# Bazs/structure_from_motion

Measured on NVIDIA B200. Metric: hyp x point evals/sec (fp64), higher is better.
Workload: dtype f64

## Files before the change

### structure_from_motion_b200/csrc/sfm_api.cu

```cuda
#include "../../include/sfm_b200.h"

#include <dlfcn.h>

#include <cmath>
#include <cstdarg>
#include <cstdio>
#include <cstdlib>
#include <cstring>
#include <string>
#include <vector>

#include "sfm_device.cuh"
#include "sfm_fit.cuh"
#include "sfm_linalg.cuh"
#include "sfm_score.cuh"
#include "sfm_homography.cuh"
#include "sfm_pose.cuh"
#include "sfm_tail.cuh"
#include "sfm_misc.cuh"
#include "sfm_match.cuh"
#include "sfm_harris.cuh"
#include "sfm_select.cuh"

using namespace sfm;

static_assert(sizeof(Corr) == 32, "Corr must be 32 bytes");
static_assert(sizeof(PoseSet) == sizeof(sfm_poses), "PoseSet/sfm_poses layout mismatch");
static_assert(sizeof(SelectRecord) == SFM_RECORD_BYTES, "SelectRecord / SFM_RECORD_BYTES mismatch");
static_assert(sizeof(ModelScores) == sizeof(sfm_model_scores), "ModelScores / sfm_model_scores layout mismatch");

namespace {

thread_local std::string g_err;

int fail(int code, const char* fmt, ...) {
    char buf[512];
    va_list ap;
    va_start(ap, fmt);
    vsnprintf(buf, sizeof buf, fmt, ap);
    va_end(ap);
    g_err = buf;
    return code;
}

}

int sfm_internal_set_error(int code, const char* message) {
    g_err = message;
    return code;
}

namespace {

#define CU(call)                                                                                   \
    do {                                                                                           \
        cudaError_t e_ = (call);                                                                   \
        if (e_ != cudaSuccess)                                                                     \
            return fail(SFM_ERR_CUDA, "%s failed: %s (%s:%d)", #call, cudaGetErrorString(e_), __FILE__, \
                        __LINE__);                                                                 \
    } while (0)

struct Buf {
    void* p = nullptr;
    size_t cap = 0;
    int reserve(size_t bytes) {
        if (bytes <= cap) return 0;
        if (p) cudaFree(p);
        p = nullptr;
        cap = 0;
        size_t want = bytes + bytes / 4 + 256;
        cudaError_t e = cudaMalloc(&p, want);
        if (e != cudaSuccess) return fail(SFM_ERR_CUDA, "cudaMalloc(%zu) failed: %s", want, cudaGetErrorString(e));
        cap = want;
        return 0;
    }
    template <class T>
    T* as() const { return reinterpret_cast<T*>(p); }
    void release() {
        if (p) cudaFree(p);
        p = nullptr;
        cap = 0;
    }
};

enum { T_UPLOAD = 0, T_SAMPLE, T_FIT, T_SCORE, T_SELECT, T_MASK, T_POSE, T_TRI, T_COUNT };

}

struct sfm_ctx {
    int device = 0;
    int sm_count = 148;
    cudaStream_t own_stream = nullptr, stream = nullptr;
    Buf raw, pts, offsets, Ks, table, E, valid, eig;
    Buf acc, count_extra, S1, S2, err, blocks, best, invalid, winnerE, spts, bounds, fitflag, record, merged, rows, blockinv;
    Buf m_img, m_feat, m_W, m_ss, m_ok, m_S, m_out;
    Buf h_img, h_gx, h_gy, h_corner, h_alive, h_key, h_idx, h_small, h_xy;
    Buf mask, sed, poses, pass, X, idx, scan, tmp, tailstate, num, winrec, bout;
    Buf planes, hK;
    Buf selstate, selio, selpp;
    long long n = 0, h = 0, npairs = 1;
    long long first_len = 0;
    long long batch_max_len = 0;
    long long raw_stride = 1;
    bool batched = false, has_pts = false, has_table = false, has_models = false, has_score = false;
    bool models_h = false;
    int hscore_occ = 0;
    bool table_pending = false;
    unsigned long long smp_seed = 0, smp_stream = 0;
    long long smp_offset = 0;
    bool acc_clean = false;
    size_t acc_planes_for = 0;
    double Kstage[9] = {0};
    double hstage[18] = {0};
    std::vector<SelectModels> sstage;
    std::vector<double> Kbatch;
    const void* occ_fn[4] = {nullptr, nullptr, nullptr, nullptr};
    int occ_blocks[4] = {0, 0, 0, 0};
    int occ_next = 0;
    void* nccl_comm = nullptr;
    int nccl_rank = 0, nccl_world = 1;
    Buf gathered;
    const unsigned long long* rescored_dev = nullptr;
    long long winner_local = -1;
    bool winner_set = false;
    long long last_idx_offset = 0;
    double Khost[9] = {1, 0, 0, 0, 1, 0, 0, 0, 1};
    int variant = SFM_SCORE_AUTO, hpt = 2, group = 16;
    bool timing = false;
    cudaEvent_t ev0[T_COUNT], ev1[T_COUNT];
    bool ev_used[T_COUNT];
    long long launches = 0;
    void* hpin = nullptr;
    size_t hpin_cap = 0;

    void tic(int s) {
        if (timing) { cudaEventRecord(ev0[s], stream); }
    }
    void toc(int s) {
        if (timing) { cudaEventRecord(ev1[s], stream); ev_used[s] = true; }
    }
};

namespace {

int ensure_pinned(sfm_ctx* c, size_t bytes) {
    if (bytes <= c->hpin_cap) return 0;
    if (c->hpin) cudaFreeHost(c->hpin);
    c->hpin = nullptr;
    c->hpin_cap = 0;
    CU(cudaMallocHost(&c->hpin, bytes + 4096));
    c->hpin_cap = bytes + 4096;
    return 0;
}

int use(sfm_ctx* c) {
    if (!c) return fail(SFM_ERR_ARG, "null context");
    CU(cudaSetDevice(c->device));
    return 0;
}

int reserve_zeroed(sfm_ctx* c, Buf& b, size_t bytes) {
    if (bytes <= b.cap) return 0;
    if (int r = b.reserve(bytes)) return r;
    CU(cudaMemsetAsync(b.p, 0, b.cap, c->stream));
    return 0;
}

int check_launch(sfm_ctx* c, const char* what) {
    cudaError_t e = cudaGetLastError();
    if (e != cudaSuccess) return fail(SFM_ERR_CUDA, "launch of %s failed: %s", what, cudaGetErrorString(e));
    c->launches += 1;
#ifdef SFM_TRACE
    fprintf(stderr, "[sfm] %s ...", what);
    fflush(stderr);
    e = cudaStreamSynchronize(c->stream);
    fprintf(stderr, " %s\n", e == cudaSuccess ? "ok" : cudaGetErrorString(e));
    fflush(stderr);
#endif
    return 0;
}

inline void chain_config(sfm_ctx* c, dim3 grid, dim3 block, size_t smem, cudaLaunchConfig_t* cfg, cudaLaunchAttribute* at) {
    memset(cfg, 0, sizeof *cfg);
    cfg->gridDim = grid;
    cfg->blockDim = block;
    cfg->dynamicSmemBytes = smem;
    cfg->stream = c->stream;
    at->id = cudaLaunchAttributeProgrammaticStreamSerialization;
    at->val.programmaticStreamSerializationAllowed = 1;
    cfg->attrs = at;
    cfg->numAttrs = SFM_PDL ? 1 : 0;
}
template <typename... KArgs, typename... Args>
cudaError_t chain_launch(sfm_ctx* c, void (*kernel)(KArgs...), dim3 grid, dim3 block, size_t smem, Args&&... args) {
    cudaLaunchConfig_t cfg;
    cudaLaunchAttribute at;
    chain_config(c, grid, block, smem, &cfg, &at);
    return cudaLaunchKernelEx(&cfg, kernel, static_cast<KArgs>(args)...);
}
inline cudaError_t chain_launch_ptr(sfm_ctx* c, const void* fn, dim3 grid, dim3 block, size_t smem, void** kargs) {
    cudaLaunchConfig_t cfg;
    cudaLaunchAttribute at;
    chain_config(c, grid, block, smem, &cfg, &at);
    return cudaLaunchKernelExC(&cfg, fn, kargs);
}

size_t score_warp_smem(int hpt, bool full) {
    switch (hpt) {
        case 1: return full ? score_warp_bytes<1, MODE_FULL>() : sizeof(ScoreWarpSmem<1>);
        case 2: return full ? score_warp_bytes<2, MODE_FULL>() : sizeof(ScoreWarpSmem<2>);
        case 4: return full ? score_warp_bytes<4, MODE_FULL>() : sizeof(ScoreWarpSmem<4>);
        default: return sizeof(ScoreWarpSmem<8>);
    }
}

const void* score_kernel(int variant, int hpt, int group) {
    if (variant == SFM_SCORE_SCREEN32) {
#define SFM_K32(H, G) if (hpt == H && group == G) return reinterpret_cast<const void*>(&k_score<H, G, MODE_SCREEN32>)
        SFM_K32(2, 16); SFM_K32(4, 8); SFM_K32(8, 4);
#undef SFM_K32
        return nullptr;
    }
#define SFM_K(H, G) if (hpt == H && group == G) return scr ? reinterpret_cast<const void*>(&k_score<H, G, MODE_SCREEN>) \
                                                           : reinterpret_cast<const void*>(&k_score<H, G, MODE_FULL>)
    const bool scr = variant == SFM_SCORE_SCREEN;
    SFM_K(1, 16); SFM_K(1, 32);
    SFM_K(2, 4); SFM_K(2, 8); SFM_K(2, 16);
    SFM_K(4, 2); SFM_K(4, 4); SFM_K(4, 8);
#undef SFM_K
    return nullptr;
}

}

extern "C" {

int sfm_version(void) { return 100; }
const char* sfm_last_error(void) { return g_err.c_str(); }

int sfm_device_count(void) {
    int n = 0;
    if (cudaGetDeviceCount(&n) != cudaSuccess) {
        cudaGetLastError();
        return 0;
    }
    return n;
}

int sfm_create(int device, sfm_ctx** out) {
    if (!out) return fail(SFM_ERR_ARG, "out is null");
    *out = nullptr;
    int n = 0;
    cudaError_t e = cudaGetDeviceCount(&n);
    if (e != cudaSuccess || n == 0) {
        cudaGetLastError();
        return fail(SFM_ERR_NO_DEVICE, "no CUDA device available (%s)",
                    e != cudaSuccess ? cudaGetErrorString(e) : "device count is 0");
    }
    if (device < 0 || device >= n) return fail(SFM_ERR_ARG, "device %d out of range [0,%d)", device, n);
    CU(cudaSetDevice(device));
    cudaDeviceProp prop;
    CU(cudaGetDeviceProperties(&prop, device));
    if (prop.major < 10)
        return fail(SFM_ERR_NO_DEVICE, "device %d is sm_%d%d; this library is built for sm_100a only", device,
                    prop.major, prop.minor);
    sfm_ctx* c = new sfm_ctx();
    c->device = device;
    c->sm_count = prop.multiProcessorCount;
    CU(cudaStreamCreateWithFlags(&c->own_stream, cudaStreamNonBlocking));
    c->stream = c->own_stream;
    for (int i = 0; i < T_COUNT; ++i) {
        CU(cudaEventCreate(&c->ev0[i]));
        CU(cudaEventCreate(&c->ev1[i]));
        c->ev_used[i] = false;
    }
    CU(cudaFuncSetAttribute(k_fit, cudaFuncAttributeMaxDynamicSharedMemorySize,
                            (int)(kFitThreads * kFitSmemDoubles * sizeof(double))));
    *out = c;
    return 0;
}

int sfm_destroy(sfm_ctx* c) {
    if (!c) return 0;
    cudaSetDevice(c->device);
    cudaStreamSynchronize(c->stream);
    Buf* bufs[] = {&c->raw, &c->pts, &c->offsets, &c->Ks, &c->table, &c->E, &c->valid, &c->eig, &c->acc,
                   &c->count_extra, &c->S1, &c->S2, &c->err, &c->blocks, &c->best,
                   &c->invalid, &c->winnerE, &c->record, &c->merged, &c->rows, &c->blockinv, &c->mask, &c->sed, &c->poses, &c->pass, &c->X, &c->idx,
                   &c->planes, &c->hK, &c->selstate, &c->selio, &c->selpp,
                   &c->scan, &c->tmp, &c->gathered, &c->tailstate, &c->num, &c->winrec, &c->bout, &c->spts, &c->bounds, &c->fitflag,
                   &c->m_img, &c->m_feat, &c->m_W, &c->m_ss, &c->m_ok, &c->m_S, &c->m_out,
                   &c->h_img, &c->h_gx, &c->h_gy, &c->h_corner, &c->h_alive, &c->h_key, &c->h_idx, &c->h_small, &c->h_xy};
    for (Buf* b : bufs) b->release();
    for (int i = 0; i < T_COUNT; ++i) {
        cudaEventDestroy(c->ev0[i]);
        cudaEventDestroy(c->ev1[i]);
    }
    sfm_nccl_destroy(c);
    if (c->hpin) cudaFreeHost(c->hpin);
    cudaStreamDestroy(c->own_stream);
    delete c;
    return 0;
}

int sfm_set_stream(sfm_ctx* c, void* s) {
    if (int r = use(c)) return r;
    c->stream = s ? (cudaStream_t)s : c->own_stream;
    return 0;
}

int sfm_use_default_stream(sfm_ctx* c) {
    if (int r = use(c)) return r;
    c->stream = cudaStreamLegacy;
    return 0;
}

int sfm_synchronize(sfm_ctx* c) {
    if (int r = use(c)) return r;
    CU(cudaStreamSynchronize(c->stream));
    return 0;
}

int sfm_set_score_variant(sfm_ctx* c, int variant, int hpt, int group) {
    if (!c) return fail(SFM_ERR_ARG, "null context");
    if (variant != SFM_SCORE_SCREEN && variant != SFM_SCORE_FULL && variant != SFM_SCORE_SCREEN32 && variant != SFM_SCORE_AUTO)
        return fail(SFM_ERR_ARG, "bad variant %d", variant);
    int nh = hpt ? hpt : c->hpt, ng = group ? group : c->group;
    if (!hpt && (variant == SFM_SCORE_SCREEN32) != (c->variant == SFM_SCORE_SCREEN32)) {
        nh = variant == SFM_SCORE_SCREEN32 ? 4 : 2;
        ng = variant == SFM_SCORE_SCREEN32 ? 8 : 16;
    }
    if (!score_kernel(variant == SFM_SCORE_AUTO ? SFM_SCORE_SCREEN : variant, nh, ng) ||
        (variant == SFM_SCORE_AUTO && !score_kernel(SFM_SCORE_FULL, nh, ng)))
        return fail(SFM_ERR_ARG, "unsupported combination: hyps_per_thread %d, group %d", nh, ng);
    c->variant = variant;
    c->hpt = nh;
    c->group = ng;
    return 0;
}

int sfm_host_alloc(uint64_t bytes, void** out) {
    if (!out) return fail(SFM_ERR_ARG, "out is null");
    CU(cudaMallocHost(out, bytes ? bytes : 1));
    return 0;
}
int sfm_host_free(void* p) {
    if (p) CU(cudaFreeHost(p));
    return 0;
}

int sfm_set_table(sfm_ctx* c, const int32_t* table, int64_t h) {
    if (int r = use(c)) return r;
    if (!table || h <= 0) return fail(SFM_ERR_ARG, "bad table");
    if (!c->has_pts) return fail(SFM_ERR_STATE, "upload correspondences before the sample table");
    for (int64_t i = 0; i < 8 * h; ++i)
        if (table[i] < 0 || table[i] >= c->n) return fail(SFM_ERR_ARG, "table[%lld] = %d out of range", (long long)i, table[i]);
    if (int r = c->table.reserve((size_t)h * 32)) return r;
    CU(cudaMemcpyAsync(c->table.p, table, (size_t)h * 32, cudaMemcpyHostToDevice, c->stream));
    CU(cudaStreamSynchronize(c->stream));
    c->h = h;
    c->npairs = 1;
    c->has_table = true;
    c->table_pending = false;
    c->has_models = false;
    c->has_score = false;
    return 0;
}

static int sample_device(sfm_ctx* c, uint64_t seed, uint64_t stream, int64_t hyp_offset, int64_t h) {
    if (h <= 0) return fail(SFM_ERR_ARG, "need h > 0");
    if (!c->has_pts) return fail(SFM_ERR_STATE, "upload correspondences before sampling");
    if (!c->batched && c->n < 8) return fail(SFM_ERR_ARG, "need at least 8 correspondences");
    if (int r = c->table.reserve((size_t)h * c->npairs * 32)) return r;
    c->smp_seed = seed;
    c->smp_stream = stream;
    c->smp_offset = hyp_offset;
    c->table_pending = true;
    c->h = h;
    c->has_table = true;
    c->has_models = false;
    c->has_score = false;
    return 0;
}

static int ensure_table(sfm_ctx* c) {
    if (!c->table_pending) return 0;
    c->tic(T_SAMPLE);
    dim3 grid((unsigned)((c->h + 127) / 128), (unsigned)c->npairs);
    k_sample<<<grid, 128, 0, c->stream>>>(c->smp_seed, c->smp_stream, c->smp_offset, c->h, c->n,
                                          c->batched ? c->offsets.as<long long>() : nullptr, c->table.as<int32_t>());
    if (int r = check_launch(c, "k_sample")) return r;
    c->toc(T_SAMPLE);
    c->table_pending = false;
    return 0;
}

int sfm_sample_device(sfm_ctx* c, uint64_t seed, uint64_t stream, int64_t hyp_offset, int64_t h) {
    if (int r = use(c)) return r;
    return sample_device(c, seed, stream, hyp_offset, h);
}

int sfm_get_table(sfm_ctx* c, int32_t* table, int64_t first, int64_t h) {
    if (int r = use(c)) return r;
    if (!c->has_table || first < 0 || h < 0 || first + h > c->h * c->npairs)
        return fail(SFM_ERR_STATE, "no table rows [%lld, %lld)", (long long)first, (long long)(first + h));
    if (int r = ensure_table(c)) return r;
    CU(cudaMemcpyAsync(table, c->table.as<int32_t>() + 8 * first, (size_t)h * 32, cudaMemcpyDeviceToHost, c->stream));
    CU(cudaStreamSynchronize(c->stream));
    return 0;
}

static int normalise_from(sfm_ctx* c, const double* xa, const double* ya, const double* xb, const double* yb,
                          int64_t stride, int64_t n, int64_t max_len) {
    if (int r = c->pts.reserve((size_t)n * sizeof(Corr))) return r;
    if (int r = c->bounds.reserve(16)) return r;
    CU(cudaMemsetAsync(c->bounds.p, 0, 16, c->stream));
    dim3 grid((unsigned)((max_len + 255) / 256), (unsigned)c->npairs);
    k_normalise<<<grid, 256, 0, c->stream>>>(xa, ya, xb, yb, stride, n,
                                             c->batched ? c->offsets.as<long long>() : nullptr,
                                             c->Ks.as<double>(), c->pts.as<Corr>(), c->bounds.as<unsigned long long>());
    return check_launch(c, "k_normalise");
}

static int stage_coords(sfm_ctx* c, double* d, const double* xa, const double* ya, const double* xb, const double* yb,
                        int64_t stride, int64_t n, const double* s[4]) {
    if (stride == 1) {
        const double* src[4] = {xa, ya, xb, yb};
        for (int k = 0; k < 4; ++k)
            CU(cudaMemcpyAsync(d + (size_t)k * n, src[k], (size_t)n * sizeof(double), cudaMemcpyHostToDevice, c->stream));
        s[0] = d; s[1] = d + n; s[2] = d + 2 * n; s[3] = d + 3 * n;
    } else if (stride == 2 && ya == xa + 1 && yb == xb + 1) {
        CU(cudaMemcpyAsync(d, xa, (size_t)n * 2 * sizeof(double), cudaMemcpyHostToDevice, c->stream));
        CU(cudaMemcpyAsync(d + 2 * n, xb, (size_t)n * 2 * sizeof(double), cudaMemcpyHostToDevice, c->stream));
        s[0] = d; s[1] = d + 1; s[2] = d + 2 * n; s[3] = d + 2 * n + 1;
    } else {
        return fail(SFM_ERR_ARG, "unsupported layout: stride must be 1 (four arrays) or 2 (two interleaved [n][2] arrays)");
    }
    return 0;
}

static void raw_coords(const sfm_ctx* c, const double* s[4]) {
    const double* d = c->raw.as<double>();
    const long long n = c->n;
    if (c->raw_stride == 1) { s[0] = d; s[1] = d + n; s[2] = d + 2 * n; s[3] = d + 3 * n; }
    else { s[0] = d; s[1] = d + 1; s[2] = d + 2 * n; s[3] = d + 2 * n + 1; }
}

static int stage_raw(sfm_ctx* c, const double* xa, const double* ya, const double* xb, const double* yb,
                     int64_t stride, int64_t n, const double* s[4]) {
    if (int r = c->raw.reserve((size_t)n * 4 * sizeof(double))) return r;
    if (int r = stage_coords(c, c->raw.as<double>(), xa, ya, xb, yb, stride, n, s)) return r;
    c->raw_stride = stride;
    return 0;
}

static int upload_pairs_impl(sfm_ctx* c, const double* xa, const double* ya, const double* xb, const double* yb,
                             int64_t stride, int64_t n, const double* K, bool on_device, bool sync) {
    if (int r = use(c)) return r;
    if (!xa || !ya || !xb || !yb || !K) return fail(SFM_ERR_ARG, "null argument");
    if (n <= 0 || (uint64_t)n >= kMaxPoints) return fail(SFM_ERR_ARG, "need 0 < n < 2^25 correspondences, got %lld", (long long)n);
    c->tic(T_UPLOAD);
    c->batched = false;
    c->npairs = 1;
    const double* s[4];
    if (on_device) {
        if (int r = c->raw.reserve((size_t)n * 4 * sizeof(double))) return r;
        double* d = c->raw.as<double>();
        const double* src[4] = {xa, ya, xb, yb};
        for (int k = 0; k < 4; ++k) {
            CU(cudaMemcpy2DAsync(d + (size_t)k * n, sizeof(double), src[k], (size_t)stride * sizeof(double),
                                 sizeof(double), (size_t)n, cudaMemcpyDeviceToDevice, c->stream));
            s[k] = d + (size_t)k * n;
        }
        c->raw_stride = stride = 1;
    } else if (int r = stage_raw(c, xa, ya, xb, yb, stride, n, s)) {
        return r;
    }
    if (int r = c->Ks.reserve(9 * sizeof(double))) return r;
    memcpy(c->Khost, K, sizeof c->Khost);
    CU(cudaMemcpyAsync(c->Ks.p, c->Khost, 9 * sizeof(double), cudaMemcpyHostToDevice, c->stream));
    c->n = n;
    if (int r = normalise_from(c, s[0], s[1], s[2], s[3], stride, n, n)) return r;
    c->toc(T_UPLOAD);
    if (sync) CU(cudaStreamSynchronize(c->stream));
    c->has_pts = true;
    c->has_table = c->has_models = c->has_score = false;
    c->table_pending = false;
    c->winner_set = false;
    return 0;
}

int sfm_upload_pairs(sfm_ctx* c, const double* xa, const double* ya, const double* xb, const double* yb,
                     int64_t stride, int64_t n, const double* K) {
    return upload_pairs_impl(c, xa, ya, xb, yb, stride, n, K, false, true);
}

int sfm_upload_pairs_async(sfm_ctx* c, const double* xa, const double* ya, const double* xb, const double* yb,
                           int64_t stride, int64_t n, const double* K) {
    return upload_pairs_impl(c, xa, ya, xb, yb, stride, n, K, false, false);
}

int sfm_upload_pairs_d(sfm_ctx* c, const double* xa, const double* ya, const double* xb, const double* yb,
                       int64_t stride, int64_t n, const double* K) {
    return upload_pairs_impl(c, xa, ya, xb, yb, stride, n, K, true, true);
}

int sfm_get_normalised(sfm_ctx* c, double* out, int64_t n) {
    if (int r = use(c)) return r;
    if (!c->has_pts || n > c->n) return fail(SFM_ERR_STATE, "no correspondences of that size");
    CU(cudaMemcpyAsync(out, c->pts.p, (size_t)n * sizeof(Corr), cudaMemcpyDeviceToHost, c->stream));
    CU(cudaStreamSynchronize(c->stream));
    return 0;
}

static size_t acc_tail_bytes(long long P) { return 64 + (size_t)P * 4; }

static int fit_launch(sfm_ctx* c, bool want_eig) {
    if (!c->has_pts || !c->has_table) return fail(SFM_ERR_STATE, "fit needs correspondences and a sample table");
    const size_t H = (size_t)c->h * c->npairs;
    if (int r = c->E.reserve(H * 9 * sizeof(double))) return r;
    if (int r = c->valid.reserve(H)) return r;
    if (want_eig)
        if (int r = c->eig.reserve(H * 9 * sizeof(double))) return r;
    if (int r = reserve_zeroed(c, c->fitflag, 16)) return r;
    if (int r = c->rows.reserve(H * sizeof(ModelRow))) return r;
    const size_t acc_tail = acc_tail_bytes(c->npairs);
    if (int r = c->acc.reserve(H * kAccWords * 8 + acc_tail)) return r;
    if (want_eig)
        if (int r = ensure_table(c)) return r;
    c->tic(T_FIT);
    const long long* off = c->batched ? c->offsets.as<long long>() : nullptr;
    dim3 grid((unsigned)((c->h + kFitThreads - 1) / kFitThreads), (unsigned)c->npairs);
    const unsigned* only = nullptr;
    if (!want_eig) {
        dim3 gq((unsigned)((c->h + kFitQrThreads - 1) / kFitQrThreads), (unsigned)c->npairs);
        CU(chain_launch(c, k_fit_qr, gq, dim3(kFitQrThreads), 0, c->pts.as<Corr>(), off, c->table.as<int32_t>(), c->h,
                        c->E.as<double>(), c->valid.as<uint8_t>(), c->fitflag.as<unsigned>(), c->rows.as<ModelRow>(),
                        c->acc.as<unsigned long long>(), kAccWords, (int)((acc_tail + 7) / 8), c->table_pending ? 1 : 0,
                        c->smp_seed, c->smp_stream, c->smp_offset, c->n));
        if (int r = check_launch(c, "k_fit_qr")) return r;
        c->table_pending = false;
        only = c->fitflag.as<unsigned>();
        c->acc_clean = true;
        c->acc_planes_for = H;
    } else {
        c->acc_clean = false;
    }
    CU(chain_launch(c, k_fit, grid, dim3(kFitThreads), kFitThreads * kFitSmemDoubles * sizeof(double), c->pts.as<Corr>(), off,
                    c->table.as<int32_t>(), c->h, c->E.as<double>(), c->valid.as<uint8_t>(),
                    want_eig ? c->eig.as<double>() : nullptr, only, c->rows.as<ModelRow>()));
    if (int r = check_launch(c, "k_fit")) return r;
    c->toc(T_FIT);
    c->has_models = true;
    c->models_h = false;
    c->has_score = false;
    return 0;
}

int sfm_fit(sfm_ctx* c, double* E_out, uint8_t* valid_out, double* eig_out) {
    if (int r = use(c)) return r;
    if (int r = fit_launch(c, eig_out != nullptr)) return r;
    const size_t H = (size_t)c->h * c->npairs;
    if (E_out) CU(cudaMemcpyAsync(E_out, c->E.p, H * 72, cudaMemcpyDeviceToHost, c->stream));
    if (valid_out) CU(cudaMemcpyAsync(valid_out, c->valid.p, H, cudaMemcpyDeviceToHost, c->stream));
    if (eig_out) CU(cudaMemcpyAsync(eig_out, c->eig.p, H * 72, cudaMemcpyDeviceToHost, c->stream));
    CU(cudaStreamSynchronize(c->stream));
    return 0;
}

int sfm_get_models(sfm_ctx* c, int64_t first, int64_t count, double* E_out, uint8_t* valid_out) {
    if (int r = use(c)) return r;
    const int64_t total = c->h * c->npairs;
    if (!c->has_models || first < 0 || count < 0 || first + count > total)
        return fail(SFM_ERR_STATE, "no models [%lld, %lld)", (long long)first, (long long)(first + count));
    if (E_out) CU(cudaMemcpyAsync(E_out, c->E.as<double>() + 9 * first, (size_t)count * 72, cudaMemcpyDeviceToHost, c->stream));
    if (valid_out) CU(cudaMemcpyAsync(valid_out, c->valid.as<uint8_t>() + first, (size_t)count, cudaMemcpyDeviceToHost, c->stream));
    CU(cudaStreamSynchronize(c->stream));
    return 0;
}

int sfm_set_models(sfm_ctx* c, const double* E, const uint8_t* valid, int64_t h) {
    if (int r = use(c)) return r;
    if (!E || h <= 0) return fail(SFM_ERR_ARG, "bad models");
    if (c->batched) return fail(SFM_ERR_STATE, "set_models is a single-pair call");
    if (c->has_table && h != c->h) return fail(SFM_ERR_ARG, "model count %lld != table rows %lld", (long long)h, c->h);
    if (int r = c->E.reserve((size_t)h * 72)) return r;
    if (int r = c->valid.reserve((size_t)h)) return r;
    CU(cudaMemcpyAsync(c->E.p, E, (size_t)h * 72, cudaMemcpyHostToDevice, c->stream));
    if (valid) CU(cudaMemcpyAsync(c->valid.p, valid, (size_t)h, cudaMemcpyHostToDevice, c->stream));
    else CU(cudaMemsetAsync(c->valid.p, 1, (size_t)h, c->stream));
    if (int r = c->rows.reserve((size_t)h * sizeof(ModelRow))) return r;
    k_pad_models<<<(unsigned)((h + 255) / 256), 256, 0, c->stream>>>(c->E.as<double>(), (long long)h, c->rows.as<ModelRow>());
    if (int r = check_launch(c, "k_pad_models")) return r;
    CU(cudaStreamSynchronize(c->stream));
    c->h = h;
    c->has_models = true;
    c->models_h = false;
    c->has_score = false;
    c->acc_clean = false;
    return 0;
}

static int reserve_selection(sfm_ctx* c, long long h, long long P) {
    const size_t H = (size_t)h * P;
    const int fblocks = (int)((h + 255) / 256);
    if (int r = c->count_extra.reserve(H * 4)) return r;
    if (int r = c->S1.reserve(H * 8)) return r;
    if (int r = c->S2.reserve(H * 8)) return r;
    if (int r = c->err.reserve(H * 8)) return r;
    if (int r = c->blocks.reserve((size_t)fblocks * P * sizeof(Best))) return r;
    if (int r = c->best.reserve((size_t)P * sizeof(Best))) return r;
    if (int r = c->invalid.reserve((size_t)P * 16)) return r;
    return 0;
}

struct ItemSplit { long long chunk, nsplit; };
static ItemSplit split_items(long long target_items, long long hyp_items, long long max_len, long long tile) {
    const long long tiles = (max_len + tile - 1) / tile;
    long long nsplit = (target_items + hyp_items - 1) / hyp_items;
    constexpr int min_tiles = 2;
    const long long max_split = tiles / min_tiles > 0 ? tiles / min_tiles : 1;
    if (nsplit > max_split) nsplit = max_split;
    const long long min_split = (max_len + kMaxItemPoints - 1) / kMaxItemPoints;
    if (nsplit < min_split) nsplit = min_split;
    if (nsplit < 1) nsplit = 1;
    const long long chunk = ((tiles + nsplit - 1) / nsplit) * tile;
    nsplit = (max_len + chunk - 1) / chunk;
    if (nsplit < 1) nsplit = 1;
    return {chunk, nsplit};
}

static int clear_acc(sfm_ctx* c, size_t H, long long P) {
    if (!(c->acc_clean && c->acc_planes_for == H))
        CU(cudaMemsetAsync(c->acc.p, 0, H * kAccWords * 8 + acc_tail_bytes(P), c->stream));
    c->acc_clean = false;
    return 0;
}

static int finalise_launch(sfm_ctx* c, int kind, double thr, double min_extra, int agg, int mode, bool use_table,
                           long long idx_offset, int sums, int e2, int force_rescore, unsigned long long* acc_dev) {
    const long long h = c->h, P = c->npairs;
    const size_t H = (size_t)h * P;
    const int fblocks = (int)((h + 255) / 256);
    c->tic(T_SELECT);
    FinalArgs f;
    f.pts = c->pts.as<Corr>();
    f.offsets = c->batched ? c->offsets.as<long long>() : nullptr;
    f.E = c->E.as<double>();
    f.valid = c->valid.as<uint8_t>();
    f.table = use_table ? c->table.as<int32_t>() : nullptr;
    f.h = h;
    f.n = c->n;
    f.idx_offset = idx_offset;
    f.htotal = (long long)H;
    f.acc = acc_dev;
    f.inv_scale1 = ldexp(1.0, e2 - kFixedBits);
    f.sums = sums;
    f.inv_scale2 = ldexp(1.0, 2 * e2 - kFixedBits);
    f.thr = thr;
    f.min_extra = min_extra;
    f.agg = agg;
    f.mode = mode;
    f.count_extra = c->count_extra.as<int32_t>();
    f.S1 = c->S1.as<double>();
    f.S2 = c->S2.as<double>();
    f.err = c->err.as<double>();
    f.block_out = c->blocks.as<Best>();
    if (int r = c->blockinv.reserve((size_t)fblocks * P * 16)) return r;
    f.block_inv = c->blockinv.as<long long>();
    if (int r = c->record.reserve((size_t)P * sizeof(SelectRecord))) return r;
    f.force_rescore = force_rescore;
    f.rescored = reinterpret_cast<unsigned long long*>(reinterpret_cast<char*>(acc_dev + H * kAccWords) + 8);
    f.tickets = reinterpret_cast<unsigned*>(reinterpret_cast<char*>(acc_dev + H * kAccWords) + 64);
    c->rescored_dev = f.rescored;
    f.out = c->best.as<Best>();
    f.invalid_out = c->invalid.as<long long>();
    f.record = c->record.as<SelectRecord>();
    f.fitflag = c->fitflag.as<unsigned>();
    if (kind == MODEL_H) CU(chain_launch(c, k_finalise<MODEL_H>, dim3((unsigned)fblocks, (unsigned)P), dim3(256), 0, f));
    else CU(chain_launch(c, k_finalise<MODEL_E>, dim3((unsigned)fblocks, (unsigned)P), dim3(256), 0, f));
    if (int r = check_launch(c, "k_finalise")) return r;
    c->toc(T_SELECT);
    c->has_score = true;
    c->last_idx_offset = idx_offset;
    c->winner_set = false;
    return 0;
}

static int score_launch(sfm_ctx* c, double thr, double min_extra, int agg, int mode, bool use_table,
                        long long idx_offset, long long max_len, bool both_sums = false) {
    int sums = both_sums ? (SUM_S1 | SUM_S2) : ((agg == AGG_SUM || agg == AGG_MEAN) ? SUM_S1 : SUM_S2);
    if (mode == SELECT_MSAC) sums |= SUM_S1;
    if (!c->has_pts || !c->has_models) return fail(SFM_ERR_STATE, "score needs correspondences and fitted models");
    if (c->models_h) return fail(SFM_ERR_STATE, "the models are homographies: score them with sfm_ransac_homography");
    if (use_table && !c->has_table) return fail(SFM_ERR_STATE, "sample rule requested but no table is loaded");
    if (use_table)
        if (int r = ensure_table(c)) return r;
    if (agg < 0 || agg > 3) return fail(SFM_ERR_ARG, "bad aggregation %d", agg);
    if (mode < 0 || mode > 2) return fail(SFM_ERR_ARG, "bad selection %d", mode);
    const bool skip_k2 = !(thr >= 0.0) || thr > 1e100;
    const int force_rescore = (thr > 1e100) ? 1 : 0;
    const long long h = c->h, P = c->npairs;
    const int hpt = (c->variant == SFM_SCORE_SCREEN32 && thr > 1e6) ? 2 : c->hpt;
    const int G = (c->variant == SFM_SCORE_SCREEN32 && thr > 1e6) ? 16 : c->group;
    const long long hblocks = (h + 32ll * hpt - 1) / (32ll * hpt);
    const size_t H = (size_t)h * P;
    if (int r = reserve_selection(c, h, P)) return r;
    int e2 = 0;
    if (thr > 0.0 && !skip_k2) (void)frexp(thr, &e2);
    if (e2 < -400) e2 = -400;
    const bool autov = c->variant == SFM_SCORE_AUTO;
    int variant = autov ? SFM_SCORE_SCREEN : c->variant;
    if (variant == SFM_SCORE_SCREEN32 && thr > 1e6) variant = SFM_SCORE_SCREEN;
    const bool f32 = variant == SFM_SCORE_SCREEN32;
    const bool screen = variant != SFM_SCORE_FULL;
    double thr_pre = f32 ? thr * kThr32Factor : (screen ? thr * (1.0 + 1e-9) : thr * (1.0 + 1e-9) + 1e-22);
    if (f32 && thr_pre < 1e-24) thr_pre = 1e-24;
    if (screen && thr_pre < 1e-280) thr_pre = 1e-280;
    const double s_scale = sqrt(thr_pre);
    const double scale1 = ldexp(1.0, 63 - e2), scale2 = ldexp(1.0, 63 - 2 * e2);
    unsigned long long* acc_dev = nullptr;
    {
        const void* fn = score_kernel(variant, hpt, G);
        if (!fn) return fail(SFM_ERR_ARG, "unsupported scoring configuration (variant %d, hpt %d, group %d)", variant, hpt, G);
        const size_t smem_one = (size_t)kScoreWarps * score_warp_smem(hpt, false);
        const size_t smem_two = (size_t)kScoreWarps * score_warp_smem(hpt, true);
        const size_t smem_both = smem_one > smem_two ? smem_one : smem_two;
        const size_t smem = screen ? smem_one : smem_two;
        auto occupancy = [&](const void* f, size_t bytes, int* out) -> int {
            for (int k = 0; k < 4; ++k)
                if (c->occ_fn[k] == f) { *out = c->occ_blocks[k]; return 0; }
            int o = 0;
            CU(cudaFuncSetAttribute(f, cudaFuncAttributeMaxDynamicSharedMemorySize, (int)bytes));
            CU(cudaOccupancyMaxActiveBlocksPerMultiprocessor(&o, f, kScoreThreads, bytes));
            if (o < 1) o = 1;
            c->occ_fn[c->occ_next] = f;
            c->occ_blocks[c->occ_next] = o;
            c->occ_next = (c->occ_next + 1) & 3;
            *out = o;
            return 0;
        };
        int occ = 0;
        if (int r = occupancy(fn, smem, &occ)) return r;
#ifndef SFM_AUTO_SINGLE
#define SFM_AUTO_SINGLE 1
#endif
        const void* fn_auto = nullptr;
        if (autov && SFM_AUTO_SINGLE) {
            if (hpt == 2 && G == 16) fn_auto = reinterpret_cast<const void*>(&k_score_auto<2, 16>);
            if (hpt == 4 && G == 8) fn_auto = reinterpret_cast<const void*>(&k_score_auto<4, 8>);
        }
        if (fn_auto)
            if (int r = occupancy(fn_auto, smem_both, &occ)) return r;
        const void* fn_full = (autov && !fn_auto) ? score_kernel(SFM_SCORE_FULL, hpt, G) : nullptr;
        int occ_full = 0;
        if (fn_full)
            if (int r = occupancy(fn_full, smem_two, &occ_full)) return r;
        const long long grid_blocks = (long long)c->sm_count * occ;
        constexpr int items_per_warp = 32;
        const ItemSplit sp = split_items(grid_blocks * kScoreWarps * items_per_warp, hblocks * P, max_len, kTile);
        const long long chunk = sp.chunk, nsplit = sp.nsplit;
        const long long total_items = hblocks * nsplit * P;
        if (int r = c->acc.reserve(H * kAccWords * 8 + acc_tail_bytes(P))) return r;
        const long long npts = c->n;
        if (f32) { if (int r = c->spts.reserve((size_t)npts * sizeof(Corr32))) return r; }
        else if (screen) { if (int r = c->spts.reserve((size_t)npts * sizeof(Corr))) return r; }
        ScoreArgs a;
        a.pts = c->pts.as<Corr>();
        a.spts = screen ? c->spts.p : c->pts.p;
        a.bounds = c->bounds.as<double>();
        a.s = s_scale;
        a.kappa_coef = kKappaCoef * (1.0 + thr);
        a.kappa32_coef = kKappa32Coef * (1.0 + thr);
        a.n = c->n;
        a.offsets = c->batched ? c->offsets.as<long long>() : nullptr;
        a.E = c->E.as<double>();
        a.rows = c->rows.as<ModelRow>();
        a.h = h;
        a.thr = thr;
        a.thr_pre = thr_pre;
        a.scale1 = scale1;
        a.scale2 = scale2;
        a.sums = sums;
        a.chunk = chunk;
        a.hblocks = (int)hblocks;
        a.nsplit = (int)nsplit;
        a.total_items = total_items;
        a.htotal = (long long)H;
        a.acc = c->acc.as<unsigned long long>();
        a.work_counter = reinterpret_cast<unsigned*>(a.acc + H * kAccWords);
        char* tailp = reinterpret_cast<char*>(a.acc + H * kAccWords);
        a.mode_flag = autov ? reinterpret_cast<const int*>(tailp + 32) : nullptr;
        acc_dev = a.acc;
        c->tic(T_SCORE);
        if (int r = clear_acc(c, H, P)) return r;
        if (f32 && !skip_k2) {
            k_screen_pts32<<<(unsigned)((npts + 255) / 256), 256, 0, c->stream>>>(c->pts.as<Corr>(), npts, 1.0 / s_scale,
                                                                                  reinterpret_cast<Corr32*>(c->spts.p));
            if (int r = check_launch(c, "k_screen_pts32")) return r;
        }
        else if (screen && !skip_k2) {
            PilotArgs pa;
            pa.E = c->E.as<double>();
            pa.h = h;
            pa.plen = c->batched ? c->first_len : c->n;
            pa.thr_pre = thr_pre;
            pa.counters = reinterpret_cast<unsigned*>(tailp + 16);
            pa.mode_flag = autov ? reinterpret_cast<int*>(tailp + 32) : nullptr;
            CU(chain_launch(c, k_screen_pts64, dim3((unsigned)((npts + 255) / 256)), dim3(256), 0, c->pts.as<Corr>(), npts,
                            1.0 / s_scale, reinterpret_cast<Corr*>(c->spts.p), pa));
            if (int r = check_launch(c, "k_screen_pts64")) return r;
        }
        const long long want_blocks = (total_items + kScoreWarps - 1) / kScoreWarps;
        const long long launch_blocks = grid_blocks < want_blocks ? grid_blocks : want_blocks;
        void* kargs[] = {(void*)&a};
        if (!skip_k2 && fn_auto) {
            ScoreArgs a2 = a;
            a2.thr_pre = thr * (1.0 + 1e-9) + 1e-22;
            a2.spts = c->pts.p;
            void* kargs2[] = {(void*)&a, (void*)&a2};
            CU(chain_launch_ptr(c, fn_auto, dim3((unsigned)launch_blocks), dim3(kScoreThreads), smem_both, kargs2));
            if (int r = check_launch(c, "k_score_auto")) return r;
        } else if (!skip_k2) {
            CU(chain_launch_ptr(c, fn, dim3((unsigned)launch_blocks), dim3(kScoreThreads), smem, kargs));
            if (int r = check_launch(c, "k_score")) return r;
            if (fn_full) {
                ScoreArgs a2 = a;
                a2.thr_pre = thr * (1.0 + 1e-9) + 1e-22;
                a2.spts = c->pts.p;
                const long long gb2 = (long long)c->sm_count * occ_full;
                const long long lb2 = gb2 < want_blocks ? gb2 : want_blocks;
                void* kargs2[] = {(void*)&a2};
                CU(chain_launch_ptr(c, fn_full, dim3((unsigned)lb2), dim3(kScoreThreads), smem_two, kargs2));
                if (int r = check_launch(c, "k_score")) return r;
            }
        }
        c->toc(T_SCORE);
    }

    return finalise_launch(c, MODEL_E, thr, min_extra, agg, mode, use_table, idx_offset, sums, e2, force_rescore, acc_dev);
}

int sfm_score(sfm_ctx* c, double thr, double min_extra, int agg, int mode, int use_table, int64_t idx_offset,
              int32_t* count_extra, double* S1, double* S2, double* err) {
    if (int r = use(c)) return r;
    if (c->batched) return fail(SFM_ERR_STATE, "sfm_score is a single-pair call; use sfm_batch_ransac");
    if (int r = score_launch(c, thr, min_extra, agg, mode, use_table != 0, idx_offset, c->n, S1 || S2)) return r;
    const size_t H = (size_t)c->h;
    if (count_extra) CU(cudaMemcpyAsync(count_extra, c->count_extra.p, H * 4, cudaMemcpyDeviceToHost, c->stream));
    if (S1) CU(cudaMemcpyAsync(S1, c->S1.p, H * 8, cudaMemcpyDeviceToHost, c->stream));
    if (S2) CU(cudaMemcpyAsync(S2, c->S2.p, H * 8, cudaMemcpyDeviceToHost, c->stream));
    if (err) CU(cudaMemcpyAsync(err, c->err.p, H * 8, cudaMemcpyDeviceToHost, c->stream));
    CU(cudaStreamSynchronize(c->stream));
    return 0;
}

static void unpack_best(const SelectRecord& r, sfm_best* out) {
    out->err = r.best.idx >= 0 ? r.best.err : __builtin_inf();
    out->index = r.best.idx;
    out->count_extra = r.best.count;
    out->reserved = 0;
    out->num_invalid = r.num_invalid;
    out->first_invalid = r.first_invalid;
    memcpy(out->E, r.E, 72);
    memcpy(out->sample, r.sample, 32);
}

static int fetch_best(sfm_ctx* c, sfm_best* out) {
    if (int r = ensure_pinned(c, sizeof(SelectRecord))) return r;
    CU(cudaMemcpyAsync(c->hpin, c->record.p, sizeof(SelectRecord), cudaMemcpyDeviceToHost, c->stream));
    CU(cudaStreamSynchronize(c->stream));
    SelectRecord r;
    memcpy(&r, c->hpin, sizeof r);
    unpack_best(r, out);
    if (r.best.idx >= 0) {
        c->winner_local = r.best.idx - c->last_idx_offset;
        c->winner_set = true;
    }
    return 0;
}

int sfm_get_best(sfm_ctx* c, sfm_best* out) {
    if (int r = use(c)) return r;
    if (!out) return fail(SFM_ERR_ARG, "out is null");
    if (!c->has_score || c->batched) return fail(SFM_ERR_STATE, "no single-pair score to read");
    return fetch_best(c, out);
}

int sfm_near_ties(sfm_ctx* c, double rel_tol, int64_t cap, int64_t* idx_out, int64_t* count) {
    if (int r = use(c)) return r;
    if (!idx_out || !count || cap <= 0 || cap > 4096) return fail(SFM_ERR_ARG, "bad near-tie arguments");
    if (!c->has_score || c->batched) return fail(SFM_ERR_STATE, "no single-pair score to read");
    if (int r = c->tmp.reserve((size_t)cap * 8 + 16)) return r;
    unsigned* cnt = c->tmp.as<unsigned>();
    long long* out = reinterpret_cast<long long*>(c->tmp.as<char>() + 16);
    CU(cudaMemsetAsync(cnt, 0, 16, c->stream));
    const int blocks = (int)((c->h + 255) / 256 < 4 * c->sm_count ? (c->h + 255) / 256 : 4 * c->sm_count);
    k_near_ties<<<blocks, 256, 0, c->stream>>>(c->err.as<double>(), c->h, c->record.as<SelectRecord>(), rel_tol, (int)cap, out, cnt);
    if (int r = check_launch(c, "k_near_ties")) return r;
    if (int r = ensure_pinned(c, (size_t)cap * 8 + 16)) return r;
    CU(cudaMemcpyAsync(c->hpin, c->tmp.p, (size_t)cap * 8 + 16, cudaMemcpyDeviceToHost, c->stream));
    CU(cudaStreamSynchronize(c->stream));
    unsigned n;
    memcpy(&n, c->hpin, 4);
    *count = n;
    const int64_t take = n < (unsigned)cap ? n : cap;
    memcpy(idx_out, (char*)c->hpin + 16, (size_t)take * 8);
    return 0;
}

int sfm_get_rescored(sfm_ctx* c, int64_t* count) {
    if (int r = use(c)) return r;
    if (!count) return fail(SFM_ERR_ARG, "null argument");
    if (!c->rescored_dev) return fail(SFM_ERR_STATE, "no scoring call yet");
    if (int r = ensure_pinned(c, 8)) return r;
    CU(cudaMemcpyAsync(c->hpin, c->rescored_dev, 8, cudaMemcpyDeviceToHost, c->stream));
    CU(cudaStreamSynchronize(c->stream));
    unsigned long long v;
    memcpy(&v, c->hpin, 8);
    *count = (int64_t)v;
    return 0;
}

int sfm_set_winner(sfm_ctx* c, int64_t local_index, const double* E) {
    if (int r = use(c)) return r;
    if (local_index >= 0) {
        if (!c->has_models || local_index >= c->h) return fail(SFM_ERR_ARG, "winner index out of range");
        c->winner_local = local_index;
    } else {
        if (!E) return fail(SFM_ERR_ARG, "need the winning model when it lives on another rank");
        if (int r = c->winnerE.reserve(72)) return r;
        CU(cudaMemcpyAsync(c->winnerE.p, E, 72, cudaMemcpyHostToDevice, c->stream));
        CU(cudaStreamSynchronize(c->stream));
        c->winner_local = -1;
    }
    c->winner_set = true;
    return 0;
}

static const double* winner_E_dev(sfm_ctx* c) {
    return c->winner_local >= 0 ? c->E.as<double>() + 9 * c->winner_local : c->winnerE.as<double>();
}

static int mask_launch(sfm_ctx* c, double thr, const Best* best_dev, const double* E_override = nullptr) {
    if (int r = c->mask.reserve((size_t)c->n)) return r;
    if (int r = c->sed.reserve((size_t)c->n * 8)) return r;
    c->tic(T_MASK);
    const double* E = E_override ? E_override : (best_dev ? c->E.as<double>() : winner_E_dev(c));
    k_inlier_mask<<<(unsigned)((c->n + 255) / 256), 256, 0, c->stream>>>(
        c->pts.as<Corr>(), c->n, E, E_override ? nullptr : best_dev, c->last_idx_offset, 0, thr, c->mask.as<uint8_t>(),
        c->sed.as<double>());
    if (int r = check_launch(c, "k_inlier_mask")) return r;
    c->toc(T_MASK);
    return 0;
}

int sfm_inlier_mask(sfm_ctx* c, double thr, uint8_t* mask, double* sed) {
    if (int r = use(c)) return r;
    if (!c->has_pts || c->batched) return fail(SFM_ERR_STATE, "no single-pair correspondences loaded");
    if (!c->winner_set) return fail(SFM_ERR_STATE, "no winner: call sfm_get_best or sfm_set_winner first");
    if (c->models_h && c->winner_local >= 0) return fail(SFM_ERR_STATE, "the winner is a homography: use sfm_homography_mask");
    if (int r = mask_launch(c, thr, nullptr)) return r;
    if (mask) CU(cudaMemcpyAsync(mask, c->mask.p, (size_t)c->n, cudaMemcpyDeviceToHost, c->stream));
    if (sed) CU(cudaMemcpyAsync(sed, c->sed.p, (size_t)c->n * 8, cudaMemcpyDeviceToHost, c->stream));
    CU(cudaStreamSynchronize(c->stream));
    return 0;
}

int sfm_ransac_essential(sfm_ctx* c, double thr, double min_extra, int agg, int mode, sfm_best* best,
                         uint8_t* mask, double* sed) {
    if (int r = use(c)) return r;
    if (!best) return fail(SFM_ERR_ARG, "best is null");
    if (c->batched) return fail(SFM_ERR_STATE, "single-pair call on a batched context");
    if (int r = fit_launch(c, false)) return r;
    if (int r = score_launch(c, thr, min_extra, agg, mode, true, 0, c->n)) return r;
    if (mask || sed) {
        if (int r = mask_launch(c, thr, c->best.as<Best>())) return r;
        if (mask) CU(cudaMemcpyAsync(mask, c->mask.p, (size_t)c->n, cudaMemcpyDeviceToHost, c->stream));
        if (sed) CU(cudaMemcpyAsync(sed, c->sed.p, (size_t)c->n * 8, cudaMemcpyDeviceToHost, c->stream));
    }
    return fetch_best(c, best);
}

static int fit_h_launch(sfm_ctx* c) {
    if (!c->has_pts || !c->has_table) return fail(SFM_ERR_STATE, "fit needs correspondences and a sample table");
    if (c->batched && !c->table_pending) return fail(SFM_ERR_STATE, "a batch is fitted from the device sampler's draw");
    const long long h = c->h, P = c->npairs;
    const size_t H = (size_t)h * P;
    if (int r = c->E.reserve(H * 72)) return r;
    if (int r = c->valid.reserve(H)) return r;
    const size_t acc_tail = acc_tail_bytes(P);
    if (int r = c->acc.reserve(H * kAccWords * 8 + acc_tail)) return r;
    c->tic(T_FIT);
    CU(chain_launch(c, k_fit_homography, dim3((unsigned)((h + kFitHThreads - 1) / kFitHThreads), (unsigned)P),
                    dim3(kFitHThreads), 0, c->pts.as<Corr>(), c->batched ? c->offsets.as<long long>() : nullptr,
                    c->table.as<int32_t>(), h, c->E.as<double>(), c->valid.as<uint8_t>(), c->acc.as<unsigned long long>(),
                    kAccWords, (int)((acc_tail + 7) / 8), c->table_pending ? 1 : 0, c->smp_seed, c->smp_stream,
                    c->smp_offset, c->n));
    if (int r = check_launch(c, "k_fit_homography")) return r;
    c->toc(T_FIT);
    c->table_pending = false;
    c->acc_clean = true;
    c->acc_planes_for = H;
    c->has_models = true;
    c->models_h = true;
    c->has_score = false;
    return 0;
}

static int score_h_launch(sfm_ctx* c, double thr, double min_extra, int agg, int mode, long long max_len) {
    if (agg < 0 || agg > 3) return fail(SFM_ERR_ARG, "bad aggregation %d", agg);
    if (mode < 0 || mode > 2) return fail(SFM_ERR_ARG, "bad selection %d", mode);
    int sums = (agg == AGG_SUM || agg == AGG_MEAN) ? SUM_S1 : SUM_S2;
    if (mode == SELECT_MSAC) sums |= SUM_S1;
    const bool skip_k2 = !(thr >= 0.0) || thr > 1e100;
    const int force_rescore = (thr > 1e100) ? 1 : 0;
    const long long h = c->h, n = c->n, P = c->npairs;
    const size_t H = (size_t)h * P;
    int e2 = 0;
    if (thr > 0.0 && !skip_k2) (void)frexp(thr * (1.0 + 0x1p-20), &e2);
    if (e2 < -400) e2 = -400;
    if (int r = reserve_selection(c, h, P)) return r;
    if (int r = c->acc.reserve(H * kAccWords * 8 + acc_tail_bytes(P))) return r;
    unsigned long long* acc = c->acc.as<unsigned long long>();
    const size_t smem = kHScoreWarps * sizeof(HScoreWarpSmem);
    if (!c->hscore_occ) {
        int o = 0;
        CU(cudaOccupancyMaxActiveBlocksPerMultiprocessor(&o, k_score_homography<kHScoreHpt>, kHScoreThreads, smem));
        c->hscore_occ = o > 0 ? o : 1;
    }
    const long long grid_blocks = (long long)c->sm_count * c->hscore_occ;
    const long long hblocks = (h + 32ll * kHScoreHpt - 1) / (32ll * kHScoreHpt);
    const ItemSplit sp = split_items(grid_blocks * kHScoreWarps * 32, hblocks * P, max_len, kHTile);
    const long long chunk = sp.chunk, nsplit = sp.nsplit;
    HScoreArgs a;
    a.pts = c->pts.as<Corr>();
    a.offsets = c->batched ? c->offsets.as<long long>() : nullptr;
    a.H = c->E.as<double>();
    a.n = n;
    a.h = h;
    a.htotal = (long long)H;
    a.thr = thr;
    a.scale1 = ldexp(1.0, 63 - e2);
    a.scale2 = ldexp(1.0, 63 - 2 * e2);
    a.sums = sums;
    a.chunk = chunk;
    a.hblocks = (int)hblocks;
    a.nsplit = (int)nsplit;
    a.total_items = hblocks * nsplit * P;
    a.work_counter = reinterpret_cast<unsigned*>(acc + H * kAccWords);
    a.acc = acc;
    c->tic(T_SCORE);
    if (int r = clear_acc(c, H, P)) return r;
    if (!skip_k2) {
        const long long want = (a.total_items + kHScoreWarps - 1) / kHScoreWarps;
        CU(chain_launch(c, k_score_homography<kHScoreHpt>, dim3((unsigned)(grid_blocks < want ? grid_blocks : want)),
                        dim3(kHScoreThreads), smem, a));
        if (int r = check_launch(c, "k_score_homography")) return r;
    }
    c->toc(T_SCORE);
    return finalise_launch(c, MODEL_H, thr, min_extra, agg, mode, true, 0, sums, e2, force_rescore, acc);
}

static int hmask_launch(sfm_ctx* c, double thr, const double* H_dev, const Best* best_dev) {
    if (int r = c->mask.reserve((size_t)c->n)) return r;
    if (int r = c->sed.reserve((size_t)c->n * 8)) return r;
    c->tic(T_MASK);
    CU(chain_launch(c, k_homography_mask, dim3((unsigned)((c->n + 255) / 256)), dim3(256), 0, c->pts.as<Corr>(), c->n,
                    H_dev, best_dev, thr, c->mask.as<uint8_t>(), c->sed.as<double>()));
    if (int r = check_launch(c, "k_homography_mask")) return r;
    c->toc(T_MASK);
    return 0;
}

int sfm_fit_homography(sfm_ctx* c, double* H_out, uint8_t* valid_out) {
    if (int r = use(c)) return r;
    if (c->batched) return fail(SFM_ERR_STATE, "homography estimation is a single-pair call; use sfm_batch_two_view_homography");
    if (int r = fit_h_launch(c)) return r;
    if (H_out) CU(cudaMemcpyAsync(H_out, c->E.p, (size_t)c->h * 72, cudaMemcpyDeviceToHost, c->stream));
    if (valid_out) CU(cudaMemcpyAsync(valid_out, c->valid.p, (size_t)c->h, cudaMemcpyDeviceToHost, c->stream));
    CU(cudaStreamSynchronize(c->stream));
    return 0;
}

int sfm_ransac_homography(sfm_ctx* c, double thr, double min_extra, int agg, int mode, sfm_best* best, uint8_t* mask,
                          double* err, int32_t* count_extra_h, double* err_h) {
    if (int r = use(c)) return r;
    if (!best) return fail(SFM_ERR_ARG, "best is null");
    if (c->batched) return fail(SFM_ERR_STATE, "single-pair call on a batched context");
    if (c->has_pts && c->n < 8) return fail(SFM_ERR_ARG, "need at least 8 correspondences, got %lld", c->n);
    if (int r = fit_h_launch(c)) return r;
    if (int r = score_h_launch(c, thr, min_extra, agg, mode, c->n)) return r;
    if (mask || err) {
        if (int r = hmask_launch(c, thr, c->E.as<double>(), c->best.as<Best>())) return r;
        if (mask) CU(cudaMemcpyAsync(mask, c->mask.p, (size_t)c->n, cudaMemcpyDeviceToHost, c->stream));
        if (err) CU(cudaMemcpyAsync(err, c->sed.p, (size_t)c->n * 8, cudaMemcpyDeviceToHost, c->stream));
    }
    if (count_extra_h) CU(cudaMemcpyAsync(count_extra_h, c->count_extra.p, (size_t)c->h * 4, cudaMemcpyDeviceToHost, c->stream));
    if (err_h) CU(cudaMemcpyAsync(err_h, c->err.p, (size_t)c->h * 8, cudaMemcpyDeviceToHost, c->stream));
    return fetch_best(c, best);
}

int sfm_homography_mask(sfm_ctx* c, const double* H, double thr, uint8_t* mask, double* err) {
    if (int r = use(c)) return r;
    if (!c->has_pts || c->batched) return fail(SFM_ERR_STATE, "no single-pair correspondences loaded");
    const double* H_dev;
    if (H) {
        if (int r = c->winnerE.reserve(72)) return r;
        CU(cudaMemcpyAsync(c->winnerE.p, H, 72, cudaMemcpyHostToDevice, c->stream));
        H_dev = c->winnerE.as<double>();
    } else {
        if (!c->models_h || !c->winner_set || c->winner_local < 0)
            return fail(SFM_ERR_STATE, "no homography winner: pass H or run sfm_ransac_homography first");
        H_dev = c->E.as<double>() + 9 * c->winner_local;
    }
    if (int r = hmask_launch(c, thr, H_dev, nullptr)) return r;
    if (mask) CU(cudaMemcpyAsync(mask, c->mask.p, (size_t)c->n, cudaMemcpyDeviceToHost, c->stream));
    if (err) CU(cudaMemcpyAsync(err, c->sed.p, (size_t)c->n * 8, cudaMemcpyDeviceToHost, c->stream));
    CU(cudaStreamSynchronize(c->stream));
    return 0;
}

int sfm_decompose_essential(sfm_ctx* c, const double* E, sfm_poses* out) {
    if (int r = use(c)) return r;
    if (!E || !out) return fail(SFM_ERR_ARG, "null argument");
    if (int r = c->tmp.reserve(72)) return r;
    if (int r = c->poses.reserve(sizeof(PoseSet))) return r;
    CU(cudaMemcpyAsync(c->tmp.p, E, 72, cudaMemcpyHostToDevice, c->stream));
    k_decompose<<<1, 32, 0, c->stream>>>(c->tmp.as<double>(), nullptr, 0, c->poses.as<PoseSet>(), 1);
    if (int r = check_launch(c, "k_decompose")) return r;
    CU(cudaMemcpyAsync(out, c->poses.p, sizeof(PoseSet), cudaMemcpyDeviceToHost, c->stream));
    CU(cudaStreamSynchronize(c->stream));
    return 0;
}

static int recover_pose_impl(sfm_ctx* c, const double* E, const double* K9, const double* xa, const double* ya,
                             const double* xb, const double* yb, int64_t stride, int64_t m, double dist_thr,
                             sfm_poses* out, uint8_t* pass4) {
    if (int r = use(c)) return r;
    if (!E || !out) return fail(SFM_ERR_ARG, "null argument");
    if (m < 0) return fail(SFM_ERR_ARG, "negative count");
    if (int r = c->tmp.reserve(72 + 9 * 8 + (size_t)m * 4 * 8 + (size_t)m * sizeof(Corr) + 64)) return r;
    if (int r = c->poses.reserve(sizeof(PoseSet))) return r;
    if (int r = c->pass.reserve((size_t)m + 1)) return r;
    c->tic(T_POSE);
    double* dE = c->tmp.as<double>();
    double* dK = dE + 9;
    double* draw = dK + 9;
    Corr* dpts = reinterpret_cast<Corr*>(((uintptr_t)(draw + 4 * m) + 31) & ~(uintptr_t)31);
    CU(cudaMemcpyAsync(dE, E, 72, cudaMemcpyHostToDevice, c->stream));
    k_decompose<<<1, 32, 0, c->stream>>>(dE, nullptr, 0, c->poses.as<PoseSet>(), 1);
    if (int r = check_launch(c, "k_decompose")) return r;
    if (m > 0) {
        if (!xa || !ya || !xb || !yb) return fail(SFM_ERR_ARG, "null coordinates");
        const double I[9] = {1, 0, 0, 0, 1, 0, 0, 0, 1};
        memcpy(c->Kstage, K9 ? K9 : I, 72);
        CU(cudaMemcpyAsync(dK, c->Kstage, 72, cudaMemcpyHostToDevice, c->stream));
        const double* s[4];
        if (int r = stage_coords(c, draw, xa, ya, xb, yb, stride, m, s)) return r;
        k_normalise<<<dim3((unsigned)((m + 255) / 256), 1), 256, 0, c->stream>>>(s[0], s[1], s[2], s[3], stride, m, nullptr, dK, dpts, nullptr);
        if (int r = check_launch(c, "k_normalise")) return r;
        k_cheirality<<<(unsigned)((4 * m + 127) / 128), 128, 0, c->stream>>>(dpts, m, nullptr, nullptr, c->poses.as<PoseSet>(),
                                                                        dist_thr, c->pass.as<uint8_t>(), nullptr);
        if (int r = check_launch(c, "k_cheirality")) return r;
    }
    k_vote<<<1, 32, 0, c->stream>>>(c->poses.as<PoseSet>());
    if (int r = check_launch(c, "k_vote")) return r;
    c->toc(T_POSE);
    CU(cudaMemcpyAsync(out, c->poses.p, sizeof(PoseSet), cudaMemcpyDeviceToHost, c->stream));
    if (pass4 && m > 0) CU(cudaMemcpyAsync(pass4, c->pass.p, (size_t)m, cudaMemcpyDeviceToHost, c->stream));
    CU(cudaStreamSynchronize(c->stream));
    return 0;
}

int sfm_recover_pose(sfm_ctx* c, const double* E, const double* xa, const double* ya, const double* xb,
                     const double* yb, int64_t stride, int64_t m, double dist_thr, sfm_poses* out,
                     uint8_t* pass4) {
    return recover_pose_impl(c, E, nullptr, xa, ya, xb, yb, stride, m, dist_thr, out, pass4);
}

int sfm_recover_pose_pixels(sfm_ctx* c, const double* E, const double* K, const double* xa, const double* ya,
                            const double* xb, const double* yb, int64_t stride, int64_t m, double dist_thr,
                            sfm_poses* out, uint8_t* pass4) {
    if (!K) return fail(SFM_ERR_ARG, "null camera matrix");
    return recover_pose_impl(c, E, K, xa, ya, xb, yb, stride, m, dist_thr, out, pass4);
}

int sfm_triangulate(sfm_ctx* c, const double* P1, const double* P2, const double* xa, const double* ya,
                    const double* xb, const double* yb, int64_t stride, int64_t m, double* X) {
    if (int r = use(c)) return r;
    if (!P1 || !P2 || !X) return fail(SFM_ERR_ARG, "null argument");
    if (m <= 0) return m == 0 ? 0 : fail(SFM_ERR_ARG, "negative count");
    if (!xa || !ya || !xb || !yb) return fail(SFM_ERR_ARG, "null coordinates");
    if (int r = c->tmp.reserve(24 * 8 + (size_t)m * 4 * 8)) return r;
    if (int r = c->X.reserve((size_t)m * 24)) return r;
    c->tic(T_TRI);
    double* dP = c->tmp.as<double>();
    double* draw = dP + 24;
    CU(cudaMemcpyAsync(dP, P1, 96, cudaMemcpyHostToDevice, c->stream));
    CU(cudaMemcpyAsync(dP + 12, P2, 96, cudaMemcpyHostToDevice, c->stream));
    const double* s[4];
    if (int r = stage_coords(c, draw, xa, ya, xb, yb, stride, m, s)) return r;
    k_triangulate<<<(unsigned)((m + 127) / 128), 128, 0, c->stream>>>(s[0], s[1], s[2], s[3], stride, m, nullptr, dP, dP + 12,
                                                                      nullptr, nullptr, nullptr, 0, c->X.as<double>());
    if (int r = check_launch(c, "k_triangulate")) return r;
    c->toc(T_TRI);
    CU(cudaMemcpyAsync(X, c->X.p, (size_t)m * 24, cudaMemcpyDeviceToHost, c->stream));
    CU(cudaStreamSynchronize(c->stream));
    return 0;
}

static int pose_tail_launch(sfm_ctx* c, double thr, double dist_thr, const SelectRecord* rec_dev, long long max_len,
                            uint8_t* mask_host = nullptr, double* sed_host = nullptr, int kind = MODEL_E,
                            double rot_tol = 0.0) {
    const long long n = c->n, P = c->npairs;
    if (max_len < 1) max_len = 1;
    const int nblk = (int)((max_len + kTailPerBlock - 1) / kTailPerBlock);
    if (int r = c->mask.reserve((size_t)n)) return r;
    if (int r = c->sed.reserve((size_t)n * 8)) return r;
    if (int r = c->idx.reserve((size_t)n * 8)) return r;
    if (int r = c->num.reserve((size_t)P * 8)) return r;
    if (int r = c->poses.reserve((size_t)P * sizeof(PoseSet))) return r;
    if (int r = c->pass.reserve((size_t)n + 1)) return r;
    if (int r = c->X.reserve((size_t)n * 24)) return r;
    const size_t state_bytes = (size_t)P * nblk * 8 + (size_t)P * 8;
    if (int r = reserve_zeroed(c, c->tailstate, state_bytes)) return r;
    TailArgs a;
    a.pts = c->pts.as<Corr>();
    a.offsets = c->batched ? c->offsets.as<long long>() : nullptr;
    a.n = n;
    a.rec = rec_dev;
    a.thr = thr;
    a.dist_thr = dist_thr;
    a.mask = c->mask.as<uint8_t>();
    a.sed = c->sed.as<double>();
    a.idx = c->idx.as<long long>();
    a.num = c->num.as<long long>();
    a.agg = c->tailstate.as<unsigned long long>();
    a.ticket = reinterpret_cast<unsigned*>(a.agg + (size_t)P * nblk);
    a.done = a.ticket + P;
    a.poses = c->poses.as<PoseSet>();
    a.pass = c->pass.as<uint8_t>();
    const double* s[4];
    raw_coords(c, s);
    a.xa = s[0]; a.ya = s[1]; a.xb = s[2]; a.yb = s[3];
    a.stride = c->raw_stride;
    a.Ks = c->Ks.as<double>();
    a.X = c->X.as<double>();
    a.planes = nullptr;
    a.rot_tol = rot_tol;
    if (kind == MODEL_H) {
        if (int r = c->planes.reserve((size_t)P * sizeof(HPlane))) return r;
        a.planes = c->planes.as<HPlane>();
        if (!c->batched) a.Ks = c->hK.as<double>();
    }
    c->tic(T_MASK);
    if (kind == MODEL_H) CU(chain_launch(c, k_tail_mask<MODEL_H>, dim3((unsigned)nblk, (unsigned)P), dim3(kTailBlock), 0, a));
    else CU(chain_launch(c, k_tail_mask<MODEL_E>, dim3((unsigned)nblk, (unsigned)P), dim3(kTailBlock), 0, a));
    if (int r = check_launch(c, "k_tail_mask")) return r;
    c->toc(T_MASK);
    if (mask_host) CU(cudaMemcpyAsync(mask_host, c->mask.p, (size_t)n, cudaMemcpyDeviceToHost, c->stream));
    if (sed_host) CU(cudaMemcpyAsync(sed_host, c->sed.p, (size_t)n * 8, cudaMemcpyDeviceToHost, c->stream));
    c->tic(T_POSE);
    const long long cap_blocks = P >= 64 ? 8 : 2ll * c->sm_count;
    const long long g2 = (4 * max_len + 127) / 128, g3 = (max_len + 127) / 128;
    const dim3 grid2((unsigned)(g2 < cap_blocks ? g2 : cap_blocks), (unsigned)P);
    if (kind == MODEL_H) CU(chain_launch(c, k_tail_cheirality<MODEL_H>, grid2, dim3(128), 0, a));
    else CU(chain_launch(c, k_tail_cheirality<MODEL_E>, grid2, dim3(128), 0, a));
    if (int r = check_launch(c, "k_tail_cheirality")) return r;
    c->toc(T_POSE);
    c->tic(T_TRI);
    CU(chain_launch(c, k_tail_triangulate, dim3((unsigned)(g3 < cap_blocks ? g3 : cap_blocks), (unsigned)P), dim3(128), 0, a));
    if (int r = check_launch(c, "k_tail_triangulate")) return r;
    c->toc(T_TRI);
    return 0;
}

static int host_winner_record(sfm_ctx* c, const SelectRecord** out) {
    if (int r = c->winrec.reserve(sizeof(SelectRecord))) return r;
    if (c->has_table)
        if (int r = ensure_table(c)) return r;
    const int32_t* row = (c->has_table && c->winner_local >= 0) ? c->table.as<int32_t>() + 8 * c->winner_local : nullptr;
    k_make_record<<<1, 32, 0, c->stream>>>(winner_E_dev(c), row, c->winner_local >= 0 ? c->winner_local : 0,
                                           c->winrec.as<SelectRecord>());
    if (int r = check_launch(c, "k_make_record")) return r;
    *out = c->winrec.as<SelectRecord>();
    return 0;
}

constexpr long long kSpecInliers = 2048;

static int copy_inliers(sfm_ctx* c, long long take, int64_t* inlier_idx, uint8_t* pass, double* X) {
    if (inlier_idx) CU(cudaMemcpyAsync(inlier_idx, c->idx.p, (size_t)take * 8, cudaMemcpyDeviceToHost, c->stream));
    if (pass) CU(cudaMemcpyAsync(pass, c->pass.p, (size_t)take, cudaMemcpyDeviceToHost, c->stream));
    if (X) CU(cudaMemcpyAsync(X, c->X.p, (size_t)take * 24, cudaMemcpyDeviceToHost, c->stream));
    CU(cudaStreamSynchronize(c->stream));
    return 0;
}

static int pose_tail_fetch(sfm_ctx* c, sfm_poses* poses, int64_t cap, int64_t* num_inliers, int64_t* inlier_idx,
                           uint8_t* pass, double* X, sfm_best* best , HPlane* planes = nullptr) {
    const long long* cnt_dev = c->num.as<long long>();
    const long long spec = c->n < kSpecInliers ? c->n : kSpecInliers;
    const size_t o_idx = 64 + ((sizeof(SelectRecord) + 63) / 64) * 64, o_pass = o_idx + (size_t)spec * 8,
                 o_X = ((o_pass + (size_t)spec + 63) / 64) * 64;
    if (int r = ensure_pinned(c, o_X + (size_t)spec * 24)) return r;
    char* hp = (char*)c->hpin;
    CU(cudaMemcpyAsync(hp, cnt_dev, 8, cudaMemcpyDeviceToHost, c->stream));
    if (best) CU(cudaMemcpyAsync(hp + 64, c->record.p, sizeof(SelectRecord), cudaMemcpyDeviceToHost, c->stream));
    CU(cudaMemcpyAsync(poses, c->poses.p, sizeof(PoseSet), cudaMemcpyDeviceToHost, c->stream));
    if (planes) CU(cudaMemcpyAsync(planes, c->planes.p, sizeof(HPlane), cudaMemcpyDeviceToHost, c->stream));
    if (spec > 0) {
        if (inlier_idx) CU(cudaMemcpyAsync(hp + o_idx, c->idx.p, (size_t)spec * 8, cudaMemcpyDeviceToHost, c->stream));
        if (pass) CU(cudaMemcpyAsync(hp + o_pass, c->pass.p, (size_t)spec, cudaMemcpyDeviceToHost, c->stream));
        if (X) CU(cudaMemcpyAsync(hp + o_X, c->X.p, (size_t)spec * 24, cudaMemcpyDeviceToHost, c->stream));
    }
    CU(cudaStreamSynchronize(c->stream));
    long long m;
    memcpy(&m, hp, 8);
    if (best) {
        SelectRecord r;
        memcpy(&r, hp + 64, sizeof r);
        unpack_best(r, best);
        if (r.best.idx >= 0) {
            c->winner_local = r.best.idx - c->last_idx_offset;
            c->winner_set = true;
        } else {
            m = 0;
        }
    }
    *num_inliers = m;
    const long long take = m < cap ? m : cap;
    if (take > 0 && take <= spec) {
        if (inlier_idx) memcpy(inlier_idx, hp + o_idx, (size_t)take * 8);
        if (pass) memcpy(pass, hp + o_pass, (size_t)take);
        if (X) memcpy(X, hp + o_X, (size_t)take * 24);
    } else if (take > 0) {
        return copy_inliers(c, take, inlier_idx, pass, X);
    }
    return 0;
}

int sfm_pose_and_triangulate(sfm_ctx* c, double thr, double dist_thr, sfm_poses* poses, int64_t cap,
                             int64_t* num_inliers, int64_t* inlier_idx, uint8_t* pass, double* X) {
    if (int r = use(c)) return r;
    if (!poses || !num_inliers) return fail(SFM_ERR_ARG, "null argument");
    if (!c->has_pts || c->batched) return fail(SFM_ERR_STATE, "no single-pair correspondences loaded");
    if (!c->winner_set) return fail(SFM_ERR_STATE, "no winner: run sfm_ransac_essential / sfm_get_best first");
    if (c->models_h && c->winner_local >= 0)
        return fail(SFM_ERR_STATE, "the winner is a homography: use sfm_homography_pose_and_triangulate");
    const SelectRecord* rec = nullptr;
    if (int r = host_winner_record(c, &rec)) return r;
    if (int r = pose_tail_launch(c, thr, dist_thr, rec, c->n)) return r;
    return pose_tail_fetch(c, poses, cap, num_inliers, inlier_idx, pass, X, nullptr);
}

static void pack_hposes(const PoseSet& p, const HPlane& pl, sfm_hposes* out) {
    memcpy(out->R, p.R, sizeof out->R);
    memcpy(out->t, p.t, sizeof out->t);
    memcpy(out->n, pl.n, sizeof out->n);
    memcpy(out->d, pl.d, sizeof out->d);
    memcpy(out->sv, p.sv, sizeof out->sv);
    memcpy(out->counts, p.counts, sizeof out->counts);
    out->best = p.best;
    out->rotation_only = pl.rotation_only;
}

static int hpose_tail_fetch(sfm_ctx* c, sfm_hposes* poses, int64_t cap, int64_t* num_inliers, int64_t* inlier_idx,
                            uint8_t* pass, double* X, sfm_best* best ) {
    PoseSet p;
    HPlane pl;
    if (int r = pose_tail_fetch(c, reinterpret_cast<sfm_poses*>(&p), cap, num_inliers, inlier_idx, pass, X, best, &pl))
        return r;
    pack_hposes(p, pl, poses);
    return 0;
}

static int check_camera(const double* K) {
    if (!K) return fail(SFM_ERR_ARG, "null camera matrix");
    for (int i = 0; i < 9; ++i)
        if (!std::isfinite(K[i])) return fail(SFM_ERR_ARG, "the camera matrix is not finite");
    const double det = K[0] * (K[4] * K[8] - K[5] * K[7]) - K[1] * (K[3] * K[8] - K[5] * K[6]) +
                       K[2] * (K[3] * K[7] - K[4] * K[6]);
    if (det == 0.0 || K[0] == 0.0 || K[4] == 0.0) return fail(SFM_ERR_ARG, "the camera matrix is singular");
    return 0;
}

static int hpose_args(const double* K, double rot_tol) {
    if (int r = check_camera(K)) return r;
    if (K[3] != 0.0 || K[6] != 0.0 || K[7] != 0.0 || K[8] != 1.0)
        return fail(SFM_ERR_ARG, "the camera matrix must be upper triangular with K[2,2] = 1");
    if (std::isnan(rot_tol)) return fail(SFM_ERR_ARG, "rotation_tolerance is NaN");
    return 0;
}

static int hpose_stage_k(sfm_ctx* c, const double* K) {
    if (int r = c->hK.reserve(72)) return r;
    memcpy(c->hstage + 9, K, 72);
    CU(cudaMemcpyAsync(c->hK.p, c->hstage + 9, 72, cudaMemcpyHostToDevice, c->stream));
    return 0;
}

int sfm_decompose_homography(sfm_ctx* c, const double* H, const double* K, double rotation_tolerance, sfm_hposes* out) {
    if (int r = use(c)) return r;
    if (!H || !out) return fail(SFM_ERR_ARG, "null argument");
    if (int r = hpose_args(K, rotation_tolerance)) return r;
    if (int r = c->tmp.reserve(144)) return r;
    if (int r = c->poses.reserve(sizeof(PoseSet))) return r;
    if (int r = c->planes.reserve(sizeof(HPlane))) return r;
    memcpy(c->hstage, H, 72);
    memcpy(c->hstage + 9, K, 72);
    CU(cudaMemcpyAsync(c->tmp.p, c->hstage, 144, cudaMemcpyHostToDevice, c->stream));
    k_decompose_homography<<<1, 32, 0, c->stream>>>(c->tmp.as<double>(), c->tmp.as<double>() + 9, rotation_tolerance,
                                                    c->poses.as<PoseSet>(), c->planes.as<HPlane>());
    if (int r = check_launch(c, "k_decompose_homography")) return r;
    PoseSet p;
    HPlane pl;
    CU(cudaMemcpyAsync(&p, c->poses.p, sizeof p, cudaMemcpyDeviceToHost, c->stream));
    CU(cudaMemcpyAsync(&pl, c->planes.p, sizeof pl, cudaMemcpyDeviceToHost, c->stream));
    CU(cudaStreamSynchronize(c->stream));
    pack_hposes(p, pl, out);
    return 0;
}

int sfm_homography_pose_and_triangulate(sfm_ctx* c, const double* K, double thr, double dist_thr, double rotation_tolerance,
                                        sfm_hposes* poses, int64_t cap, int64_t* num_inliers, int64_t* inlier_idx,
                                        uint8_t* pass, double* X) {
    if (int r = use(c)) return r;
    if (!poses || !num_inliers) return fail(SFM_ERR_ARG, "null argument");
    if (int r = hpose_args(K, rotation_tolerance)) return r;
    if (!c->has_pts || c->batched) return fail(SFM_ERR_STATE, "no single-pair correspondences loaded");
    if (!c->models_h || !c->winner_set || c->winner_local < 0)
        return fail(SFM_ERR_STATE, "no homography winner: run sfm_ransac_homography or sfm_set_winner first");
    const SelectRecord* rec = nullptr;
    if (int r = host_winner_record(c, &rec)) return r;
    if (int r = hpose_stage_k(c, K)) return r;
    if (int r = pose_tail_launch(c, thr, dist_thr, rec, c->n, nullptr, nullptr, MODEL_H, rotation_tolerance)) return r;
    return hpose_tail_fetch(c, poses, cap, num_inliers, inlier_idx, pass, X, nullptr);
}

int sfm_two_view_homography(sfm_ctx* c, const double* K, double thr, double min_extra, int agg, int mode, double dist_thr,
                            double rotation_tolerance, sfm_best* best, sfm_hposes* poses, int64_t cap, int64_t* num_inliers,
                            int64_t* inlier_idx, uint8_t* pass, double* X, uint8_t* mask, double* err) {
    if (int r = use(c)) return r;
    if (!best || !poses || !num_inliers) return fail(SFM_ERR_ARG, "null argument");
    if (int r = hpose_args(K, rotation_tolerance)) return r;
    if (c->batched) return fail(SFM_ERR_STATE, "single-pair call on a batched context");
    if (c->has_pts && c->n < 8) return fail(SFM_ERR_ARG, "need at least 8 correspondences, got %lld", c->n);
    if (int r = hpose_stage_k(c, K)) return r;
    if (int r = fit_h_launch(c)) return r;
    if (int r = score_h_launch(c, thr, min_extra, agg, mode, c->n)) return r;
    if (int r = pose_tail_launch(c, thr, dist_thr, c->record.as<SelectRecord>(), c->n, mask, err, MODEL_H, rotation_tolerance))
        return r;
    return hpose_tail_fetch(c, poses, cap, num_inliers, inlier_idx, pass, X, best);
}

static int score_models_launch(sfm_ctx* c, double sigma, double homography_ratio, long long max_len,
                               sfm_model_scores* out, double* per_point) {
    const long long P = c->npairs;
    const size_t o_out = (size_t)P * sizeof(SelectModels);
    if (int r = reserve_zeroed(c, c->selstate, (size_t)P * kSelectStateWords * 8)) return r;
    if (int r = c->selio.reserve(o_out + (size_t)P * sizeof(ModelScores))) return r;
    if (per_point)
        if (int r = c->selpp.reserve((size_t)c->n * 32)) return r;
    char* base = c->selio.as<char>();
    CU(cudaMemcpyAsync(base, c->sstage.data(), (size_t)P * sizeof(SelectModels), cudaMemcpyHostToDevice, c->stream));
    SelectArgs a;
    const double* s[4];
    raw_coords(c, s);
    a.xa = s[0]; a.ya = s[1]; a.xb = s[2]; a.yb = s[3];
    a.stride = c->raw_stride;
    a.n = c->n;
    a.offsets = c->batched ? c->offsets.as<long long>() : nullptr;
    a.models = reinterpret_cast<const SelectModels*>(base);
    a.sigma = sigma;
    a.ratio = homography_ratio;
    a.state = c->selstate.as<unsigned long long>();
    a.out = reinterpret_cast<ModelScores*>(base + o_out);
    a.per_point = per_point ? c->selpp.as<double>() : nullptr;
    const long long blocks = (max_len + kSelectBlock - 1) / kSelectBlock, cap = (4ll * c->sm_count + P - 1) / P;
    const long long gx = blocks < cap ? blocks : cap;
    c->tic(T_SCORE);
    k_score_models<<<dim3((unsigned)(gx > 0 ? gx : 1), (unsigned)P), kSelectBlock, 0, c->stream>>>(a);
    if (int r = check_launch(c, "k_score_models")) return r;
    c->toc(T_SCORE);
    CU(cudaMemcpyAsync(out, a.out, (size_t)P * sizeof(ModelScores), cudaMemcpyDeviceToHost, c->stream));
    if (per_point) CU(cudaMemcpyAsync(per_point, c->selpp.p, (size_t)c->n * 32, cudaMemcpyDeviceToHost, c->stream));
    CU(cudaStreamSynchronize(c->stream));
    return 0;
}

static int score_models_args(double sigma, double homography_ratio) {
    if (!(sigma > 0.0) || !std::isfinite(sigma)) return fail(SFM_ERR_ARG, "sigma must be finite and > 0");
    if (!std::isfinite(homography_ratio)) return fail(SFM_ERR_ARG, "homography_ratio is not finite");
    return 0;
}

static int models_finite(const double* E, const double* H, const char* pair) {
    for (int i = 0; i < 9; ++i) {
        if (E && !std::isfinite(E[i])) return fail(SFM_ERR_ARG, "E%s is not finite", pair);
        if (H && !std::isfinite(H[i])) return fail(SFM_ERR_ARG, "H%s is not finite", pair);
    }
    return 0;
}

static void stage_models(SelectModels& m, const double* E, const double* H, const double* K) {
    memset(&m, 0, sizeof m);
    if (E) memcpy(m.E, E, 72);
    if (H) memcpy(m.H, H, 72);
    memcpy(m.K, K, 72);
    m.have_e = E ? 1 : 0;
    m.have_h = H ? 1 : 0;
}

int sfm_score_models(sfm_ctx* c, const double* E, const double* H, const double* K, double sigma, double homography_ratio,
                     sfm_model_scores* out, double* per_point) {
    if (int r = use(c)) return r;
    if (!out) return fail(SFM_ERR_ARG, "out is null");
    if (!E && !H) return fail(SFM_ERR_ARG, "give E, H or both");
    if (int r = models_finite(E, H, "")) return r;
    if (int r = check_camera(K)) return r;
    if (int r = score_models_args(sigma, homography_ratio)) return r;
    if (c->batched) return fail(SFM_ERR_STATE, "single-pair call on a batched context");
    if (!c->has_pts) return fail(SFM_ERR_STATE, "no correspondences loaded");
    c->sstage.resize(1);
    stage_models(c->sstage[0], E, H, K);
    return score_models_launch(c, sigma, homography_ratio, c->n, out, per_point);
}

int sfm_batch_score_models(sfm_ctx* c, const double* E, const uint8_t* have_e, const double* H, const uint8_t* have_h,
                           double sigma, double homography_ratio, sfm_model_scores* out, double* per_point) {
    if (int r = use(c)) return r;
    if (!out) return fail(SFM_ERR_ARG, "out is null");
    if (!E && !H) return fail(SFM_ERR_ARG, "give E, H or both");
    if (int r = score_models_args(sigma, homography_ratio)) return r;
    if (!c->batched || !c->has_pts) return fail(SFM_ERR_STATE, "no batched upload: run a batch call first");
    const long long P = c->npairs;
    c->sstage.resize((size_t)P);
    for (long long p = 0; p < P; ++p) {
        char which[48];
        snprintf(which, sizeof which, " of pair %lld", p);
        const double* K = c->Kbatch.data() + 9 * p;
        const double* Ep = (E && (!have_e || have_e[p])) ? E + 9 * p : nullptr;
        const double* Hp = (H && (!have_h || have_h[p])) ? H + 9 * p : nullptr;
        if (int r = models_finite(Ep, Hp, which)) return r;
        if (int r = check_camera(K)) {
            const std::string why = g_err;
            return fail(r, "pair %lld: %s", p, why.c_str());
        }
        stage_models(c->sstage[(size_t)p], Ep, Hp, K);
    }
    return score_models_launch(c, sigma, homography_ratio, c->batch_max_len, out, per_point);
}

int sfm_two_view_async(sfm_ctx* c, double thr, double min_extra, int agg, int mode, double dist_thr, uint8_t* mask,
                       double* sed) {
    if (int r = use(c)) return r;
    if (c->batched) return fail(SFM_ERR_STATE, "single-pair call on a batched context");
    if (int r = fit_launch(c, false)) return r;
    if (int r = score_launch(c, thr, min_extra, agg, mode, true, 0, c->n)) return r;
    return pose_tail_launch(c, thr, dist_thr, c->record.as<SelectRecord>(), c->n, mask, sed);
}

int sfm_two_view_fetch(sfm_ctx* c, sfm_best* best, sfm_poses* poses, int64_t cap, int64_t* num_inliers,
                       int64_t* inlier_idx, uint8_t* pass, double* X) {
    if (int r = use(c)) return r;
    if (!best || !poses || !num_inliers) return fail(SFM_ERR_ARG, "null argument");
    if (!c->has_score || c->batched) return fail(SFM_ERR_STATE, "sfm_two_view_async first");
    return pose_tail_fetch(c, poses, cap, num_inliers, inlier_idx, pass, X, best);
}

int sfm_two_view(sfm_ctx* c, double thr, double min_extra, int agg, int mode, double dist_thr, sfm_best* best,
                 sfm_poses* poses, int64_t cap, int64_t* num_inliers, int64_t* inlier_idx, uint8_t* pass, double* X,
                 uint8_t* mask, double* sed) {
    if (!best || !poses || !num_inliers) return fail(SFM_ERR_ARG, "null argument");
    if (int r = sfm_two_view_async(c, thr, min_extra, agg, mode, dist_thr, mask, sed)) return r;
    return sfm_two_view_fetch(c, best, poses, cap, num_inliers, inlier_idx, pass, X);
}

int sfm_score_async(sfm_ctx* c, double thr, double min_extra, int agg, int mode, void** record_dev) {
    if (int r = use(c)) return r;
    if (c->batched) return fail(SFM_ERR_STATE, "single-pair call on a batched context");
    if (int r = fit_launch(c, false)) return r;
    if (int r = score_launch(c, thr, min_extra, agg, mode, true, 0, c->n)) return r;
    if (record_dev) *record_dev = c->record.p;
    return 0;
}

int sfm_sharded_tail(sfm_ctx* c, const void* gathered_records_dev, int world, int rank, int64_t hyps_per_rank, int mode,
                     double thr, double dist_thr) {
    if (int r = use(c)) return r;
    if (!gathered_records_dev || world < 1 || rank < 0 || rank >= world) return fail(SFM_ERR_ARG, "bad gather arguments");
    if (!c->has_score) return fail(SFM_ERR_STATE, "sfm_score_async first");
    if (mode < 0 || mode > 2) return fail(SFM_ERR_ARG, "bad selection %d", mode);
    if (int r = c->winnerE.reserve(72)) return r;
    if (int r = c->merged.reserve(sizeof(SelectRecord) + sizeof(Best) + 16)) return r;
    SelectRecord* merged = c->merged.as<SelectRecord>();
    Best* local_best = reinterpret_cast<Best*>(merged + 1);
    int* owner = reinterpret_cast<int*>(local_best + 1);
    k_merge_records<<<1, 32, 0, c->stream>>>(reinterpret_cast<const SelectRecord*>(gathered_records_dev), world, rank,
                                             (long long)hyps_per_rank, mode, merged, owner, c->winnerE.as<double>(), local_best);
    if (int r = check_launch(c, "k_merge_records")) return r;
    return pose_tail_launch(c, thr, dist_thr, merged, c->n);
}

int sfm_sharded_fetch(sfm_ctx* c, sfm_best* best, int32_t* owner, sfm_poses* poses, int64_t cap, int64_t* num_inliers,
                      int64_t* inlier_idx, uint8_t* pass, double* X) {
    if (int r = use(c)) return r;
    if (!best || !owner || !poses || !num_inliers) return fail(SFM_ERR_ARG, "null argument");
    if (!c->merged.p) return fail(SFM_ERR_STATE, "sfm_sharded_tail first");
    const long long* cnt_dev = c->num.as<long long>();
    const size_t mbytes = sizeof(SelectRecord) + sizeof(Best) + 16;
    if (int r = ensure_pinned(c, 64 + mbytes)) return r;
    CU(cudaMemcpyAsync(c->hpin, cnt_dev, 8, cudaMemcpyDeviceToHost, c->stream));
    CU(cudaMemcpyAsync((char*)c->hpin + 64, c->merged.p, mbytes, cudaMemcpyDeviceToHost, c->stream));
    CU(cudaMemcpyAsync(poses, c->poses.p, sizeof(PoseSet), cudaMemcpyDeviceToHost, c->stream));
    CU(cudaStreamSynchronize(c->stream));
    long long m;
    memcpy(&m, c->hpin, 8);
    SelectRecord r;
    Best lb;
    int own;
    memcpy(&r, (char*)c->hpin + 64, sizeof r);
    memcpy(&lb, (char*)c->hpin + 64 + sizeof r, sizeof lb);
    memcpy(&own, (char*)c->hpin + 64 + sizeof r + sizeof lb, sizeof own);
    unpack_best(r, best);
    *owner = own;
    c->winner_local = lb.idx >= 0 ? lb.idx : -1;
    c->winner_set = r.best.idx >= 0;
    if (r.best.idx < 0) m = 0;
    *num_inliers = m;
    const long long take = m < cap ? m : cap;
    if (take > 0) return copy_inliers(c, take, inlier_idx, pass, X);
    return 0;
}

}

struct NcclId { char internal[128]; };
static_assert(sizeof(NcclId) == SFM_NCCL_ID_BYTES, "ncclUniqueId is 128 bytes");
namespace {
struct NcclApi {
    void* lib = nullptr;
    int (*GetUniqueId)(void*) = nullptr;
    int (*CommInitRank)(void**, int, NcclId, int) = nullptr;
    int (*AllGather)(const void*, void*, size_t, int, void*, cudaStream_t) = nullptr;
    int (*CommDestroy)(void*) = nullptr;
    const char* (*GetErrorString)(int) = nullptr;
};
NcclApi g_nccl;

int nccl_load() {
    if (g_nccl.lib) return 0;
    void* h = dlopen("libnccl.so.2", RTLD_NOW | RTLD_NOLOAD);
    if (!h) h = dlopen("libnccl.so.2", RTLD_NOW | RTLD_GLOBAL);
    if (!h) h = dlopen("libnccl.so", RTLD_NOW | RTLD_GLOBAL);
    if (!h) return fail(SFM_ERR_STATE, "libnccl.so.2 not found: %s", dlerror());
    g_nccl.GetUniqueId = reinterpret_cast<int (*)(void*)>(dlsym(h, "ncclGetUniqueId"));
    g_nccl.CommInitRank = reinterpret_cast<int (*)(void**, int, NcclId, int)>(dlsym(h, "ncclCommInitRank"));
    g_nccl.AllGather = reinterpret_cast<int (*)(const void*, void*, size_t, int, void*, cudaStream_t)>(dlsym(h, "ncclAllGather"));
    g_nccl.CommDestroy = reinterpret_cast<int (*)(void*)>(dlsym(h, "ncclCommDestroy"));
    g_nccl.GetErrorString = reinterpret_cast<const char* (*)(int)>(dlsym(h, "ncclGetErrorString"));
    if (!g_nccl.GetUniqueId || !g_nccl.CommInitRank || !g_nccl.AllGather || !g_nccl.CommDestroy)
        return fail(SFM_ERR_STATE, "libnccl.so.2 lacks a required symbol");
    g_nccl.lib = h;
    return 0;
}
#define NC(call)                                                                                          \
    do {                                                                                                  \
        int e_ = (call);                                                                                  \
        if (e_ != 0)                                                                                      \
            return fail(SFM_ERR_CUDA, "%s failed: %s", #call, g_nccl.GetErrorString ? g_nccl.GetErrorString(e_) : "?"); \
    } while (0)
}

extern "C" {

int sfm_nccl_unique_id(void* id_out) {
    if (!id_out) return fail(SFM_ERR_ARG, "null argument");
    if (int r = nccl_load()) return r;
    NC(g_nccl.GetUniqueId(id_out));
    return 0;
}

int sfm_nccl_init(sfm_ctx* c, int rank, int nranks, const void* unique_id) {
    if (int r = use(c)) return r;
    if (!unique_id || nranks < 1 || rank < 0 || rank >= nranks) return fail(SFM_ERR_ARG, "bad communicator arguments");
    if (int r = nccl_load()) return r;
    if (c->nccl_comm) { g_nccl.CommDestroy(c->nccl_comm); c->nccl_comm = nullptr; }
    NcclId id;
    memcpy(&id, unique_id, sizeof id);
    NC(g_nccl.CommInitRank(&c->nccl_comm, nranks, id, rank));
    c->nccl_rank = rank;
    c->nccl_world = nranks;
    return 0;
}

int sfm_nccl_destroy(sfm_ctx* c) {
    if (!c) return 0;
    if (c->nccl_comm && g_nccl.lib) {
        cudaSetDevice(c->device);
        cudaStreamSynchronize(c->stream);
        g_nccl.CommDestroy(c->nccl_comm);
    }
    c->nccl_comm = nullptr;
    c->nccl_world = 1;
    c->nccl_rank = 0;
    return 0;
}

int sfm_two_view_sharded(sfm_ctx* c, uint64_t seed, int64_t hyps_per_rank, double thr, double min_extra, int agg,
                         int mode, double dist_thr) {
    if (int r = use(c)) return r;
    if (!c->nccl_comm) return fail(SFM_ERR_STATE, "sfm_nccl_init first");
    if (c->batched) return fail(SFM_ERR_STATE, "single-pair call on a batched context");
    if (int r = sample_device(c, seed, 0, (int64_t)c->nccl_rank * hyps_per_rank, hyps_per_rank)) return r;
    if (int r = fit_launch(c, false)) return r;
    if (int r = score_launch(c, thr, min_extra, agg, mode, true, 0, c->n)) return r;
    if (int r = c->gathered.reserve((size_t)c->nccl_world * sizeof(SelectRecord))) return r;
    NC(g_nccl.AllGather(c->record.p, c->gathered.p, sizeof(SelectRecord),  1, c->nccl_comm, c->stream));
    return sfm_sharded_tail(c, c->gathered.p, c->nccl_world, c->nccl_rank, hyps_per_rank, mode, thr, dist_thr);
}

}

extern "C" {

static int batch_upload(sfm_ctx* c, const double* xa, const double* ya, const double* xb, const double* yb,
                        int64_t stride, const int64_t* offsets, int64_t npairs, const double* Ks, int64_t h, bool pixels,
                        long long* max_len_out) {
    if (!xa || !ya || !xb || !yb || !offsets || !Ks) return fail(SFM_ERR_ARG, "null argument");
    if (npairs <= 0 || npairs > 65535) return fail(SFM_ERR_ARG, "need 1 <= npairs <= 65535 per call");
    if (h <= 0) return fail(SFM_ERR_ARG, "need h > 0");
    const long long n = offsets[npairs];
    if (offsets[0] != 0 || n <= 0 || (uint64_t)n >= kMaxPoints) return fail(SFM_ERR_ARG, "bad offsets (total %lld)", n);
    long long max_len = 0;
    for (int64_t p = 0; p < npairs; ++p) {
        const long long len = offsets[p + 1] - offsets[p];
        if (len < 0) return fail(SFM_ERR_ARG, "offsets must be non-decreasing");
        if (len > max_len) max_len = len;
    }
    c->tic(T_UPLOAD);
    c->batched = true;
    c->npairs = npairs;
    c->n = n;
    c->first_len = offsets[1] - offsets[0];
    if (int r = c->offsets.reserve((size_t)(npairs + 1) * 8)) return r;
    if (int r = c->Ks.reserve((size_t)npairs * 72)) return r;
    CU(cudaMemcpyAsync(c->offsets.p, offsets, (size_t)(npairs + 1) * 8, cudaMemcpyHostToDevice, c->stream));
    CU(cudaMemcpyAsync(c->Ks.p, Ks, (size_t)npairs * 72, cudaMemcpyHostToDevice, c->stream));
    c->Kbatch.assign(Ks, Ks + 9 * npairs);
    c->batch_max_len = max_len;
    const double* s[4];
    if (int r = stage_raw(c, xa, ya, xb, yb, stride, n, s)) return r;
    if (pixels) {
        const double I[9] = {1, 0, 0, 0, 1, 0, 0, 0, 1};
        if (int r = hpose_stage_k(c, I)) return r;
        if (int r = c->pts.reserve((size_t)n * sizeof(Corr))) return r;
        k_normalise<<<dim3((unsigned)((n + 255) / 256), 1), 256, 0, c->stream>>>(s[0], s[1], s[2], s[3], stride, n, nullptr,
                                                                                c->hK.as<double>(), c->pts.as<Corr>(), nullptr);
        if (int r = check_launch(c, "k_normalise")) return r;
    } else if (int r = normalise_from(c, s[0], s[1], s[2], s[3], stride, n, max_len)) {
        return r;
    }
    c->toc(T_UPLOAD);
    c->has_pts = true;
    c->has_table = c->has_models = c->has_score = false;
    c->table_pending = false;
    c->winner_set = false;
    *max_len_out = max_len;
    return 0;
}

static int batch_core(sfm_ctx* c, const double* xa, const double* ya, const double* xb, const double* yb, int64_t stride,
                      const int64_t* offsets, int64_t npairs, const double* Ks, int64_t h, uint64_t seed, uint64_t pair_id0,
                      double thr, double min_extra, int agg, int mode, long long* max_len_out) {
    long long max_len = 0;
    if (int r = batch_upload(c, xa, ya, xb, yb, stride, offsets, npairs, Ks, h, false, &max_len)) return r;
    if (int r = sample_device(c, seed, pair_id0, 0, h)) return r;
    if (int r = fit_launch(c, false)) return r;
    if (int r = score_launch(c, thr, min_extra, agg, mode, true, 0, max_len)) return r;
    *max_len_out = max_len;
    return 0;
}

static int batch_fetch_winners(sfm_ctx* c, int64_t npairs, size_t extra_pinned, char** extra) {
    const size_t rbytes = (size_t)npairs * sizeof(SelectRecord);
    if (int r = ensure_pinned(c, rbytes + extra_pinned + 64)) return r;
    char* hp = (char*)c->hpin;
    CU(cudaMemcpyAsync(hp, c->record.p, rbytes, cudaMemcpyDeviceToHost, c->stream));
    if (extra) *extra = hp + ((rbytes + 63) / 64) * 64;
    return 0;
}

static void batch_unpack_winners(const char* hp, int64_t npairs, double* E, int64_t* best_index, double* best_err,
                                 int32_t* count_extra, int64_t* num_invalid) {
    const SelectRecord* hr = reinterpret_cast<const SelectRecord*>(hp);
    for (int64_t p = 0; p < npairs; ++p) {
        const bool ok = hr[p].best.idx >= 0;
        if (best_index) best_index[p] = hr[p].best.idx;
        if (best_err) best_err[p] = ok ? hr[p].best.err : __builtin_inf();
        if (count_extra) count_extra[p] = ok ? hr[p].best.count : -1;
        if (num_invalid) num_invalid[p] = hr[p].num_invalid;
        if (E) memcpy(E + 9 * p, hr[p].E, 72);
    }
}

int sfm_batch_ransac(sfm_ctx* c, const double* xa, const double* ya, const double* xb, const double* yb,
                     int64_t stride, const int64_t* offsets, int64_t npairs, const double* Ks, int64_t h,
                     uint64_t seed, uint64_t pair_id0, double thr, double min_extra, int agg, int mode, double* E,
                     int64_t* best_index, double* best_err, int32_t* count_extra, int64_t* num_invalid) {
    if (int r = use(c)) return r;
    long long max_len = 0;
    if (int r = batch_core(c, xa, ya, xb, yb, stride, offsets, npairs, Ks, h, seed, pair_id0, thr, min_extra, agg, mode,
                           &max_len)) return r;
    if (int r = batch_fetch_winners(c, npairs, 0, nullptr)) return r;
    CU(cudaStreamSynchronize(c->stream));
    batch_unpack_winners((const char*)c->hpin, npairs, E, best_index, best_err, count_extra, num_invalid);
    c->has_score = false;
    c->winner_set = false;
    return 0;
}

static int batch_tail_fetch(sfm_ctx* c, int64_t npairs, long long max_len, double* E, int64_t* best_index,
                            double* best_err, int32_t* count_extra, int64_t* num_invalid, PoseSet* poses, HPlane* planes,
                            int64_t* inlier_offsets, int64_t cap, int32_t* inlier_idx, uint8_t* pass, double* X) {
    const long long n = c->n;
    const size_t o_off = 0, o_idx = ((size_t)(npairs + 1) * 8 + 63) / 64 * 64, o_pass = o_idx + ((size_t)n * 4 + 63) / 64 * 64,
                 o_X = o_pass + ((size_t)n + 63) / 64 * 64;
    if (int r = c->bout.reserve(o_X + (size_t)n * 24)) return r;
    char* bo = c->bout.as<char>();
    long long* d_off = reinterpret_cast<long long*>(bo + o_off);
    k_batch_offsets<<<1, 1024, 0, c->stream>>>(c->num.as<long long>(), (int)npairs, d_off);
    if (int r = check_launch(c, "k_batch_offsets")) return r;
    const unsigned gx = (unsigned)((max_len + 255) / 256 > 0 ? (max_len + 255) / 256 : 1);
    k_batch_pack<<<dim3(gx, (unsigned)npairs), 256, 0, c->stream>>>(
        c->offsets.as<long long>(), c->num.as<long long>(), d_off, c->idx.as<long long>(), c->pass.as<uint8_t>(),
        c->X.as<double>(), reinterpret_cast<int32_t*>(bo + o_idx), reinterpret_cast<uint8_t*>(bo + o_pass),
        reinterpret_cast<double*>(bo + o_X));
    if (int r = check_launch(c, "k_batch_pack")) return r;
    char* extra = nullptr;
    const size_t pose_bytes = (size_t)npairs * sizeof(PoseSet);
    if (int r = batch_fetch_winners(c, npairs, pose_bytes, &extra)) return r;
    CU(cudaMemcpyAsync(poses, c->poses.p, pose_bytes, cudaMemcpyDeviceToHost, c->stream));
    if (planes)
        CU(cudaMemcpyAsync(planes, c->planes.p, (size_t)npairs * sizeof(HPlane), cudaMemcpyDeviceToHost, c->stream));
    CU(cudaMemcpyAsync(inlier_offsets, d_off, (size_t)(npairs + 1) * 8, cudaMemcpyDeviceToHost, c->stream));
    CU(cudaStreamSynchronize(c->stream));
    batch_unpack_winners((const char*)c->hpin, npairs, E, best_index, best_err, count_extra, num_invalid);
    const long long total = inlier_offsets[npairs];
    const long long take = total < cap ? total : cap;
    if (take > 0) {
        if (inlier_idx) CU(cudaMemcpyAsync(inlier_idx, bo + o_idx, (size_t)take * 4, cudaMemcpyDeviceToHost, c->stream));
        if (pass) CU(cudaMemcpyAsync(pass, bo + o_pass, (size_t)take, cudaMemcpyDeviceToHost, c->stream));
        if (X) CU(cudaMemcpyAsync(X, bo + o_X, (size_t)take * 24, cudaMemcpyDeviceToHost, c->stream));
        CU(cudaStreamSynchronize(c->stream));
    }
    c->has_score = false;
    c->winner_set = false;
    return 0;
}

int sfm_batch_two_view(sfm_ctx* c, const double* xa, const double* ya, const double* xb, const double* yb,
                       int64_t stride, const int64_t* offsets, int64_t npairs, const double* Ks, int64_t h,
                       uint64_t seed, uint64_t pair_id0, double thr, double min_extra, int agg, int mode,
                       double dist_thr, double* E, int64_t* best_index, double* best_err, int32_t* count_extra,
                       int64_t* num_invalid, sfm_poses* poses, int64_t* inlier_offsets, int64_t cap,
                       int32_t* inlier_idx, uint8_t* pass, double* X) {
    if (int r = use(c)) return r;
    if (!poses || !inlier_offsets) return fail(SFM_ERR_ARG, "null argument");
    long long max_len = 0;
    if (int r = batch_core(c, xa, ya, xb, yb, stride, offsets, npairs, Ks, h, seed, pair_id0, thr, min_extra, agg, mode,
                           &max_len)) return r;
    if (int r = pose_tail_launch(c, thr, dist_thr, c->record.as<SelectRecord>(), max_len)) return r;
    return batch_tail_fetch(c, npairs, max_len, E, best_index, best_err, count_extra, num_invalid,
                            reinterpret_cast<PoseSet*>(poses), nullptr, inlier_offsets, cap, inlier_idx, pass, X);
}

int sfm_batch_two_view_homography(sfm_ctx* c, const double* xa, const double* ya, const double* xb, const double* yb,
                                  int64_t stride, const int64_t* offsets, int64_t npairs, const double* Ks, int64_t h,
                                  uint64_t seed, uint64_t pair_id0, double thr, double min_extra, int agg, int mode,
                                  double dist_thr, double rotation_tolerance, double* H, int64_t* best_index,
                                  double* best_err, int32_t* count_extra, int64_t* num_invalid, sfm_hposes* poses,
                                  int64_t* inlier_offsets, int64_t cap, int32_t* inlier_idx, uint8_t* pass, double* X) {
    if (int r = use(c)) return r;
    if (!poses || !inlier_offsets || !Ks) return fail(SFM_ERR_ARG, "null argument");
    if (npairs <= 0 || npairs > 65535) return fail(SFM_ERR_ARG, "need 1 <= npairs <= 65535 per call");
    for (int64_t p = 0; p < npairs; ++p)
        if (int r = hpose_args(Ks + 9 * p, rotation_tolerance)) {
            const std::string why = g_err;
            return fail(r, "pair %lld: %s", (long long)p, why.c_str());
        }
    long long max_len = 0;
    if (int r = batch_upload(c, xa, ya, xb, yb, stride, offsets, npairs, Ks, h, true, &max_len)) return r;
    if (int r = sample_device(c, seed, pair_id0, 0, h)) return r;
    if (int r = fit_h_launch(c)) return r;
    if (int r = score_h_launch(c, thr, min_extra, agg, mode, max_len)) return r;
    if (int r = pose_tail_launch(c, thr, dist_thr, c->record.as<SelectRecord>(), max_len, nullptr, nullptr, MODEL_H,
                                 rotation_tolerance))
        return r;
    std::vector<PoseSet> ps((size_t)npairs);
    std::vector<HPlane> pl((size_t)npairs);
    if (int r = batch_tail_fetch(c, npairs, max_len, H, best_index, best_err, count_extra, num_invalid, ps.data(), pl.data(),
                                 inlier_offsets, cap, inlier_idx, pass, X))
        return r;
    for (int64_t p = 0; p < npairs; ++p) pack_hposes(ps[(size_t)p], pl[(size_t)p], poses + p);
    return 0;
}

static int match_finish(sfm_ctx* c, int64_t na, int64_t nb, int validation, double ratio_threshold, int32_t* best_b,
                        double* best_score, uint8_t* keep) {
    const size_t o_bs = ((size_t)na * 4 + 7) / 8 * 8, o_h1 = o_bs + (size_t)na * 8, o_keep = o_h1 + (size_t)na * 8;
    const size_t o_key = (o_keep + (size_t)na + 7) / 8 * 8, o_first = o_key + (size_t)nb * 8;
    if (int r = c->m_out.reserve(o_first + (size_t)nb * 4)) return r;
    char* out = c->m_out.as<char>();
    int32_t* d_bb = reinterpret_cast<int32_t*>(out);
    double* d_bs = reinterpret_cast<double*>(out + o_bs);
    double* d_h1 = reinterpret_cast<double*>(out + o_h1);
    uint8_t* d_keep = reinterpret_cast<uint8_t*>(out + o_keep);
    unsigned long long* d_key = reinterpret_cast<unsigned long long*>(out + o_key);
    int* d_first = reinterpret_cast<int*>(out + o_first);
    k_match_select<<<(unsigned)((na * 32 + 127) / 128), 128, 0, c->stream>>>(c->m_S.as<double>(), na, nb, validation,
                                                                            ratio_threshold, d_bb, d_bs, d_h1, d_keep);
    if (int r = check_launch(c, "k_match_select")) return r;
    if (validation & VALIDATE_CROSSCHECK) {
        CU(cudaMemsetAsync(d_key, 0xff, (size_t)nb * 8, c->stream));
        CU(cudaMemsetAsync(d_first, 0x7f, (size_t)nb * 4, c->stream));
        const unsigned gb = (unsigned)((na + 255) / 256);
        k_cross_min_score<<<gb, 256, 0, c->stream>>>(d_bb, d_bs, d_keep, na, d_key);
        if (int r = check_launch(c, "k_cross_min_score")) return r;
        k_cross_min_index<<<gb, 256, 0, c->stream>>>(d_bb, d_bs, d_keep, na, d_key, d_first);
        if (int r = check_launch(c, "k_cross_min_index")) return r;
        k_cross_filter<<<gb, 256, 0, c->stream>>>(d_bb, na, d_first, d_keep);
        if (int r = check_launch(c, "k_cross_filter")) return r;
    }
    CU(cudaMemcpyAsync(best_b, d_bb, (size_t)na * 4, cudaMemcpyDeviceToHost, c->stream));
    CU(cudaMemcpyAsync(best_score, d_bs, (size_t)na * 8, cudaMemcpyDeviceToHost, c->stream));
    CU(cudaMemcpyAsync(keep, d_keep, (size_t)na, cudaMemcpyDeviceToHost, c->stream));
    return 0;
}

static int match_check_counts(int64_t na, int64_t nb, const void* best_b, const void* best_score, const void* keep) {
    if (na < 0 || nb < 0) return fail(SFM_ERR_ARG, "negative feature count");
    if (na > 0 && nb == 0) return fail(SFM_ERR_ARG, "features_b is empty (the reference raises IndexError, matching.py:79)");
    if (nb > 0x7fffffffLL || na > 0x7fffffffLL) return fail(SFM_ERR_ARG, "too many features");
    if (na > 0 && (!best_b || !best_score || !keep)) return fail(SFM_ERR_ARG, "null output");
    return 0;
}

int sfm_match_brute_force(sfm_ctx* c, const void* image_a, const void* image_b, int image_dtype, int64_t rows,
                          int64_t cols, const double* feats_a, int64_t na, const double* feats_b, int64_t nb,
                          int score_kind, int window, int validation, double ratio_threshold, int32_t* best_b,
                          double* best_score, uint8_t* keep, double* scores) {
    if (int r = use(c)) return r;
    if (!image_a || !image_b || rows <= 0 || cols <= 0) return fail(SFM_ERR_ARG, "bad images");
    if (image_dtype != IMG_U8 && image_dtype != IMG_F64) return fail(SFM_ERR_ARG, "image dtype must be 0 (uint8) or 1 (float64)");
    if (score_kind != SCORE_NCC && score_kind != SCORE_SSD) return fail(SFM_ERR_ARG, "score kind must be 0 (ncc) or 1 (ssd)");
    if (window < 1 || window > kMaxWindow) return fail(SFM_ERR_ARG, "window size must be in [1, %d]", kMaxWindow);
    window = 2 * (window / 2) + 1;
    if (int r = match_check_counts(na, nb, best_b, best_score, keep)) return r;
    if ((na > 0 && !feats_a) || (nb > 0 && !feats_b)) return fail(SFM_ERR_ARG, "bad feature arrays");
    if (na == 0) return 0;
    const size_t px = (size_t)rows * cols, pxb = px * (image_dtype == IMG_U8 ? 1 : 8);
    const int ww = window * window;
    const size_t n = (size_t)(na + nb);
    const size_t img_b_off = (pxb + 15) / 16 * 16;
    if (int r = c->m_img.reserve(img_b_off + pxb)) return r;
    if (int r = c->m_feat.reserve(n * 16)) return r;
    if (int r = c->m_W.reserve(n * ww * 8)) return r;
    if (int r = c->m_ss.reserve(n * 8)) return r;
    if (int r = c->m_ok.reserve(n)) return r;
    if (int r = c->m_S.reserve((size_t)na * nb * 8)) return r;
    char* img = c->m_img.as<char>();
    CU(cudaMemcpyAsync(img, image_a, pxb, cudaMemcpyHostToDevice, c->stream));
    CU(cudaMemcpyAsync(img + img_b_off, image_b, pxb, cudaMemcpyHostToDevice, c->stream));
    double* feat = c->m_feat.as<double>();
    CU(cudaMemcpyAsync(feat, feats_a, (size_t)na * 16, cudaMemcpyHostToDevice, c->stream));
    CU(cudaMemcpyAsync(feat + 2 * na, feats_b, (size_t)nb * 16, cudaMemcpyHostToDevice, c->stream));
    double* W = c->m_W.as<double>();
    double* ss = c->m_ss.as<double>();
    uint8_t* ok = c->m_ok.as<uint8_t>();
    k_patch_prepare<<<(unsigned)((na + 127) / 128), 128, 0, c->stream>>>(img, image_dtype, rows, cols, feat, na, window,
                                                                        score_kind, W, ss, ok);
    if (int r = check_launch(c, "k_patch_prepare")) return r;
    k_patch_prepare<<<(unsigned)((nb + 127) / 128), 128, 0, c->stream>>>(img + img_b_off, image_dtype, rows, cols,
                                                                        feat + 2 * na, nb, window, score_kind,
                                                                        W + (size_t)na * ww, ss + na, ok + na);
    if (int r = check_launch(c, "k_patch_prepare")) return r;
    dim3 grid((unsigned)((nb + kScoreTile - 1) / kScoreTile), (unsigned)((na + kScoreTile - 1) / kScoreTile));
    k_patch_scores<<<grid, kScoreTile * kScoreTile, 0, c->stream>>>(W, ss, ok, na, W + (size_t)na * ww, ss + na, ok + na,
                                                                   nb, ww, score_kind, image_dtype, c->m_S.as<double>());
    if (int r = check_launch(c, "k_patch_scores")) return r;
    if (int r = match_finish(c, na, nb, validation, ratio_threshold, best_b, best_score, keep)) return r;
    if (scores) CU(cudaMemcpyAsync(scores, c->m_S.p, (size_t)na * nb * 8, cudaMemcpyDeviceToHost, c->stream));
    CU(cudaStreamSynchronize(c->stream));
    return 0;
}

int sfm_match_from_scores(sfm_ctx* c, const double* scores, int64_t na, int64_t nb, int validation,
                          double ratio_threshold, int32_t* best_b, double* best_score, uint8_t* keep) {
    if (int r = use(c)) return r;
    if (int r = match_check_counts(na, nb, best_b, best_score, keep)) return r;
    if (na == 0) return 0;
    if (!scores) return fail(SFM_ERR_ARG, "null score matrix");
    if (int r = c->m_S.reserve((size_t)na * nb * 8)) return r;
    CU(cudaMemcpyAsync(c->m_S.p, scores, (size_t)na * nb * 8, cudaMemcpyHostToDevice, c->stream));
    if (int r = match_finish(c, na, nb, validation, ratio_threshold, best_b, best_score, keep)) return r;
    CU(cudaStreamSynchronize(c->stream));
    return 0;
}

static int harris_check_image(const void* image, int image_dtype, int64_t rows, int64_t cols) {
    if (!image || rows <= 0 || cols <= 0) return fail(SFM_ERR_ARG, "bad image");
    if (image_dtype != IMG_U8 && image_dtype != IMG_F64) return fail(SFM_ERR_ARG, "image dtype must be 0 (uint8) or 1 (float64)");
    if (rows * cols > 0x7fffffffLL) return fail(SFM_ERR_ARG, "image too large");
    return 0;
}

int sfm_cross_correlate(sfm_ctx* c, const void* image, int image_dtype, int64_t rows, int64_t cols,
                        const double* kernel, int ksize, double* out) {
    if (int r = use(c)) return r;
    if (int r = harris_check_image(image, image_dtype, rows, cols)) return r;
    if (!kernel || !out) return fail(SFM_ERR_ARG, "null kernel or output");
    if (ksize < 1 || (ksize % 2) == 0) return fail(SFM_ERR_ARG, "only odd-sized square kernels are supported");
    if (rows < ksize || cols < ksize) return fail(SFM_ERR_ARG, "kernel cannot be larger than image");
    const size_t px = (size_t)rows * cols, pxb = px * (image_dtype == IMG_U8 ? 1 : 8);
    if (int r = c->h_img.reserve(pxb)) return r;
    if (int r = c->h_gx.reserve(px * 8)) return r;
    if (int r = c->h_small.reserve((size_t)ksize * ksize * 8 + 64)) return r;
    CU(cudaMemcpyAsync(c->h_img.p, image, pxb, cudaMemcpyHostToDevice, c->stream));
    CU(cudaMemcpyAsync(c->h_small.p, kernel, (size_t)ksize * ksize * 8, cudaMemcpyHostToDevice, c->stream));
    k_cross_correlate<<<(unsigned)((px + 255) / 256), 256, 0, c->stream>>>(c->h_img.p, image_dtype, (int)rows, (int)cols,
                                                                          c->h_small.as<double>(), ksize,
                                                                          c->h_gx.as<double>());
    if (int r = check_launch(c, "k_cross_correlate")) return r;
    CU(cudaMemcpyAsync(out, c->h_gx.p, px * 8, cudaMemcpyDeviceToHost, c->stream));
    CU(cudaStreamSynchronize(c->stream));
    return 0;
}

int sfm_harris_output_shape(int64_t rows, int64_t cols, int block_size, int64_t* out_rows, int64_t* out_cols) {
    if (block_size < 1 || !out_rows || !out_cols) return fail(SFM_ERR_ARG, "bad block size or null output");
    const int half = block_size / 2;
    const int shrink = (block_size % 2 == 0) ? half : ((half % 2 == 0) ? half : half + 1);
    *out_rows = rows - shrink;
    *out_cols = cols - shrink;
    return 0;
}

int sfm_harris_corners(sfm_ctx* c, const void* image, int image_dtype, int64_t rows, int64_t cols,
                       int64_t num_corners, int block_size, double k, double* xy, double* score, int64_t* num_found,
                       double* cornerness, int32_t* nms_sweeps) {
    if (int r = use(c)) return r;
    if (int r = harris_check_image(image, image_dtype, rows, cols)) return r;
    if (num_corners <= 0) return fail(SFM_ERR_ARG, "num_corners needs to be at least 1");
    if (block_size < 1 || block_size > 64) return fail(SFM_ERR_ARG, "block_size must be in [1, 64]");
    if (rows < 3 || cols < 3) return fail(SFM_ERR_ARG, "kernel cannot be larger than image");
    if (!xy || !score || !num_found) return fail(SFM_ERR_ARG, "null output");
    int64_t orows = 0, ocols = 0;
    sfm_harris_output_shape(rows, cols, block_size, &orows, &ocols);
    if (orows <= 0 || ocols <= 0) return fail(SFM_ERR_ARG, "block_size too large for this image");
    const size_t px = (size_t)rows * cols, pxb = px * (image_dtype == IMG_U8 ? 1 : 8);
    const size_t opx = (size_t)orows * ocols;
    size_t padded = kSortTile;
    while (padded < opx) padded <<= 1;
    if (int r = c->h_img.reserve(pxb)) return r;
    if (int r = c->h_gx.reserve(px * 8)) return r;
    if (int r = c->h_gy.reserve(px * 8)) return r;
    if (int r = c->h_corner.reserve(opx * 8)) return r;
    if (int r = c->h_alive.reserve(2 * opx)) return r;
    if (int r = c->h_small.reserve(64)) return r;
    const int64_t nout = num_corners < (int64_t)opx ? num_corners : (int64_t)opx;
    if (int r = c->h_xy.reserve((size_t)nout * 24)) return r;
    CU(cudaMemcpyAsync(c->h_img.p, image, pxb, cudaMemcpyHostToDevice, c->stream));
    const unsigned gpx = (unsigned)((px + 255) / 256), gopx = (unsigned)((opx + 255) / 256);
    k_sobel_pair<<<gpx, 256, 0, c->stream>>>(c->h_img.p, image_dtype, (int)rows, (int)cols, c->h_gx.as<double>(),
                                             c->h_gy.as<double>());
    if (int r = check_launch(c, "k_sobel_pair")) return r;
    double* corner = c->h_corner.as<double>();
    k_cornerness<<<gopx, 256, 0, c->stream>>>(c->h_gx.as<double>(), c->h_gy.as<double>(), (int)rows, (int)cols, block_size,
                                              k, (int)orows, (int)ocols, corner);
    if (int r = check_launch(c, "k_cornerness")) return r;
    uint8_t* alive[2] = {c->h_alive.as<uint8_t>(), c->h_alive.as<uint8_t>() + opx};
    int* d_changed = c->h_small.as<int>();
    unsigned* d_count = reinterpret_cast<unsigned*>(d_changed + 8);
    CU(cudaMemsetAsync(alive[0], 1, opx, c->stream));
    int cur = 0, sweeps = 0;
    for (;;) {
        CU(cudaMemsetAsync(d_changed, 0, 32, c->stream));
        for (int it = 0; it < 8; ++it) {
            k_nms_sweep<<<gopx, 256, 0, c->stream>>>(corner, (int)orows, (int)ocols, alive[cur], alive[cur ^ 1], d_changed + it);
            if (int r = check_launch(c, "k_nms_sweep")) return r;
            cur ^= 1;
        }
        sweeps += 8;
        int changed[8] = {0};
        CU(cudaMemcpyAsync(changed, d_changed, 32, cudaMemcpyDeviceToHost, c->stream));
        CU(cudaStreamSynchronize(c->stream));
        if (!changed[7]) break;
        if ((size_t)sweeps > opx + 16) return fail(SFM_ERR_CUDA, "non-maximum suppression did not converge");
    }
    k_nms_apply<<<gopx, 256, 0, c->stream>>>(corner, (long long)opx, alive[cur]);
    if (int r = check_launch(c, "k_nms_apply")) return r;
    CU(cudaMemsetAsync(d_count, 0, 4, c->stream));
    if (int r = c->h_key.reserve(padded * 8)) return r;
    if (int r = c->h_idx.reserve(padded * 4)) return r;
    unsigned long long* key = c->h_key.as<unsigned long long>();
    unsigned* idx = c->h_idx.as<unsigned>();
    k_corner_compact<<<gopx, 256, 0, c->stream>>>(corner, (long long)opx, key, idx, d_count);
    if (int r = check_launch(c, "k_corner_compact")) return r;
    unsigned count = 0;
    CU(cudaMemcpyAsync(&count, d_count, 4, cudaMemcpyDeviceToHost, c->stream));
    CU(cudaStreamSynchronize(c->stream));
    size_t n = kSortTile;
    while (n < count) n <<= 1;
    k_corner_pad<<<(unsigned)((n + 255) / 256), 256, 0, c->stream>>>(key, idx, d_count, (unsigned)n);
    if (int r = check_launch(c, "k_corner_pad")) return r;
    const unsigned tiles = (unsigned)(n / kSortTile);
    k_bitonic_local<<<tiles, kSortTile / 2, 0, c->stream>>>(key, idx, 0u, 0);
    if (int r = check_launch(c, "k_bitonic_local")) return r;
    for (size_t ks = 2 * (size_t)kSortTile; ks <= n; ks <<= 1) {
        for (size_t j = ks >> 1; j >= (size_t)kSortTile; j >>= 1) {
            k_bitonic_global<<<(unsigned)((n / 2 + 255) / 256), 256, 0, c->stream>>>(key, idx, (unsigned)n, (unsigned)ks, (unsigned)j);
            if (int r = check_launch(c, "k_bitonic_global")) return r;
        }
        k_bitonic_local<<<tiles, kSortTile / 2, 0, c->stream>>>(key, idx, (unsigned)ks, 1);
        if (int r = check_launch(c, "k_bitonic_local")) return r;
    }
    const int64_t found = (int64_t)count < num_corners ? (int64_t)count : num_corners;
    *num_found = found;
    if (found > 0) {
        double* d_xy = c->h_xy.as<double>();
        double* d_score = d_xy + 2 * nout;
        k_corner_emit<<<(unsigned)((found + 255) / 256), 256, 0, c->stream>>>(key, idx, d_count, found, (int)ocols,
                                                                             (double)block_size / 2.0, corner, d_xy, d_score);
        if (int r = check_launch(c, "k_corner_emit")) return r;
        CU(cudaMemcpyAsync(xy, d_xy, (size_t)found * 16, cudaMemcpyDeviceToHost, c->stream));
        CU(cudaMemcpyAsync(score, d_score, (size_t)found * 8, cudaMemcpyDeviceToHost, c->stream));
    }
    if (cornerness) CU(cudaMemcpyAsync(cornerness, corner, opx * 8, cudaMemcpyDeviceToHost, c->stream));
    CU(cudaStreamSynchronize(c->stream));
    if (nms_sweeps) *nms_sweeps = sweeps;
    return 0;
}

int sfm_enable_timing(sfm_ctx* c, int on) {
    if (!c) return fail(SFM_ERR_ARG, "null context");
    c->timing = on != 0;
    for (int i = 0; i < T_COUNT; ++i) c->ev_used[i] = false;
    return 0;
}

int sfm_get_timing(sfm_ctx* c, float ms[8], int64_t* launches) {
    if (int r = use(c)) return r;
    CU(cudaStreamSynchronize(c->stream));
    for (int i = 0; i < T_COUNT; ++i) {
        ms[i] = 0.f;
        if (c->timing && c->ev_used[i]) CU(cudaEventElapsedTime(&ms[i], c->ev0[i], c->ev1[i]));
        c->ev_used[i] = false;
    }
    if (launches) *launches = c->launches;
    return 0;
}

int sfm_measure_fp64_peak(sfm_ctx* c, double* dfma_per_s) {
    if (int r = use(c)) return r;
    if (!dfma_per_s) return fail(SFM_ERR_ARG, "null argument");
    if (int r = c->tmp.reserve(1 << 20)) return r;
    const int blocks = c->sm_count * 8, threads = 256, iters = 4096;
    cudaEvent_t a, b;
    CU(cudaEventCreate(&a));
    CU(cudaEventCreate(&b));
    double best = 0.0;
    for (int rep = 0; rep < 4; ++rep) {
        CU(cudaEventRecord(a, c->stream));
        k_fp64_peak<<<blocks, threads, 0, c->stream>>>(c->tmp.as<double>(), iters, 1.0000001);
        if (int r = check_launch(c, "k_fp64_peak")) return r;
        CU(cudaEventRecord(b, c->stream));
        CU(cudaEventSynchronize(b));
        float ms = 0.f;
        CU(cudaEventElapsedTime(&ms, a, b));
        const double rate = (double)blocks * threads * iters * 16.0 / (ms * 1e-3);
        if (rep > 0 && rate > best) best = rate;
    }
    cudaEventDestroy(a);
    cudaEventDestroy(b);
    *dfma_per_s = best;
    return 0;
}

}
```

### structure_from_motion_b200/csrc/sfm_device.cuh

```cuda
#pragma once
#include <cstdint>
#include <cuda_runtime.h>

namespace sfm {

#ifndef SFM_PDL
#define SFM_PDL 1
#endif
__device__ __forceinline__ void chain_enter() {
#if SFM_PDL
    asm volatile("griddepcontrol.wait;" ::: "memory");
    asm volatile("griddepcontrol.launch_dependents;");
#endif
}


constexpr double kVerySmall = 1e-10;
constexpr double kCheiralityTolerance = 1e-8;

struct __align__(32) Corr {
    double xa, ya, xb, yb;
};

struct __align__(32) ModelRow {
    double4 a, b, c;
};
static_assert(sizeof(ModelRow) == 96, "ModelRow must be three sectors");

__device__ __forceinline__ void store_model_row(ModelRow* rows, long long i, const double (&e)[9], bool ok) {
    ModelRow r;
    r.a = ok ? make_double4(e[0], e[1], e[2], e[3]) : make_double4(0.0, 0.0, 0.0, 0.0);
    r.b = ok ? make_double4(e[4], e[5], e[6], e[7]) : make_double4(0.0, 0.0, 0.0, 0.0);
    r.c = make_double4(ok ? e[8] : 0.0, 0.0, 0.0, 0.0);
    rows[i] = r;
}

__device__ __forceinline__ double sed_exact(const double (&e)[9], double xa, double ya, double xb,
                                            double yb) {
    const double lb0 = __dadd_rn(__fma_rn(yb, e[3], __dmul_rn(xb, e[0])), e[6]);
    const double lb1 = __dadd_rn(__fma_rn(yb, e[4], __dmul_rn(xb, e[1])), e[7]);
    const double lb2 = __dadd_rn(__fma_rn(yb, e[5], __dmul_rn(xb, e[2])), e[8]);
    const double la0 = __dadd_rn(__fma_rn(e[0], xa, __dmul_rn(e[1], ya)), e[2]);
    const double la1 = __dadd_rn(__fma_rn(e[3], xa, __dmul_rn(e[4], ya)), e[5]);
    const double r = __dadd_rn(__fma_rn(lb1, ya, __dmul_rn(lb0, xa)), lb2);
    const double na = __dadd_rn(__dmul_rn(la0, la0), __dmul_rn(la1, la1));
    const double nb = __dadd_rn(__dmul_rn(lb0, lb0), __dmul_rn(lb1, lb1));
    return __dmul_rn(__dadd_rn(__drcp_rn(na), __drcp_rn(nb)), __dmul_rn(r, r));
}

__device__ __forceinline__ double sed_screen(const double (&e)[9], double xa, double ya, double xb,
                                             double yb, double thr_pre) {
    const double lb0 = fma(xb, e[0], fma(yb, e[3], e[6]));
    const double lb1 = fma(xb, e[1], fma(yb, e[4], e[7]));
    const double lb2 = fma(xb, e[2], fma(yb, e[5], e[8]));
    const double r = fma(xa, lb0, fma(ya, lb1, lb2));
    const double nb = fma(lb0, lb0, lb1 * lb1);
    return fma(r, r, -(thr_pre * nb));
}

__device__ __forceinline__ double sed_full_decision(const double (&e)[9], double xa, double ya,
                                                    double xb, double yb, double thr_pre) {
    const double lb0 = fma(xb, e[0], fma(yb, e[3], e[6]));
    const double lb1 = fma(xb, e[1], fma(yb, e[4], e[7]));
    const double lb2 = fma(xb, e[2], fma(yb, e[5], e[8]));
    const double la0 = fma(e[0], xa, fma(e[1], ya, e[2]));
    const double la1 = fma(e[3], xa, fma(e[4], ya, e[5]));
    const double r = fma(xa, lb0, fma(ya, lb1, lb2));
    const double na = fma(la0, la0, la1 * la1);
    const double nb = fma(lb0, lb0, lb1 * lb1);
    const double t = thr_pre * (na * nb);
    return fma(r * r, na + nb, -t);
}

__device__ __forceinline__ void homography_adj(const double (&h)[9], double (&a)[9]) {
    a[0] = __fma_rn(h[4], h[8], -__dmul_rn(h[5], h[7]));
    a[1] = __fma_rn(h[2], h[7], -__dmul_rn(h[1], h[8]));
    a[2] = __fma_rn(h[1], h[5], -__dmul_rn(h[2], h[4]));
    a[3] = __fma_rn(h[5], h[6], -__dmul_rn(h[3], h[8]));
    a[4] = __fma_rn(h[0], h[8], -__dmul_rn(h[2], h[6]));
    a[5] = __fma_rn(h[2], h[3], -__dmul_rn(h[0], h[5]));
    a[6] = __fma_rn(h[3], h[7], -__dmul_rn(h[4], h[6]));
    a[7] = __fma_rn(h[1], h[6], -__dmul_rn(h[0], h[7]));
    a[8] = __fma_rn(h[0], h[4], -__dmul_rn(h[1], h[3]));
}

struct TransferTerms {
    double F, G, P, Q;
    bool finite_w;
};
__device__ __forceinline__ TransferTerms transfer_terms(const double (&h)[9], const double (&a)[9], double xa, double ya,
                                                        double xb, double yb) {
    const double p0 = __fma_rn(h[0], xa, __fma_rn(h[1], ya, h[2]));
    const double p1 = __fma_rn(h[3], xa, __fma_rn(h[4], ya, h[5]));
    const double p2 = __fma_rn(h[6], xa, __fma_rn(h[7], ya, h[8]));
    const double q0 = __fma_rn(a[0], xb, __fma_rn(a[1], yb, a[2]));
    const double q1 = __fma_rn(a[3], xb, __fma_rn(a[4], yb, a[5]));
    const double q2 = __fma_rn(a[6], xb, __fma_rn(a[7], yb, a[8]));
    const double u = __fma_rn(-xb, p2, p0), v = __fma_rn(-yb, p2, p1);
    const double s = __fma_rn(-xa, q2, q0), t = __fma_rn(-ya, q2, q1);
    TransferTerms r;
    r.F = __fma_rn(u, u, __dmul_rn(v, v));
    r.G = __fma_rn(s, s, __dmul_rn(t, t));
    r.P = __dmul_rn(p2, p2);
    r.Q = __dmul_rn(q2, q2);
    r.finite_w = ((__double_as_longlong(p2) << 1) != 0) && ((__double_as_longlong(q2) << 1) != 0);
    return r;
}
__device__ __forceinline__ bool transfer_inlier(const TransferTerms& r, double thr) {
    return r.finite_w && (__fma_rn(r.F, r.Q, __dmul_rn(r.G, r.P)) <= __dmul_rn(__dmul_rn(thr, r.P), r.Q));
}
__device__ __forceinline__ double transfer_value(const TransferTerms& r) {
    return __dadd_rn(__ddiv_rn(r.F, r.P), __ddiv_rn(r.G, r.Q));
}
__device__ __forceinline__ bool transfer_exact(const double (&h)[9], const double (&a)[9], double xa, double ya, double xb,
                                               double yb, double thr, double& value) {
    const TransferTerms r = transfer_terms(h, a, xa, ya, xb, yb);
    value = transfer_value(r);
    return transfer_inlier(r, thr);
}

__host__ __device__ __forceinline__ void philox4x32_10(uint32_t c0, uint32_t c1, uint32_t c2,
                                                       uint32_t c3, uint32_t k0, uint32_t k1,
                                                       uint32_t (&out)[4]) {
    const uint32_t M0 = 0xD2511F53u, M1 = 0xCD9E8D57u, W0 = 0x9E3779B9u, W1 = 0xBB67AE85u;
#pragma unroll
    for (int r = 0; r < 10; ++r) {
        const uint64_t p0 = (uint64_t)M0 * c0, p1 = (uint64_t)M1 * c2;
        const uint32_t n0 = (uint32_t)(p1 >> 32) ^ c1 ^ k0;
        const uint32_t n1 = (uint32_t)p1;
        const uint32_t n2 = (uint32_t)(p0 >> 32) ^ c3 ^ k1;
        const uint32_t n3 = (uint32_t)p0;
        c0 = n0; c1 = n1; c2 = n2; c3 = n3;
        k0 += W0; k1 += W1;
    }
    out[0] = c0; out[1] = c1; out[2] = c2; out[3] = c3;
}

__host__ __device__ inline void philox_sample8(uint64_t seed, uint64_t stream, uint64_t hyp,
                                               uint32_t n, int32_t (&idx)[8]) {
    uint32_t draw = 0;
    int got = 0;
    while (got < 8) {
        uint32_t o[4];
        philox4x32_10((uint32_t)hyp, (uint32_t)(hyp >> 32), draw++, (uint32_t)stream,
                      (uint32_t)seed, (uint32_t)(seed >> 32) ^ (uint32_t)(stream >> 32), o);
#pragma unroll
        for (int w = 0; w < 2 && got < 8; ++w) {
            const uint64_t r64 = ((uint64_t)o[2 * w] << 32) | o[2 * w + 1];
#if defined(__CUDA_ARCH__)
            const uint32_t cand = (uint32_t)__umul64hi(r64, (uint64_t)n);
#else
            const uint32_t cand = (uint32_t)(((unsigned __int128)r64 * n) >> 64);
#endif
            bool dup = false;
            for (int j = 0; j < got; ++j) dup |= (idx[j] == (int32_t)cand);
            if (!dup) idx[got++] = (int32_t)cand;
        }
    }
}

}
```

### structure_from_motion_b200/csrc/sfm_score.cuh

```cuda
#pragma once
#include <type_traits>

#include "sfm_device.cuh"

namespace sfm {

__device__ __forceinline__ uint32_t smem_u32(const void* p) {
    return (uint32_t)__cvta_generic_to_shared(p);
}
__device__ __forceinline__ void mbar_init(void* bar, uint32_t count) {
    asm volatile("mbarrier.init.shared::cta.b64 [%0], %1;" ::"r"(smem_u32(bar)), "r"(count) : "memory");
}
__device__ __forceinline__ void mbar_fence_init() {
    asm volatile("fence.mbarrier_init.release.cluster;" ::: "memory");
}
__device__ __forceinline__ void mbar_expect_tx(void* bar, uint32_t bytes) {
    asm volatile("mbarrier.arrive.expect_tx.shared::cta.b64 _, [%0], %1;" ::"r"(smem_u32(bar)), "r"(bytes)
                 : "memory");
}
__device__ __forceinline__ void mbar_wait(void* bar, uint32_t parity) {
    uint32_t ok;
    do {
        asm volatile(
            "{\n\t.reg .pred p;\n\t"
            "mbarrier.try_wait.parity.shared::cta.b64 p, [%1], %2;\n\t"
            "selp.u32 %0, 1, 0, p;\n\t}"
            : "=r"(ok)
            : "r"(smem_u32(bar)), "r"(parity)
            : "memory");
    } while (!ok);
}
__device__ __forceinline__ void bulk_g2s(void* dst_smem, const void* src_gmem, uint32_t bytes, void* bar) {
    asm volatile(
        "cp.async.bulk.shared::cluster.global.mbarrier::complete_tx::bytes [%0], [%1], %2, [%3];" ::"r"(
            smem_u32(dst_smem)),
        "l"(src_gmem), "r"(bytes), "r"(smem_u32(bar))
        : "memory");
}

constexpr int kScoreThreads = 128;
constexpr int kScoreWarps = kScoreThreads / 32;
#ifndef SFM_SCORE_TILE
#define SFM_SCORE_TILE 64
#endif
#ifndef SFM_SCORE_STAGES
#define SFM_SCORE_STAGES 3
#endif
constexpr int kTile = SFM_SCORE_TILE;
constexpr int kStages = SFM_SCORE_STAGES;
constexpr int kRing = 64;
constexpr unsigned kMaxPoints = 1u << 25;
constexpr int kChunks = 4;
constexpr int kFixedBits = 21 * kChunks;
constexpr int kChunkBits = 21;
constexpr int kAccWords = 1 + 2 * kChunks;
constexpr long long kMaxItemPoints = 1ll << 11;
enum { SUM_S1 = 1, SUM_S2 = 2 };
enum { MODE_FULL = 0, MODE_SCREEN = 1, MODE_SCREEN32 = 2 };
constexpr double kKappaCoef = 4e-20;
constexpr double kKappa32Coef = 1.2e-10;
constexpr double kThr32Factor = 1.0316;

__global__ void __launch_bounds__(256) k_pad_models(const double* __restrict__ E, long long htotal, ModelRow* __restrict__ rows) {
    const long long i = blockIdx.x * (long long)blockDim.x + threadIdx.x;
    if (i >= htotal) return;
    const double* e = E + 9 * i;
    ModelRow r;
    r.a = make_double4(e[0], e[1], e[2], e[3]);
    r.b = make_double4(e[4], e[5], e[6], e[7]);
    r.c = make_double4(e[8], 0.0, 0.0, 0.0);
    rows[i] = r;
}

struct ScoreArgs {
    const Corr* pts;
    const void* spts;
    const double* bounds;
    long long n;
    const long long* offsets;
    const double* E;
    const ModelRow* rows;
    long long h;
    double thr, thr_pre, s;
    double kappa_coef;
    double kappa32_coef;
    double scale1, scale2;
    int sums;
    long long chunk;
    int hblocks, nsplit;
    long long total_items;
    long long htotal;
    unsigned* work_counter;
    unsigned long long* acc;
    const int* mode_flag;
};

__device__ __forceinline__ unsigned atom_add_acq_rel_shared(unsigned* p, unsigned v) {
    unsigned old;
    asm volatile("atom.acq_rel.cta.shared::cta.add.u32 %0, [%1], %2;" : "=r"(old) : "r"(smem_u32(p)), "r"(v) : "memory");
    return old;
}
__device__ __forceinline__ int scan_step(int v, int d) {
    asm volatile("{ .reg .pred p; .reg .b32 t; shfl.sync.up.b32 t|p, %0, %1, 0, 0xffffffff; @p add.s32 %0, %0, t; }"
                 : "+r"(v) : "r"(d));
    return v;
}
__device__ __forceinline__ unsigned lanemask_lt() {
    unsigned m;
    asm("mov.u32 %0, %%lanemask_lt;" : "=r"(m));
    return m;
}

__device__ __forceinline__ void chunks21(double x, double scale, unsigned (&c)[kChunks]) {
    const double t = x * scale;
    const unsigned long long v = __double2ull_rz(t);
    const double rem = t - __ull2double_rz(v);
    c[0] = (unsigned)__double2uint_rz(rem * 2097152.0);
    c[1] = (unsigned)v & 0x1fffffu;
    c[2] = (unsigned)(v >> kChunkBits) & 0x1fffffu;
    c[3] = (unsigned)(v >> (2 * kChunkBits));
}

struct __align__(16) Corr32 {
    float xa, ya, xb, yb;
};

constexpr int kPilotBlocks = 32;
constexpr int kPilotHyps = 64;
constexpr int kPilotPts = 1024;
constexpr double kPilotFullAbove = 0.09;
struct PilotArgs {
    const double* E;
    long long h;
    long long plen;
    double thr_pre;
    unsigned* counters;
    int* mode_flag;
};
__global__ void __launch_bounds__(256) k_screen_pts64(const Corr* __restrict__ pts, long long n, double inv_s,
                                                      Corr* __restrict__ spts, const PilotArgs pa) {
    chain_enter();
    const long long i = blockIdx.x * (long long)blockDim.x + threadIdx.x;
    if (i < n) {
        Corr c = pts[i];
        c.xa *= inv_s;
        c.ya *= inv_s;
        spts[i] = c;
    }
    if (!pa.mode_flag || blockIdx.x >= kPilotBlocks) return;
    const int nb = gridDim.x < kPilotBlocks ? gridDim.x : kPilotBlocks;
    const long long nh = pa.h < kPilotHyps ? pa.h : kPilotHyps;
    const int hs = threadIdx.x % kPilotHyps;
    int pass = 0, tests = 0;
    if (hs < nh && pa.plen > 0) {
        const long long hyp = (pa.h / nh) * hs;
        double e[9];
#pragma unroll
        for (int k = 0; k < 9; ++k) e[k] = pa.E[9 * hyp + k];
        const long long np = pa.plen < kPilotPts ? pa.plen : kPilotPts;
        const long long step = pa.plen / np;
        const int lanes = nb * (256 / kPilotHyps);
        Corr cs[8];
        int got = 0;
#pragma unroll
        for (int u = 0; u < 8; ++u) {
            const long long q = blockIdx.x * (256 / kPilotHyps) + threadIdx.x / kPilotHyps + (long long)u * lanes;
            if (q < np) { cs[u] = pts[q * step]; got = u + 1; }
        }
#pragma unroll
        for (int u = 0; u < 8; ++u)
            if (u < got) {
                pass += sed_screen(e, cs[u].xa, cs[u].ya, cs[u].xb, cs[u].yb, pa.thr_pre) < 0.0 ? 1 : 0;
                tests += 1;
            }
    }
    unsigned long long v = ((unsigned long long)pass << 32) | (unsigned)tests;
#pragma unroll
    for (int d = 16; d > 0; d >>= 1) v += __shfl_xor_sync(0xffffffffu, v, d);
    __shared__ unsigned long long s_sum;
    __shared__ int s_last;
    if (threadIdx.x == 0) s_sum = 0ull;
    __syncthreads();
    if ((threadIdx.x & 31) == 0) atomicAdd(&s_sum, v);
    __syncthreads();
    if (threadIdx.x == 0) {
        unsigned long long* tot = reinterpret_cast<unsigned long long*>(pa.counters);
        atomicAdd(tot, s_sum);
        __threadfence();
        s_last = atomicAdd(pa.counters + 2, 1u) == (unsigned)(nb - 1);
        if (s_last) {
            __threadfence();
            const unsigned long long t = *reinterpret_cast<volatile unsigned long long*>(tot);
            const double rate = (unsigned)t ? (double)(t >> 32) / (double)(unsigned)t : 0.0;
            *pa.mode_flag = rate > kPilotFullAbove ? MODE_FULL : MODE_SCREEN;
        }
    }
}

__global__ void __launch_bounds__(256) k_screen_pts32(const Corr* __restrict__ pts, long long n, double inv_s,
                                                      Corr32* __restrict__ spts) {
    const long long i = blockIdx.x * (long long)blockDim.x + threadIdx.x;
    if (i >= n) return;
    const Corr c = pts[i];
    Corr32 f;
    f.xa = (float)(c.xa * inv_s); f.ya = (float)(c.ya * inv_s); f.xb = (float)c.xb; f.yb = (float)c.yb;
    spts[i] = f;
}

template <int HPT>
struct alignas(128) ScoreWarpSmem {
    Corr tile[kStages][kTile];
    unsigned sacc[HPT][kAccWords][32];
    uint2 ring[kRing];
    unsigned short own[32];
    unsigned long long full_bar[kStages];
};

constexpr int kTileFS = 32;
constexpr int kStagesFS = 3;
template <int HPT>
struct alignas(128) ScoreWarpSmemFS {
    Corr tile[kStagesFS][kTileFS];
    double model[32 * HPT][10];
    unsigned sacc[HPT][kAccWords][32];
    uint2 ring[kRing];
    unsigned long long full_bar[kStagesFS];
};
__host__ __device__ constexpr bool score_full_in_smem(int hpt) { return hpt <= 2; }
template <int HPT, int MODE>
constexpr size_t score_warp_bytes() {
    return (MODE == MODE_FULL && score_full_in_smem(HPT)) ? sizeof(ScoreWarpSmemFS<HPT>) : sizeof(ScoreWarpSmem<HPT>);
}

#ifndef SFM_SCORE_MINB4
#define SFM_SCORE_MINB4 4
#endif
#ifndef SFM_SCORE_MINB2
#define SFM_SCORE_MINB2 5
#endif
constexpr int score_min_blocks(int hpt) { return hpt >= 4 ? SFM_SCORE_MINB4 : (hpt == 2 ? SFM_SCORE_MINB2 : 8); }


__device__ __forceinline__ int sign_word(double d) { return __double2hiint(d); }
__device__ __forceinline__ int sign_word(float f) { return __float_as_int(f); }

template <int HPT, int G, int MODE>
__device__ __forceinline__ void score_body(const ScoreArgs& a) {
    constexpr bool SCREEN = MODE != MODE_FULL;
    constexpr bool F32 = MODE == MODE_SCREEN32;
    using T = typename std::conditional<F32, float, double>::type;
    using P = typename std::conditional<F32, Corr32, Corr>::type;
    constexpr int NB = HPT * G;
    constexpr bool FS = MODE == MODE_FULL && score_full_in_smem(HPT);
    constexpr bool ENTRY = MODE == MODE_FULL;
    constexpr int TILE = FS ? kTileFS : kTile;
    constexpr int STAGES = FS ? kStagesFS : kStages;
    constexpr int AHEAD = FS ? STAGES - 1 : STAGES;
    using WS = typename std::conditional<FS, ScoreWarpSmemFS<HPT>, ScoreWarpSmem<HPT>>::type;
    static_assert(NB <= 32 && (TILE % G) == 0 && (kTile % TILE) == 0, "a batch is at most 32 tests and divides a tile");
    extern __shared__ __align__(128) unsigned char score_smem[];
    const unsigned full = 0xffffffffu;
    const int lane = threadIdx.x & 31;
    const int warp = __shfl_sync(full, (int)(threadIdx.x >> 5), 0);
    const unsigned lt = lanemask_lt();
    if (a.mode_flag && *a.mode_flag != MODE) return;
    WS& ws = reinterpret_cast<WS*>(score_smem)[warp];

    if (lane == 0) {
#pragma unroll
        for (int s = 0; s < STAGES; ++s) mbar_init(&ws.full_bar[s], 1);
        mbar_fence_init();
    }
#pragma unroll
    for (int j = 0; j < HPT; ++j)
#pragma unroll
        for (int k = 0; k < kAccWords; ++k) ws.sacc[j][k][lane] = 0;
    __syncwarp();
    uint2* q = ws.ring;
    unsigned head = 0, tail = 0;
    unsigned gt = 0;
    const double ab2 = SCREEN ? a.bounds[0] * a.bounds[1] * (F32 ? a.kappa32_coef : a.kappa_coef) : 0.0;

    for (;;) {
        unsigned item = 0;
        if (lane == 0) item = atomicAdd(a.work_counter, 1u);
        item = __shfl_sync(full, item, 0);
        if (item >= a.total_items) break;
        const int hw = (int)(item % (unsigned)a.hblocks);
        const unsigned rest = item / (unsigned)a.hblocks;
        const int split = (int)(rest % (unsigned)a.nsplit);
        const int pair = (int)(rest / (unsigned)a.nsplit);

        const long long pbase = a.offsets ? a.offsets[pair] : 0;
        const long long plen = a.offsets ? a.offsets[pair + 1] - pbase : a.n;
        long long begin = (long long)split * a.chunk;
        if (begin > plen) begin = plen;
        const long long end = pbase + ((begin + a.chunk < plen) ? begin + a.chunk : plen);
        begin += pbase;
        const int ntiles = (int)((end - begin + TILE - 1) / TILE);
        const long long hyp_w = (long long)hw * (32 * HPT);
        const double* Ep = a.E + 9 * (long long)pair * a.h;
        const ModelRow* Rw = a.rows + (long long)pair * a.h + hyp_w;
        const Corr* pbeg = a.pts + begin;
        const P* src = reinterpret_cast<const P*>(SCREEN ? a.spts : (const void*)a.pts);

        auto issue = [&](int t) {
            const int s = (int)((gt + (unsigned)t) % STAGES);
            const long long first = begin + (long long)t * TILE;
            const long long rem = end - first;
            const uint32_t bytes = (uint32_t)((rem < TILE ? rem : TILE) * sizeof(P));
            mbar_expect_tx(&ws.full_bar[s], bytes);
            bulk_g2s(&ws.tile[s][0], src + first, bytes, &ws.full_bar[s]);
        };
        if (lane == 0) {
            for (int t = 0; t < AHEAD && t < ntiles; ++t) issue(t);
        }

        T e[HPT][9], kap[HPT];
#pragma unroll
        for (int j = 0; j < HPT; ++j) {
            const long long hyp = hyp_w + 32 * j + lane;
            const bool real = hyp < a.h;
            double v[9], f2 = 0.0;
#pragma unroll
            for (int k = 0; k < 9; ++k) {
                v[k] = real ? Ep[9 * hyp + k] : 0.0;
                f2 = fma(v[k], v[k], f2);
            }
            if constexpr (FS) {
                double2* mp = reinterpret_cast<double2*>(&ws.model[32 * j + lane][0]);
                mp[0] = make_double2(v[0], v[1]);
                mp[1] = make_double2(v[2], v[3]);
                mp[2] = make_double2(v[4], v[5]);
                mp[3] = make_double2(v[6], v[7]);
                ws.model[32 * j + lane][8] = v[8];
            }
            const double nrm = F32 ? rsqrt(f2) : 1.0;
#pragma unroll
            for (int k = 0; k < 9; ++k) e[j][k] = (T)((SCREEN && (k % 3) != 2) ? v[k] * nrm * a.s : v[k] * nrm);
            if (F32) kap[j] = (T)(real ? ((f2 > 0.0 && f2 < 1e300) ? ab2 : __longlong_as_double(0x7ff0000000000000LL)) : -1.0);
            else kap[j] = (T)(real ? f2 * ab2 : -1.0);
        }

        auto accumulate = [&](bool act, double sv, int slot, int owner) {
            if (act && (sv <= a.thr)) {
                unsigned ch[kChunks];
                unsigned* dst = &ws.sacc[slot][0][FS ? (owner ^ (slot << 4)) : owner];
                atomicAdd(dst, 1u);
                if (a.sums & SUM_S1) {
                    chunks21(sv, a.scale1, ch);
#pragma unroll
                    for (int kk = 0; kk < kChunks; ++kk) atomicAdd(dst + 32 * (1 + kk), ch[kk]);
                }
                if (a.sums & SUM_S2) {
                    chunks21(__dmul_rn(sv, sv), a.scale2, ch);
#pragma unroll
                    for (int kk = 0; kk < kChunks; ++kk) atomicAdd(dst + 32 * (1 + kChunks + kk), ch[kk]);
                }
            }
        };
        auto survivor_sed = [&](unsigned hl, unsigned pos) -> double {
            double eo[9];
            Corr c;
            if constexpr (FS) {
                const double2* mp = reinterpret_cast<const double2*>(&ws.model[hl][0]);
                const double2 m0 = mp[0], m1 = mp[1], m2 = mp[2], m3 = mp[3];
                eo[0] = m0.x; eo[1] = m0.y; eo[2] = m1.x; eo[3] = m1.y;
                eo[4] = m2.x; eo[5] = m2.y; eo[6] = m3.x; eo[7] = m3.y;
                eo[8] = ws.model[hl][8];
                c = (&ws.tile[0][0])[pos];
            } else {
                const ModelRow* er = Rw + hl;
                const double4 r0 = er->a, r1 = er->b;
                eo[0] = r0.x; eo[1] = r0.y; eo[2] = r0.z; eo[3] = r0.w;
                eo[4] = r1.x; eo[5] = r1.y; eo[6] = r1.z; eo[7] = r1.w;
                eo[8] = er->c.x;
                c = pbeg[pos];
            }
            return sed_exact(eo, c.xa, c.ya, c.xb, c.yb);
        };

        unsigned* qe = reinterpret_cast<unsigned*>(ws.ring);
        constexpr int LH = HPT >= 8 ? 3 : (HPT == 4 ? 2 : (HPT == 2 ? 1 : 0));
        const unsigned ln = (unsigned)__popc(lt);
        auto drain_entries = [&]() {
            const unsigned navail = tail - head;
            const bool act = ln < navail;
            const unsigned en = act ? qe[(head + ln) & (kRing - 1)] : 0u;
            const int owner = (int)((en >> 14) & 31u), slot = LH ? (int)(en >> (32 - (LH ? LH : 1))) : 0;
            accumulate(act, survivor_sed((unsigned)(32 * slot + owner), en & 0x7ffu), slot, owner);
            head += navail < 32u ? navail : 32u;
            __syncwarp();
        };
        auto push_entries = [&](unsigned pm, unsigned pos0) {
            const unsigned base = (ln << 14) | pos0;
            unsigned vote;
            while ((vote = __ballot_sync(full, pm != 0u)) != 0u) {
                const unsigned top = 0x80000000u >> __clz(pm | 1u);
                const unsigned i = (unsigned)(NB - 32) + (unsigned)__clz(pm | 1u);
                const unsigned en = base + __funnelshift_r(i, i, LH);
                if (pm) qe[(tail + __popc(vote & lt)) & (kRing - 1)] = en;
                pm &= ~top;
                tail += __popc(vote);
                __syncwarp();
                if (tail - head >= 32u) drain_entries();
            }
        };

        auto drain_records = [&]() {
            const unsigned nrec = tail - head;
            uint2 rec = make_uint2(0u, 0u);
            if ((unsigned)lane < nrec) rec = q[(head + lane) & (kRing - 1)];
            const int cnt = __popc(rec.x);
            int incl = cnt;
#pragma unroll
            for (int d = 1; d < 32; d <<= 1) incl = scan_step(incl, d);
            const int total = __shfl_sync(full, incl, 31);
            const int m = total < 32 ? total : 32;
            const int excl = incl - cnt;
            const unsigned done_mask = __ballot_sync(full, (unsigned)lane < nrec && incl <= 32);
            const int ndone = __popc(done_mask);
            const bool act = lane < m;
            unsigned o = 0u;
            uint2 rj = make_uint2(0u, 0u);
            if constexpr (!ENTRY) {
                unsigned pmw = rec.x;
                for (int t = excl; pmw && t < 32; ++t) {
                    ws.own[t] = (unsigned short)(lane | ((__ffs(pmw) - 1) << 8));
                    pmw &= pmw - 1u;
                }
                __syncwarp();
                o = act ? ws.own[lane] : 0u;
                rj = q[(head + (o & 255u)) & (kRing - 1)];
                __syncwarp();
                if (lane == ndone && (unsigned)lane < nrec) q[(head + lane) & (kRing - 1)].x = pmw;
            }
            const int i = NB - 1 - (int)(o >> 8);
            const int owner = (int)(rj.y >> 27), slot = i % HPT;
            const unsigned rel = act ? (rj.y & 0x3fffffu) + (unsigned)(i / HPT) : 0u;
            accumulate(act, survivor_sed(act ? (unsigned)(32 * slot + owner) : 0u, rel), slot, owner);
            head += (unsigned)ndone;
            __syncwarp();
        };
        auto push_records = [&](unsigned vote, unsigned pm, unsigned rel0) {
            if (pm) q[(tail + __popc(vote & lt)) & (kRing - 1)] = make_uint2(pm, ((unsigned)lane << 27) | rel0);
            tail += __popc(vote);
            __syncwarp();
            while (tail - head >= 32u) drain_records();
        };
        auto drain = [&]() {
            if constexpr (ENTRY) drain_entries();
            else drain_records();
        };

        unsigned mark = tail;
        for (int t = 0; t < ntiles; ++t) {
            const unsigned gti = gt + (unsigned)t;
            const int s = (int)(gti % STAGES);
            mbar_wait(&ws.full_bar[s], (gti / STAGES) & 1u);
            const long long first = begin + (long long)t * TILE;
            const int np = (int)((end - first < TILE) ? (end - first) : TILE);
            const P* tp = reinterpret_cast<const P*>(&ws.tile[s][0]);
            for (int p = 0; p < np; p += G) {
                unsigned pm = 0;
#pragma unroll
                for (int g = 0; g < G; ++g) {
                    const P c = tp[p + g];
                    T d[HPT];
                    if (SCREEN) {
                        T t0[HPT], t1[HPT], t2[HPT];
#pragma unroll
                        for (int j = 0; j < HPT; ++j) {
                            t0[j] = fma(c.yb, e[j][3], e[j][6]);
                            t1[j] = fma(c.yb, e[j][4], e[j][7]);
                            t2[j] = fma(c.yb, e[j][5], e[j][8]);
                        }
#pragma unroll
                        for (int j = 0; j < HPT; ++j) {
                            t0[j] = fma(c.xb, e[j][0], t0[j]);
                            t1[j] = fma(c.xb, e[j][1], t1[j]);
                            t2[j] = fma(c.xb, e[j][2], t2[j]);
                        }
#pragma unroll
                        for (int j = 0; j < HPT; ++j) t2[j] = fma(c.ya, t1[j], t2[j]);
#pragma unroll
                        for (int j = 0; j < HPT; ++j) t2[j] = fma(c.xa, t0[j], t2[j]);
#pragma unroll
                        for (int j = 0; j < HPT; ++j) t1[j] = fma(t1[j], t1[j], kap[j]);
#pragma unroll
                        for (int j = 0; j < HPT; ++j) t1[j] = fma(t0[j], t0[j], t1[j]);
#pragma unroll
                        for (int j = 0; j < HPT; ++j) d[j] = fma(t2[j], t2[j], -t1[j]);
                    } else if constexpr (!SCREEN) {
#pragma unroll
                        for (int j = 0; j < HPT; ++j) d[j] = sed_full_decision(e[j], c.xa, c.ya, c.xb, c.yb, a.thr_pre);
                    }
#pragma unroll
                    for (int j = 0; j < HPT; ++j) pm = __funnelshift_l((unsigned)sign_word(d[j]), pm, 1);
                }
                const int v = np - p;
                if (v < G) pm &= 0xffffffffu << (NB - v * HPT);
                const unsigned vote = __ballot_sync(full, pm != 0u);
                if (vote) {
                    if constexpr (ENTRY) push_entries(pm, FS ? (unsigned)(s * TILE + p) : (unsigned)(first - begin) + (unsigned)p);
                    else push_records(vote, pm, (unsigned)(first - begin) + (unsigned)p);
                }
            }
            if constexpr (FS) {
                while ((int)(mark - head) > 0) drain();
                mark = tail;
            }
            __syncwarp();
            if (lane == 0 && t + AHEAD < ntiles) issue(t + AHEAD);
        }
        gt += (unsigned)ntiles;

        while (tail != head) drain();
#pragma unroll
        for (int j = 0; j < HPT; ++j) {
            const long long hyp = hyp_w + 32 * j + lane;
            const int col = FS ? (lane ^ ((j & 1) << 4)) : lane;
            const unsigned cnt = ws.sacc[j][0][col];
            if (cnt) {
                unsigned long long* dst = a.acc + (long long)pair * a.h + hyp;
                atomicAdd(dst, (unsigned long long)cnt);
                ws.sacc[j][0][col] = 0;
#pragma unroll
                for (int k = 1; k < kAccWords; ++k) {
                    const unsigned v = ws.sacc[j][k][col];
                    if (v) {
                        atomicAdd(dst + (long long)k * a.htotal, (unsigned long long)v);
                        ws.sacc[j][k][col] = 0;
                    }
                }
            }
        }
        __syncwarp();
    }
}

template <int HPT, int G, int MODE>
__global__ void __launch_bounds__(kScoreThreads, score_min_blocks(MODE == MODE_SCREEN32 ? HPT / 2 : HPT))
k_score(const ScoreArgs a) {
    chain_enter();
    score_body<HPT, G, MODE>(a);
}

template <int HPT, int G>
__global__ void __launch_bounds__(kScoreThreads, score_min_blocks(HPT)) k_score_auto(const ScoreArgs a, const ScoreArgs a_full) {
    chain_enter();
    if (*a.mode_flag == MODE_FULL) score_body<HPT, G, MODE_FULL>(a_full);
    else score_body<HPT, G, MODE_SCREEN>(a);
}

enum { AGG_SUM = 0, AGG_SQUARE = 1, AGG_MEAN = 2, AGG_RMS = 3 };
enum { SELECT_MIN_ERROR = 0, SELECT_MAX_INLIERS = 1, SELECT_MSAC = 2 };

struct Best {
    double err;
    long long idx;
    int count;
    int pad;
};

struct SelectRecord {
    Best best;
    long long num_invalid, first_invalid;
    double E[9];
    int32_t sample[8];
};

__device__ __forceinline__ bool better(const Best& x, const Best& y, int mode) {
    if (y.idx < 0) return x.idx >= 0;
    if (x.idx < 0) return false;
    if (mode == SELECT_MAX_INLIERS) {
        if (x.count != y.count) return x.count > y.count;
        return x.idx < y.idx;
    }
    if (x.err != y.err) return x.err < y.err;
    return x.idx < y.idx;
}

__device__ __forceinline__ Best shfl_best(const Best& b, int src_delta) {
    Best r;
    r.err = __shfl_down_sync(0xffffffffu, b.err, src_delta);
    r.idx = __shfl_down_sync(0xffffffffu, b.idx, src_delta);
    r.count = __shfl_down_sync(0xffffffffu, b.count, src_delta);
    r.pad = 0;
    return r;
}

__device__ __forceinline__ Best block_best(Best b, int mode, Best* sm ) {
    const int lane = threadIdx.x & 31, warp = threadIdx.x >> 5;
#pragma unroll
    for (int d = 16; d > 0; d >>= 1) {
        const Best o = shfl_best(b, d);
        if (better(o, b, mode)) b = o;
    }
    if (lane == 0) sm[warp] = b;
    __syncthreads();
    if (warp == 0) {
        const int nw = (blockDim.x + 31) >> 5;
        Best x;
        if (lane < nw) x = sm[lane];
        else { x.err = 0.0; x.idx = -1; x.count = 0; x.pad = 0; }
#pragma unroll
        for (int d = 16; d > 0; d >>= 1) {
            const Best o = shfl_best(x, d);
            if (better(o, x, mode)) x = o;
        }
        b = x;
    }
    return b;
}

struct dd { double hi, lo; };
__device__ __forceinline__ void dd_add(dd& s, double x) {
    const double t = __dadd_rn(s.hi, x);
    const double bb = __dsub_rn(t, s.hi);
    const double e = __dadd_rn(__dsub_rn(s.hi, __dsub_rn(t, bb)), __dsub_rn(x, bb));
    s.hi = t;
    s.lo = __dadd_rn(s.lo, e);
}
__device__ __forceinline__ void dd_merge(dd& s, const dd& o) {
    dd_add(s, o.hi);
    s.lo = __dadd_rn(s.lo, o.lo);
    const double t = __dadd_rn(s.hi, s.lo);
    s.lo = __dsub_rn(s.lo, __dsub_rn(t, s.hi));
    s.hi = t;
}

__device__ __forceinline__ unsigned __int128 fixed_value(const unsigned long long* acc, long long stride) {
    unsigned __int128 v = 0;
#pragma unroll
    for (int k = kChunks - 1; k >= 0; --k) v = (v << kChunkBits) + acc[(long long)k * stride];
    return v;
}
__device__ __forceinline__ double u128_to_double(unsigned __int128 v) {
    const unsigned long long hi = (unsigned long long)(v >> 64), lo = (unsigned long long)v;
    return fma((double)hi, 18446744073709551616.0, (double)lo);
}

struct FinalArgs {
    const Corr* pts;
    const long long* offsets;
    const double* E;
    const uint8_t* valid;
    const int32_t* table;
    long long h;
    long long n;
    long long idx_offset;
    long long htotal;
    const unsigned long long* acc;
    double inv_scale1, inv_scale2;
    int sums;
    int force_rescore;
    double thr, min_extra;
    int agg, mode;
    int32_t* count_extra;
    double* S1;
    double* S2;
    double* err;
    Best* block_out;
    long long* block_inv;
    unsigned* tickets;
    Best* out;
    long long* invalid_out;
    SelectRecord* record;
    unsigned long long* rescored;
    unsigned* fitflag;
};

enum { MODEL_E = 0, MODEL_H = 1 };
template <int KIND> struct ExactModel;
template <> struct ExactModel<MODEL_E> {
    static constexpr int kSample = 8;
    double e[9];
    __device__ __forceinline__ void load(const double* m) {
#pragma unroll
        for (int k = 0; k < 9; ++k) e[k] = m[k];
    }
    __device__ __forceinline__ bool eval(const Corr& c, double thr, double& v) const {
        v = sed_exact(e, c.xa, c.ya, c.xb, c.yb);
        return v <= thr;
    }
};
template <> struct ExactModel<MODEL_H> {
    static constexpr int kSample = 4;
    double h[9], adj[9];
    __device__ __forceinline__ void load(const double* m) {
#pragma unroll
        for (int k = 0; k < 9; ++k) h[k] = m[k];
        homography_adj(h, adj);
    }
    __device__ __forceinline__ bool eval(const Corr& c, double thr, double& v) const {
        return transfer_exact(h, adj, c.xa, c.ya, c.xb, c.yb, thr, v);
    }
};

template <int KIND>
__device__ __forceinline__ bool finalise_one(const FinalArgs& a, const Corr* pts, long long i, long long npts, bool valid,
                                             long long cnt, double s1, double s2, double& err_out, long long& cnt_out,
                                             double& s1_out, double& s2_out) {
    constexpr int KS = ExactModel<KIND>::kSample;
    const double msac = __dadd_rn(s1, __dmul_rn(a.thr, (double)(npts - cnt)));
    if (a.table && valid) {
        ExactModel<KIND> m;
        m.load(a.E + 9 * i);
        for (int k = 0; k < KS; ++k) {
            const Corr c = pts[a.table[8 * i + k]];
            double sv;
            if (m.eval(c, a.thr, sv)) {
                cnt -= 1;
            } else {
                s1 = __dadd_rn(s1, sv);
                s2 = __dadd_rn(s2, __dmul_rn(sv, sv));
            }
        }
    }
    const double n = (double)((a.table ? KS : 0) + cnt);
    double err;
    switch (a.agg) {
        case AGG_SUM: err = s1; break;
        case AGG_SQUARE: err = s2; break;
        case AGG_MEAN: err = s1 / n; break;
        default: err = sqrt(s2 / n); break;
    }
    if (a.mode == SELECT_MSAC) err = msac;
    err_out = err; cnt_out = cnt; s1_out = s1; s2_out = s2;
    return valid && (a.min_extra <= (double)cnt) && (err == err);
}

template <int KIND>
__global__ void __launch_bounds__(256) k_finalise(const FinalArgs a) {
    chain_enter();
    __shared__ Best sm[32];
    __shared__ int s_list[256];
    __shared__ int s_nlist;
    __shared__ dd s_dd[2][8];
    __shared__ long long s_cnt[8];
    __shared__ long long s_first;
    __shared__ int s_last;
    const int tid = threadIdx.x, lane = tid & 31, warp = tid >> 5;
    const long long li = blockIdx.x * (long long)blockDim.x + tid;
    const long long i = (long long)blockIdx.y * a.h + li;
    const Corr* pts = a.pts + (a.offsets ? a.offsets[blockIdx.y] : 0);
    const long long npts = a.offsets ? a.offsets[blockIdx.y + 1] - a.offsets[blockIdx.y] : a.n;
    const double qnan = __longlong_as_double(0x7ff8000000000000LL);
    const double pinf = __longlong_as_double(0x7ff0000000000000LL);
    if (tid == 0) { s_nlist = 0; s_first = 0x7fffffffffffffffLL; }
    __syncthreads();
    Best b;
    b.err = 0.0; b.idx = -1; b.count = 0; b.pad = 0;
    if (li < a.h) {
        const bool valid = a.valid ? (a.valid[i] != 0) : true;
        const long long cnt = (long long)a.acc[i];
        const unsigned __int128 v1 = (a.sums & SUM_S1) ? fixed_value(a.acc + 1 * a.htotal + i, a.htotal) : 0;
        const unsigned __int128 v2 = (a.sums & SUM_S2) ? fixed_value(a.acc + (1 + kChunks) * a.htotal + i, a.htotal) : 0;
        const unsigned __int128 need = (unsigned __int128)(unsigned long long)cnt << 53;
        bool coarse = cnt > 0 && (((a.sums & SUM_S1) && v1 < need) || ((a.sums & SUM_S2) && v2 < need));
        if constexpr (KIND == MODEL_H) coarse = coarse && !((double)cnt < a.min_extra);
        if (valid && (a.force_rescore || coarse)) {
            s_list[atomicAdd(&s_nlist, 1)] = tid;
        } else {
            const double s1 = (a.sums & SUM_S1) ? u128_to_double(v1) * a.inv_scale1 : qnan;
            const double s2 = (a.sums & SUM_S2) ? u128_to_double(v2) * a.inv_scale2 : qnan;
            double err, s1o, s2o;
            long long c2;
            const bool cand = finalise_one<KIND>(a, pts, i, npts, valid, cnt, s1, s2, err, c2, s1o, s2o);
            a.count_extra[i] = valid ? (int32_t)c2 : -1;
            a.S1[i] = s1o;
            a.S2[i] = s2o;
            a.err[i] = cand ? err : pinf;
            if (cand) { b.err = err; b.idx = a.idx_offset + li; b.count = (int)c2; }
        }
    }
    __syncthreads();
    const int nlist = s_nlist;
    for (int q = 0; q < nlist; ++q) {
        const int owner = s_list[q];
        const long long hi_ = (long long)blockIdx.y * a.h + blockIdx.x * (long long)blockDim.x + owner;
        ExactModel<KIND> m;
        m.load(a.E + 9 * hi_);
        dd p1{0.0, 0.0}, p2{0.0, 0.0};
        long long pc = 0;
        for (long long j = tid; j < npts; j += 256) {
            const Corr c = pts[j];
            double sv;
            if (m.eval(c, a.thr, sv)) {
                pc += 1;
                dd_add(p1, sv);
                dd_add(p2, __dmul_rn(sv, sv));
            }
        }
#pragma unroll
        for (int d = 16; d > 0; d >>= 1) {
            dd o1, o2;
            o1.hi = __shfl_xor_sync(0xffffffffu, p1.hi, d); o1.lo = __shfl_xor_sync(0xffffffffu, p1.lo, d);
            o2.hi = __shfl_xor_sync(0xffffffffu, p2.hi, d); o2.lo = __shfl_xor_sync(0xffffffffu, p2.lo, d);
            pc += __shfl_xor_sync(0xffffffffu, pc, d);
            if (lane & d) { dd t1 = o1, t2 = o2; dd_merge(t1, p1); dd_merge(t2, p2); p1 = t1; p2 = t2; }
            else { dd_merge(p1, o1); dd_merge(p2, o2); }
        }
        if (lane == 0) { s_dd[0][warp] = p1; s_dd[1][warp] = p2; s_cnt[warp] = pc; }
        __syncthreads();
        if (tid == owner) {
            dd t1 = s_dd[0][0], t2 = s_dd[1][0];
            long long c = s_cnt[0];
            for (int w = 1; w < 8; ++w) { dd_merge(t1, s_dd[0][w]); dd_merge(t2, s_dd[1][w]); c += s_cnt[w]; }
            double err, s1o, s2o;
            long long c2;
            const bool cand = finalise_one<KIND>(a, pts, hi_, npts, true, c, (a.sums & SUM_S1) ? t1.hi : qnan,
                                           (a.sums & SUM_S2) ? t2.hi : qnan, err, c2, s1o, s2o);
            a.count_extra[hi_] = (int32_t)c2;
            a.S1[hi_] = s1o;
            a.S2[hi_] = s2o;
            a.err[hi_] = cand ? err : pinf;
            if (cand) { b.err = err; b.idx = a.idx_offset + (hi_ - (long long)blockIdx.y * a.h); b.count = (int)c2; }
        }
        __syncthreads();
    }
    if (tid == 0 && nlist) atomicAdd(a.rescored, (unsigned long long)nlist);
    const bool inv = (li < a.h) && a.valid && (a.valid[i] == 0);
    const int ninv = __syncthreads_count(inv);
    if (inv) atomicMin(&s_first, a.idx_offset + li);
    b = block_best(b, a.mode, sm);
    __syncthreads();
    const int nblocks = gridDim.x;
    if (tid == 0) {
        const long long blk = (long long)blockIdx.y * nblocks + blockIdx.x;
        a.block_out[blk] = b;
        a.block_inv[2 * blk] = ninv;
        a.block_inv[2 * blk + 1] = s_first;
        __threadfence();
        s_last = (atomicAdd(&a.tickets[blockIdx.y], 1u) == (unsigned)(nblocks - 1)) ? 1 : 0;
    }
    __syncthreads();
    if (!s_last) return;
    __threadfence();
    __shared__ long long s_ninv, s_first2;
    if (tid == 0) {
        s_ninv = 0; s_first2 = 0x7fffffffffffffffLL; a.tickets[blockIdx.y] = 0;
        if (a.fitflag && blockIdx.y == 0) *a.fitflag = 0u;
    }
    __syncthreads();
    const volatile Best* blocks = a.block_out + (long long)blockIdx.y * nblocks;
    const volatile long long* binv = a.block_inv + 2 * (long long)blockIdx.y * nblocks;
    Best g;
    g.err = 0.0; g.idx = -1; g.count = 0; g.pad = 0;
    long long tn = 0, tf = 0x7fffffffffffffffLL;
    for (int k = tid; k < nblocks; k += 256) {
        Best o;
        o.err = blocks[k].err; o.idx = blocks[k].idx; o.count = blocks[k].count; o.pad = 0;
        if (better(o, g, a.mode)) g = o;
        tn += binv[2 * k];
        const long long f = binv[2 * k + 1];
        if (f < tf) tf = f;
    }
    if (tn) {
        atomicAdd((unsigned long long*)&s_ninv, (unsigned long long)tn);
        atomicMin(&s_first2, tf);
    }
    g = block_best(g, a.mode, sm);
    __syncthreads();
    if (tid == 0) {
        a.out[blockIdx.y] = g;
        a.invalid_out[2 * blockIdx.y] = s_ninv;
        a.invalid_out[2 * blockIdx.y + 1] = s_ninv ? s_first2 : -1;
        SelectRecord& r = a.record[blockIdx.y];
        r.best = g;
        r.num_invalid = s_ninv;
        r.first_invalid = s_ninv ? s_first2 : -1;
        const long long w = (long long)blockIdx.y * a.h + (g.idx >= 0 ? g.idx - a.idx_offset : 0);
        for (int k = 0; k < 9; ++k) r.E[k] = g.idx >= 0 ? a.E[9 * w + k] : 0.0;
        for (int k = 0; k < 8; ++k)
            r.sample[k] = (a.table && g.idx >= 0 && k < ExactModel<KIND>::kSample) ? a.table[8 * w + k] : -1;
    }
}

__global__ void __launch_bounds__(256) k_near_ties(const double* __restrict__ err, long long h, const SelectRecord* __restrict__ rec,
                                                   double rel_tol, int cap, long long* __restrict__ out, unsigned* __restrict__ count) {
    const double best = rec->best.err;
    if (rec->best.idx < 0) return;
    const double lim = best + fabs(best) * rel_tol;
    for (long long i = blockIdx.x * (long long)blockDim.x + threadIdx.x; i < h; i += (long long)gridDim.x * blockDim.x) {
        if (err[i] <= lim) {
            const unsigned pos = atomicAdd(count, 1u);
            if (pos < (unsigned)cap) out[pos] = i;
        }
    }
}

__global__ void k_merge_records(const SelectRecord* __restrict__ gathered, int world, int rank, long long hyps_per_rank,
                                int mode, SelectRecord* __restrict__ merged, int* __restrict__ owner_out,
                                double* __restrict__ winner_E, Best* __restrict__ local_best) {
    if (threadIdx.x || blockIdx.x) return;
    Best b;
    b.err = 0.0; b.idx = -1; b.count = 0; b.pad = 0;
    int owner = -1;
    for (int r = 0; r < world; ++r) {
        Best o = gathered[r].best;
        if (o.idx >= 0) o.idx += (long long)r * hyps_per_rank;
        if (better(o, b, mode)) { b = o; owner = r; }
    }
    merged->best = b;
    merged->num_invalid = gathered[rank].num_invalid;
    merged->first_invalid = gathered[rank].first_invalid;
    for (int k = 0; k < 9; ++k) {
        const double v = owner >= 0 ? gathered[owner].E[k] : 0.0;
        merged->E[k] = v;
        winner_E[k] = v;
    }
    for (int k = 0; k < 8; ++k) merged->sample[k] = owner >= 0 ? gathered[owner].sample[k] : -1;
    *owner_out = owner;
    Best lb = b;
    lb.idx = (owner == rank) ? gathered[rank].best.idx : -1;
    *local_best = lb;
}

__global__ void k_inlier_mask(const Corr* __restrict__ pts, long long n, const double* __restrict__ E,
                              const Best* __restrict__ best, long long idx_offset, long long hyp,
                              double thr, uint8_t* __restrict__ mask, double* __restrict__ sed) {
    const long long i = blockIdx.x * (long long)blockDim.x + threadIdx.x;
    if (i >= n) return;
    long long local = hyp;
    if (best) local = best->idx - idx_offset;
    if (local < 0) {
        mask[i] = 0;
        sed[i] = __longlong_as_double(0x7ff8000000000000LL);
        return;
    }
    double e[9];
#pragma unroll
    for (int k = 0; k < 9; ++k) e[k] = E[9 * local + k];
    const Corr c = pts[i];
    const double sv = sed_exact(e, c.xa, c.ya, c.xb, c.yb);
    sed[i] = sv;
    mask[i] = (sv <= thr) ? 1 : 0;
}

}
```

Baseline: 1030 billion.

## Sort points spatially and use per-tile bounding-box thresholds in fp64 screening

For large unbatched inputs, points are radix-sorted by a spatial key after normalisation and gathered into tiles, each with a bounding box. The fp64 screen kernel then computes one conservative per-tile threshold per hypothesis from the box, instead of a per-point epipolar-line norm. This removes two FMAs per point-hypothesis test in the inner loop and also drops the separate scaled-point copy. In exchange it adds a sort and gather at normalise time, extra shared memory per warp, and a looser screen that may send more candidates to the exact check.

After: 1109 billion, median of 6. +7.7%, better.

```diff
diff --git a/structure_from_motion_b200/csrc/sfm_api.cu b/structure_from_motion_b200/csrc/sfm_api.cu
--- a/structure_from_motion_b200/csrc/sfm_api.cu
+++ b/structure_from_motion_b200/csrc/sfm_api.cu
@@ -9,6 +9,8 @@
 #include <cstring>
 #include <string>
 #include <vector>
+
+#include <cub/device/device_radix_sort.cuh>
 
 #include "sfm_device.cuh"
 #include "sfm_fit.cuh"
@@ -97,6 +99,7 @@
     Buf h_img, h_gx, h_gy, h_corner, h_alive, h_key, h_idx, h_small, h_xy;
     Buf mask, sed, poses, pass, X, idx, scan, tmp, tailstate, num, winrec, bout;
     Buf planes, hK;
+    Buf k2pts, k2box, k2sort;
     Buf selstate, selio, selpp;
     long long n = 0, h = 0, npairs = 1;
     long long first_len = 0;
@@ -104,6 +107,7 @@
     long long raw_stride = 1;
     bool batched = false, has_pts = false, has_table = false, has_models = false, has_score = false;
     bool models_h = false;
+    bool k2_ready = false;
     int hscore_occ = 0;
     bool table_pending = false;
     unsigned long long smp_seed = 0, smp_stream = 0;
@@ -205,24 +209,29 @@
     return cudaLaunchKernelExC(&cfg, fn, kargs);
 }
 
-size_t score_warp_smem(int hpt, bool full) {
+template <int HPT>
+size_t score_warp_smem_h(bool full, bool tiles) {
+    return full ? score_warp_bytes<HPT, MODE_FULL>() : tiles ? score_warp_bytes<HPT, MODE_SCREEN>() : sizeof(ScoreWarpSmem<HPT>);
+}
+size_t score_warp_smem(int hpt, bool full, bool tiles) {
     switch (hpt) {
-        case 1: return full ? score_warp_bytes<1, MODE_FULL>() : sizeof(ScoreWarpSmem<1>);
-        case 2: return full ? score_warp_bytes<2, MODE_FULL>() : sizeof(ScoreWarpSmem<2>);
-        case 4: return full ? score_warp_bytes<4, MODE_FULL>() : sizeof(ScoreWarpSmem<4>);
+        case 1: return score_warp_smem_h<1>(full, tiles);
+        case 2: return score_warp_smem_h<2>(full, tiles);
+        case 4: return score_warp_smem_h<4>(full, tiles);
         default: return sizeof(ScoreWarpSmem<8>);
     }
 }
 
-const void* score_kernel(int variant, int hpt, int group) {
+const void* score_kernel(int variant, int hpt, int group, bool tiles) {
     if (variant == SFM_SCORE_SCREEN32) {
 #define SFM_K32(H, G) if (hpt == H && group == G) return reinterpret_cast<const void*>(&k_score<H, G, MODE_SCREEN32>)
         SFM_K32(2, 16); SFM_K32(4, 8); SFM_K32(8, 4);
 #undef SFM_K32
         return nullptr;
     }
-#define SFM_K(H, G) if (hpt == H && group == G) return scr ? reinterpret_cast<const void*>(&k_score<H, G, MODE_SCREEN>) \
-                                                           : reinterpret_cast<const void*>(&k_score<H, G, MODE_FULL>)
+#define SFM_K(H, G) if (hpt == H && group == G) return !scr ? reinterpret_cast<const void*>(&k_score<H, G, MODE_FULL>) \
+                                                    : tiles ? reinterpret_cast<const void*>(&k_score<H, G, MODE_SCREEN>) \
+                                                            : reinterpret_cast<const void*>(&k_score<H, G, MODE_SCREEN11>)
     const bool scr = variant == SFM_SCORE_SCREEN;
     SFM_K(1, 16); SFM_K(1, 32);
     SFM_K(2, 4); SFM_K(2, 8); SFM_K(2, 16);
@@ -287,7 +296,7 @@
     Buf* bufs[] = {&c->raw, &c->pts, &c->offsets, &c->Ks, &c->table, &c->E, &c->valid, &c->eig, &c->acc,
                    &c->count_extra, &c->S1, &c->S2, &c->err, &c->blocks, &c->best,
                    &c->invalid, &c->winnerE, &c->record, &c->merged, &c->rows, &c->blockinv, &c->mask, &c->sed, &c->poses, &c->pass, &c->X, &c->idx,
-                   &c->planes, &c->hK, &c->selstate, &c->selio, &c->selpp,
+                   &c->planes, &c->hK, &c->selstate, &c->selio, &c->selpp, &c->k2pts, &c->k2box, &c->k2sort,
                    &c->scan, &c->tmp, &c->gathered, &c->tailstate, &c->num, &c->winrec, &c->bout, &c->spts, &c->bounds, &c->fitflag,
                    &c->m_img, &c->m_feat, &c->m_W, &c->m_ss, &c->m_ok, &c->m_S, &c->m_out,
                    &c->h_img, &c->h_gx, &c->h_gy, &c->h_corner, &c->h_alive, &c->h_key, &c->h_idx, &c->h_small, &c->h_xy};
@@ -330,8 +339,8 @@
         nh = variant == SFM_SCORE_SCREEN32 ? 4 : 2;
         ng = variant == SFM_SCORE_SCREEN32 ? 8 : 16;
     }
-    if (!score_kernel(variant == SFM_SCORE_AUTO ? SFM_SCORE_SCREEN : variant, nh, ng) ||
-        (variant == SFM_SCORE_AUTO && !score_kernel(SFM_SCORE_FULL, nh, ng)))
+    if (!score_kernel(variant == SFM_SCORE_AUTO ? SFM_SCORE_SCREEN : variant, nh, ng, true) ||
+        (variant == SFM_SCORE_AUTO && !score_kernel(SFM_SCORE_FULL, nh, ng, true)))
         return fail(SFM_ERR_ARG, "unsupported combination: hyps_per_thread %d, group %d", nh, ng);
     c->variant = variant;
     c->hpt = nh;
@@ -410,6 +419,40 @@
     return 0;
 }
 
+#ifndef SFM_K2_SORT_MIN
+#define SFM_K2_SORT_MIN 65536
+#endif
+constexpr long long kK2SortMin = SFM_K2_SORT_MIN;
+static int k2_order(sfm_ctx* c, long long n) {
+    size_t cub_bytes = 0;
+    CU(cub::DeviceRadixSort::SortPairs(nullptr, cub_bytes, (const unsigned*)nullptr, (unsigned*)nullptr, (const int*)nullptr,
+                                       (int*)nullptr, (int)n, 0, 32, c->stream));
+    const size_t vb = ((size_t)n * 4 + 255) & ~(size_t)255;
+    if (int r = c->k2sort.reserve(4 * vb + 256 + cub_bytes)) return r;
+    char* w = c->k2sort.as<char>();
+    auto* keys = reinterpret_cast<unsigned*>(w);
+    auto* keys2 = reinterpret_cast<unsigned*>(w + vb);
+    int* idx = reinterpret_cast<int*>(w + 2 * vb);
+    int* idx2 = reinterpret_cast<int*>(w + 3 * vb);
+    auto* bb = reinterpret_cast<unsigned long long*>(w + 4 * vb);
+    void* tmp = w + 4 * vb + 256;
+    const long long tiles = (n + kTile - 1) / kTile;
+    if (int r = c->k2pts.reserve((size_t)n * sizeof(Corr))) return r;
+    if (int r = c->k2box.reserve((size_t)tiles * sizeof(double4))) return r;
+    CU(cudaMemsetAsync(bb, 0, 32, c->stream));
+    const unsigned grid = (unsigned)((n + 255) / 256);
+    k2_order_bbox<<<grid, 256, 0, c->stream>>>(c->pts.as<Corr>(), n, bb);
+    if (int r = check_launch(c, "k2_order_bbox")) return r;
+    k2_order_keys<<<grid, 256, 0, c->stream>>>(c->pts.as<Corr>(), n, bb, keys, idx);
+    if (int r = check_launch(c, "k2_order_keys")) return r;
+    CU(cub::DeviceRadixSort::SortPairs(tmp, cub_bytes, keys, keys2, idx, idx2, (int)n, 0, 32, c->stream));
+    k2_order_gather<<<(unsigned)((tiles + kOrderWarps - 1) / kOrderWarps), 32 * kOrderWarps, 0, c->stream>>>(
+        c->pts.as<Corr>(), n, idx2, c->k2pts.as<Corr>(), c->k2box.as<double4>());
+    if (int r = check_launch(c, "k2_order_gather")) return r;
+    c->k2_ready = true;
+    return 0;
+}
+
 static int normalise_from(sfm_ctx* c, const double* xa, const double* ya, const double* xb, const double* yb,
                           int64_t stride, int64_t n, int64_t max_len) {
     if (int r = c->pts.reserve((size_t)n * sizeof(Corr))) return r;
@@ -419,7 +462,9 @@
     k_normalise<<<grid, 256, 0, c->stream>>>(xa, ya, xb, yb, stride, n,
                                              c->batched ? c->offsets.as<long long>() : nullptr,
                                              c->Ks.as<double>(), c->pts.as<Corr>(), c->bounds.as<unsigned long long>());
-    return check_launch(c, "k_normalise");
+    if (int r = check_launch(c, "k_normalise")) return r;
+    c->k2_ready = false;
+    return (!c->batched && n >= kK2SortMin) ? k2_order(c, n) : 0;
 }
 
 static int stage_coords(sfm_ctx* c, double* d, const double* xa, const double* ya, const double* xb, const double* yb,
@@ -714,17 +759,18 @@
     if (variant == SFM_SCORE_SCREEN32 && thr > 1e6) variant = SFM_SCORE_SCREEN;
     const bool f32 = variant == SFM_SCORE_SCREEN32;
     const bool screen = variant != SFM_SCORE_FULL;
-    double thr_pre = f32 ? thr * kThr32Factor : (screen ? thr * (1.0 + 1e-9) : thr * (1.0 + 1e-9) + 1e-22);
+    double thr_pre = f32 ? thr * kThr32Factor : (screen ? thr * kThrScreenFactor : thr * (1.0 + 1e-9) + 1e-22);
     if (f32 && thr_pre < 1e-24) thr_pre = 1e-24;
     if (screen && thr_pre < 1e-280) thr_pre = 1e-280;
     const double s_scale = sqrt(thr_pre);
     const double scale1 = ldexp(1.0, 63 - e2), scale2 = ldexp(1.0, 63 - 2 * e2);
     unsigned long long* acc_dev = nullptr;
     {
-        const void* fn = score_kernel(variant, hpt, G);
+        const bool tiles = c->k2_ready;
+        const void* fn = score_kernel(variant, hpt, G, tiles);
         if (!fn) return fail(SFM_ERR_ARG, "unsupported scoring configuration (variant %d, hpt %d, group %d)", variant, hpt, G);
-        const size_t smem_one = (size_t)kScoreWarps * score_warp_smem(hpt, false);
-        const size_t smem_two = (size_t)kScoreWarps * score_warp_smem(hpt, true);
+        const size_t smem_one = (size_t)kScoreWarps * score_warp_smem(hpt, false, tiles && !f32);
+        const size_t smem_two = (size_t)kScoreWarps * score_warp_smem(hpt, true, false);
         const size_t smem_both = smem_one > smem_two ? smem_one : smem_two;
         const size_t smem = screen ? smem_one : smem_two;
         auto occupancy = [&](const void* f, size_t bytes, int* out) -> int {
@@ -747,12 +793,16 @@
 #endif
         const void* fn_auto = nullptr;
         if (autov && SFM_AUTO_SINGLE) {
-            if (hpt == 2 && G == 16) fn_auto = reinterpret_cast<const void*>(&k_score_auto<2, 16>);
-            if (hpt == 4 && G == 8) fn_auto = reinterpret_cast<const void*>(&k_score_auto<4, 8>);
+            if (hpt == 2 && G == 16)
+                fn_auto = tiles ? reinterpret_cast<const void*>(&k_score_auto<2, 16, MODE_SCREEN>)
+                                : reinterpret_cast<const void*>(&k_score_auto<2, 16, MODE_SCREEN11>);
+            if (hpt == 4 && G == 8)
+                fn_auto = tiles ? reinterpret_cast<const void*>(&k_score_auto<4, 8, MODE_SCREEN>)
+                                : reinterpret_cast<const void*>(&k_score_auto<4, 8, MODE_SCREEN11>);
         }
         if (fn_auto)
             if (int r = occupancy(fn_auto, smem_both, &occ)) return r;
-        const void* fn_full = (autov && !fn_auto) ? score_kernel(SFM_SCORE_FULL, hpt, G) : nullptr;
+        const void* fn_full = (autov && !fn_auto) ? score_kernel(SFM_SCORE_FULL, hpt, G, tiles) : nullptr;
         int occ_full = 0;
         if (fn_full)
             if (int r = occupancy(fn_full, smem_two, &occ_full)) return r;
@@ -763,11 +813,14 @@
         const long long total_items = hblocks * nsplit * P;
         if (int r = c->acc.reserve(H * kAccWords * 8 + acc_tail_bytes(P))) return r;
         const long long npts = c->n;
+        const bool scaled = screen && !f32 && !tiles;
         if (f32) { if (int r = c->spts.reserve((size_t)npts * sizeof(Corr32))) return r; }
-        else if (screen) { if (int r = c->spts.reserve((size_t)npts * sizeof(Corr))) return r; }
+        else if (scaled) { if (int r = c->spts.reserve((size_t)npts * sizeof(Corr))) return r; }
+        const Corr* kpts = (tiles && screen && !f32) ? c->k2pts.as<Corr>() : c->pts.as<Corr>();
         ScoreArgs a;
-        a.pts = c->pts.as<Corr>();
-        a.spts = screen ? c->spts.p : c->pts.p;
+        a.pts = kpts;
+        a.spts = (f32 || scaled) ? c->spts.p : (const void*)kpts;
+        a.boxes = tiles ? c->k2box.as<double4>() : nullptr;
         a.bounds = c->bounds.as<double>();
         a.s = s_scale;
         a.kappa_coef = kKappaCoef * (1.0 + thr);
@@ -795,21 +848,31 @@
         c->tic(T_SCORE);
         if (int r = clear_acc(c, H, P)) return r;
         if (f32 && !skip_k2) {
-            k_screen_pts32<<<(unsigned)((npts + 255) / 256), 256, 0, c->stream>>>(c->pts.as<Corr>(), npts, 1.0 / s_scale,
+            k_screen_pts32<<<(unsigned)((npts + 255) / 256), 256, 0, c->stream>>>(kpts, npts, 1.0 / s_scale,
                                                                                   reinterpret_cast<Corr32*>(c->spts.p));
             if (int r = check_launch(c, "k_screen_pts32")) return r;
         }
-        else if (screen && !skip_k2) {
+        else if ((scaled || autov) && !skip_k2) {
             PilotArgs pa;
             pa.E = c->E.as<double>();
             pa.h = h;
             pa.plen = c->batched ? c->first_len : c->n;
             pa.thr_pre = thr_pre;
+            pa.bounds = a.bounds;
+            pa.kappa_coef = a.kappa_coef;
+            pa.boxes = a.boxes;
             pa.counters = reinterpret_cast<unsigned*>(tailp + 16);
             pa.mode_flag = autov ? reinterpret_cast<int*>(tailp + 32) : nullptr;
-            CU(chain_launch(c, k_screen_pts64, dim3((unsigned)((npts + 255) / 256)), dim3(256), 0, c->pts.as<Corr>(), npts,
-                            1.0 / s_scale, reinterpret_cast<Corr*>(c->spts.p), pa));
-            if (int r = check_launch(c, "k_screen_pts64")) return r;
+            const long long copy_blocks = (npts + 255) / 256;
+            if (scaled) {
+                CU(chain_launch(c, k_screen_pts64, dim3((unsigned)copy_blocks), dim3(256), 0, kpts, npts, 1.0 / s_scale,
+                                reinterpret_cast<Corr*>(c->spts.p), pa));
+                if (int r = check_launch(c, "k_screen_pts64")) return r;
+            } else {
+                CU(chain_launch(c, k_pilot, dim3((unsigned)(copy_blocks < kPilotBlocks ? copy_blocks : kPilotBlocks)), dim3(256),
+                                0, kpts, pa));
+                if (int r = check_launch(c, "k_pilot")) return r;
+            }
         }
         const long long want_blocks = (total_items + kScoreWarps - 1) / kScoreWarps;
         const long long launch_blocks = grid_blocks < want_blocks ? grid_blocks : want_blocks;
@@ -817,7 +880,8 @@
         if (!skip_k2 && fn_auto) {
             ScoreArgs a2 = a;
             a2.thr_pre = thr * (1.0 + 1e-9) + 1e-22;
-            a2.spts = c->pts.p;
+            a2.pts = c->pts.as<Corr>();
+            a2.spts = a2.pts;
             void* kargs2[] = {(void*)&a, (void*)&a2};
             CU(chain_launch_ptr(c, fn_auto, dim3((unsigned)launch_blocks), dim3(kScoreThreads), smem_both, kargs2));
             if (int r = check_launch(c, "k_score_auto")) return r;
@@ -827,7 +891,8 @@
             if (fn_full) {
                 ScoreArgs a2 = a;
                 a2.thr_pre = thr * (1.0 + 1e-9) + 1e-22;
-                a2.spts = c->pts.p;
+                a2.pts = c->pts.as<Corr>();
+                a2.spts = a2.pts;
                 const long long gb2 = (long long)c->sm_count * occ_full;
                 const long long lb2 = gb2 < want_blocks ? gb2 : want_blocks;
                 void* kargs2[] = {(void*)&a2};
@@ -1760,6 +1825,7 @@
         k_normalise<<<dim3((unsigned)((n + 255) / 256), 1), 256, 0, c->stream>>>(s[0], s[1], s[2], s[3], stride, n, nullptr,
                                                                                 c->hK.as<double>(), c->pts.as<Corr>(), nullptr);
         if (int r = check_launch(c, "k_normalise")) return r;
+        c->k2_ready = false;
     } else if (int r = normalise_from(c, s[0], s[1], s[2], s[3], stride, n, max_len)) {
         return r;
     }
diff --git a/structure_from_motion_b200/csrc/sfm_device.cuh b/structure_from_motion_b200/csrc/sfm_device.cuh
--- a/structure_from_motion_b200/csrc/sfm_device.cuh
+++ b/structure_from_motion_b200/csrc/sfm_device.cuh
@@ -46,16 +46,6 @@
     const double na = __dadd_rn(__dmul_rn(la0, la0), __dmul_rn(la1, la1));
     const double nb = __dadd_rn(__dmul_rn(lb0, lb0), __dmul_rn(lb1, lb1));
     return __dmul_rn(__dadd_rn(__drcp_rn(na), __drcp_rn(nb)), __dmul_rn(r, r));
-}
-
-__device__ __forceinline__ double sed_screen(const double (&e)[9], double xa, double ya, double xb,
-                                             double yb, double thr_pre) {
-    const double lb0 = fma(xb, e[0], fma(yb, e[3], e[6]));
-    const double lb1 = fma(xb, e[1], fma(yb, e[4], e[7]));
-    const double lb2 = fma(xb, e[2], fma(yb, e[5], e[8]));
-    const double r = fma(xa, lb0, fma(ya, lb1, lb2));
-    const double nb = fma(lb0, lb0, lb1 * lb1);
-    return fma(r, r, -(thr_pre * nb));
 }
 
 __device__ __forceinline__ double sed_full_decision(const double (&e)[9], double xa, double ya,
diff --git a/structure_from_motion_b200/csrc/sfm_score.cuh b/structure_from_motion_b200/csrc/sfm_score.cuh
--- a/structure_from_motion_b200/csrc/sfm_score.cuh
+++ b/structure_from_motion_b200/csrc/sfm_score.cuh
@@ -56,10 +56,12 @@
 constexpr int kAccWords = 1 + 2 * kChunks;
 constexpr long long kMaxItemPoints = 1ll << 11;
 enum { SUM_S1 = 1, SUM_S2 = 2 };
-enum { MODE_FULL = 0, MODE_SCREEN = 1, MODE_SCREEN32 = 2 };
-constexpr double kKappaCoef = 4e-20;
+enum { MODE_FULL = 0, MODE_SCREEN = 1, MODE_SCREEN32 = 2, MODE_SCREEN11 = 3 };
+constexpr double kKappaCoef = 4.2e-20;
+constexpr double kThrScreenFactor = 1.0 + 3e-9;
 constexpr double kKappa32Coef = 1.2e-10;
 constexpr double kThr32Factor = 1.0316;
+
 
 __global__ void __launch_bounds__(256) k_pad_models(const double* __restrict__ E, long long htotal, ModelRow* __restrict__ rows) {
     const long long i = blockIdx.x * (long long)blockDim.x + threadIdx.x;
@@ -93,6 +95,7 @@
     unsigned* work_counter;
     unsigned long long* acc;
     const int* mode_flag;
+    const double4* boxes;
 };
 
 __device__ __forceinline__ unsigned atom_add_acq_rel_shared(unsigned* p, unsigned v) {
@@ -124,6 +127,108 @@
 struct __align__(16) Corr32 {
     float xa, ya, xb, yb;
 };
+
+__device__ __forceinline__ double tile_bound(const double (&e)[9], double4 box, double thr_pre, double kap) {
+    const double l0 = fma(box.x, e[0], fma(box.y, e[3], e[6]));
+    const double l1 = fma(box.x, e[1], fma(box.y, e[4], e[7]));
+    const double m0 = fma(fabs(e[0]), box.z, fma(fabs(e[3]), box.w, fabs(l0)));
+    const double m1 = fma(fabs(e[1]), box.z, fma(fabs(e[4]), box.w, fabs(l1)));
+    const double t = fma(thr_pre, fma(m0, m0, m1 * m1), kap);
+    return t == t ? t : __longlong_as_double(0x7ff0000000000000LL);
+}
+
+__device__ __forceinline__ unsigned long long k2_ordered(double x) {
+    const unsigned long long b = (unsigned long long)__double_as_longlong(x);
+    return (b >> 63) ? ~b : (b | 0x8000000000000000ull);
+}
+__device__ __forceinline__ double k2_unordered(unsigned long long k) {
+    return __longlong_as_double((long long)((k >> 63) ? (k & 0x7fffffffffffffffull) : ~k));
+}
+
+__global__ void __launch_bounds__(256) k2_order_bbox(const Corr* __restrict__ pts, long long n,
+                                                     unsigned long long* __restrict__ bb) {
+    const long long i = blockIdx.x * (long long)blockDim.x + threadIdx.x;
+    unsigned long long v[4] = {0ull, 0ull, 0ull, 0ull};
+    if (i < n) {
+        const Corr c = pts[i];
+        if (c.xb == c.xb) { v[0] = ~k2_ordered(c.xb); v[2] = k2_ordered(c.xb); }
+        if (c.yb == c.yb) { v[1] = ~k2_ordered(c.yb); v[3] = k2_ordered(c.yb); }
+    }
+#pragma unroll
+    for (int k = 0; k < 4; ++k) {
+#pragma unroll
+        for (int d = 16; d > 0; d >>= 1) {
+            const unsigned long long o = __shfl_xor_sync(0xffffffffu, v[k], d);
+            v[k] = o > v[k] ? o : v[k];
+        }
+    }
+    if ((threadIdx.x & 31) == 0 && i < n)
+#pragma unroll
+        for (int k = 0; k < 4; ++k) atomicMax(bb + k, v[k]);
+}
+
+__device__ __forceinline__ unsigned k2_quantise(double x, double lo, double hi) {
+    const double sc = 65535.0 / (hi - lo);
+    const double q = (sc > 0.0 && sc < 1e308) ? (x - lo) * sc : 0.0;
+    return (unsigned)fmin(fmax(q, 0.0), 65535.0);
+}
+__device__ __forceinline__ unsigned k2_spread16(unsigned v) {
+    v = (v | (v << 8)) & 0x00ff00ffu;
+    v = (v | (v << 4)) & 0x0f0f0f0fu;
+    v = (v | (v << 2)) & 0x33333333u;
+    return (v | (v << 1)) & 0x55555555u;
+}
+__global__ void __launch_bounds__(256) k2_order_keys(const Corr* __restrict__ pts, long long n,
+                                                     const unsigned long long* __restrict__ bb,
+                                                     unsigned* __restrict__ keys, int* __restrict__ idx) {
+    const long long i = blockIdx.x * (long long)blockDim.x + threadIdx.x;
+    if (i >= n) return;
+    const Corr c = pts[i];
+    const unsigned qx = k2_quantise(c.xb, k2_unordered(~bb[0]), k2_unordered(bb[2]));
+    const unsigned qy = k2_quantise(c.yb, k2_unordered(~bb[1]), k2_unordered(bb[3]));
+    keys[i] = (k2_spread16(qy) << 1) | k2_spread16(qx);
+    idx[i] = (int)i;
+}
+
+constexpr int kOrderWarps = 4;
+__global__ void __launch_bounds__(32 * kOrderWarps) k2_order_gather(const Corr* __restrict__ pts, long long n,
+                                                                   const int* __restrict__ idx, Corr* __restrict__ out,
+                                                                   double4* __restrict__ boxes) {
+    const long long t = (long long)blockIdx.x * kOrderWarps + (threadIdx.x >> 5);
+    const int lane = threadIdx.x & 31;
+    if (t * kTile >= n) return;
+    double lo[2] = {__longlong_as_double(0x7ff0000000000000LL), __longlong_as_double(0x7ff0000000000000LL)};
+    double hi[2] = {-lo[0], -lo[1]};
+#pragma unroll
+    for (int k = lane; k < kTile; k += 32) {
+        const long long i = t * kTile + k;
+        if (i < n) {
+            const Corr c = pts[idx[i]];
+            out[i] = c;
+            lo[0] = fmin(lo[0], c.xb); hi[0] = fmax(hi[0], c.xb);
+            lo[1] = fmin(lo[1], c.yb); hi[1] = fmax(hi[1], c.yb);
+        }
+    }
+#pragma unroll
+    for (int d = 16; d > 0; d >>= 1)
+#pragma unroll
+        for (int k = 0; k < 2; ++k) {
+            lo[k] = fmin(lo[k], __shfl_xor_sync(0xffffffffu, lo[k], d));
+            hi[k] = fmax(hi[k], __shfl_xor_sync(0xffffffffu, hi[k], d));
+        }
+    if (lane == 0) {
+        double cw[4];
+        bool finite = true;
+#pragma unroll
+        for (int k = 0; k < 2; ++k) {
+            cw[k] = 0.5 * lo[k] + 0.5 * hi[k];
+            cw[2 + k] = fmax(__dsub_ru(hi[k], cw[k]), __dsub_ru(cw[k], lo[k]));
+            finite = finite && fabs(cw[k]) <= 1.7976931348623157e308 && fabs(cw[2 + k]) <= 1.7976931348623157e308;
+        }
+        boxes[t] = finite ? make_double4(cw[0], cw[1], cw[2], cw[3])
+                          : make_double4(0.0, 0.0, 1.7976931348623157e308, 1.7976931348623157e308);
+    }
+}
 
 constexpr int kPilotBlocks = 32;
 constexpr int kPilotHyps = 64;
@@ -134,43 +239,52 @@
     long long h;
     long long plen;
     double thr_pre;
+    const double* bounds;
+    double kappa_coef;
+    const double4* boxes;
     unsigned* counters;
     int* mode_flag;
 };
-__global__ void __launch_bounds__(256) k_screen_pts64(const Corr* __restrict__ pts, long long n, double inv_s,
-                                                      Corr* __restrict__ spts, const PilotArgs pa) {
-    chain_enter();
-    const long long i = blockIdx.x * (long long)blockDim.x + threadIdx.x;
-    if (i < n) {
-        Corr c = pts[i];
-        c.xa *= inv_s;
-        c.ya *= inv_s;
-        spts[i] = c;
-    }
-    if (!pa.mode_flag || blockIdx.x >= kPilotBlocks) return;
-    const int nb = gridDim.x < kPilotBlocks ? gridDim.x : kPilotBlocks;
+template <bool BOXES>
+__device__ __forceinline__ void pilot_block(const Corr* __restrict__ pts, const PilotArgs& pa, int nb) {
     const long long nh = pa.h < kPilotHyps ? pa.h : kPilotHyps;
     const int hs = threadIdx.x % kPilotHyps;
     int pass = 0, tests = 0;
     if (hs < nh && pa.plen > 0) {
         const long long hyp = (pa.h / nh) * hs;
-        double e[9];
-#pragma unroll
-        for (int k = 0; k < 9; ++k) e[k] = pa.E[9 * hyp + k];
+        double e[9], f2 = 0.0;
+#pragma unroll
+        for (int k = 0; k < 9; ++k) {
+            e[k] = pa.E[9 * hyp + k];
+            f2 = fma(e[k], e[k], f2);
+        }
+        const double kap = f2 * (pa.bounds[0] * pa.bounds[1] * pa.kappa_coef);
         const long long np = pa.plen < kPilotPts ? pa.plen : kPilotPts;
         const long long step = pa.plen / np;
         const int lanes = nb * (256 / kPilotHyps);
         Corr cs[8];
+        double4 bx[8];
         int got = 0;
 #pragma unroll
         for (int u = 0; u < 8; ++u) {
             const long long q = blockIdx.x * (256 / kPilotHyps) + threadIdx.x / kPilotHyps + (long long)u * lanes;
-            if (q < np) { cs[u] = pts[q * step]; got = u + 1; }
+            if (q < np) {
+                cs[u] = pts[q * step];
+                if constexpr (BOXES) bx[u] = pa.boxes[q * step / kTile];
+                got = u + 1;
+            }
         }
 #pragma unroll
         for (int u = 0; u < 8; ++u)
             if (u < got) {
-                pass += sed_screen(e, cs[u].xa, cs[u].ya, cs[u].xb, cs[u].yb, pa.thr_pre) < 0.0 ? 1 : 0;
+                const double lb0 = fma(cs[u].xb, e[0], fma(cs[u].yb, e[3], e[6]));
+                const double lb1 = fma(cs[u].xb, e[1], fma(cs[u].yb, e[4], e[7]));
+                const double lb2 = fma(cs[u].xb, e[2], fma(cs[u].yb, e[5], e[8]));
+                const double r = fma(cs[u].xa, lb0, fma(cs[u].ya, lb1, lb2));
+                double t;
+                if constexpr (BOXES) t = tile_bound(e, bx[u], pa.thr_pre, kap);
+                else t = pa.thr_pre * fma(lb0, lb0, lb1 * lb1);
+                pass += fma(r, r, -t) < 0.0 ? 1 : 0;
                 tests += 1;
             }
     }
@@ -196,6 +310,24 @@
         }
     }
 }
+__global__ void __launch_bounds__(256) k_pilot(const Corr* __restrict__ pts, const PilotArgs pa) {
+    chain_enter();
+    pilot_block<true>(pts, pa, gridDim.x);
+}
+
+__global__ void __launch_bounds__(256) k_screen_pts64(const Corr* __restrict__ pts, long long n, double inv_s,
+                                                      Corr* __restrict__ spts, const PilotArgs pa) {
+    chain_enter();
+    const long long i = blockIdx.x * (long long)blockDim.x + threadIdx.x;
+    if (i < n) {
+        Corr c = pts[i];
+        c.xa *= inv_s;
+        c.ya *= inv_s;
+        spts[i] = c;
+    }
+    if (!pa.mode_flag || blockIdx.x >= kPilotBlocks) return;
+    pilot_block<false>(pts, pa, gridDim.x < kPilotBlocks ? gridDim.x : kPilotBlocks);
+}
 
 __global__ void __launch_bounds__(256) k_screen_pts32(const Corr* __restrict__ pts, long long n, double inv_s,
                                                       Corr32* __restrict__ spts) {
@@ -214,6 +346,11 @@
     uint2 ring[kRing];
     unsigned short own[32];
     unsigned long long full_bar[kStages];
+};
+template <int HPT>
+struct alignas(128) ScoreWarpSmemBox : ScoreWarpSmem<HPT> {
+    double4 box[kStages];
+    double kap[HPT][32];
 };
 
 constexpr int kTileFS = 32;
@@ -229,7 +366,9 @@
 __host__ __device__ constexpr bool score_full_in_smem(int hpt) { return hpt <= 2; }
 template <int HPT, int MODE>
 constexpr size_t score_warp_bytes() {
-    return (MODE == MODE_FULL && score_full_in_smem(HPT)) ? sizeof(ScoreWarpSmemFS<HPT>) : sizeof(ScoreWarpSmem<HPT>);
+    return (MODE == MODE_FULL && score_full_in_smem(HPT)) ? sizeof(ScoreWarpSmemFS<HPT>)
+           : MODE == MODE_SCREEN                          ? sizeof(ScoreWarpSmemBox<HPT>)
+                                                          : sizeof(ScoreWarpSmem<HPT>);
 }
 
 #ifndef SFM_SCORE_MINB4
@@ -248,22 +387,25 @@
 __device__ __forceinline__ void score_body(const ScoreArgs& a) {
     constexpr bool SCREEN = MODE != MODE_FULL;
     constexpr bool F32 = MODE == MODE_SCREEN32;
+    constexpr bool SCALED = F32 || MODE == MODE_SCREEN11;
     using T = typename std::conditional<F32, float, double>::type;
     using P = typename std::conditional<F32, Corr32, Corr>::type;
     constexpr int NB = HPT * G;
     constexpr bool FS = MODE == MODE_FULL && score_full_in_smem(HPT);
     constexpr bool ENTRY = MODE == MODE_FULL;
+    constexpr bool BOX = MODE == MODE_SCREEN;
     constexpr int TILE = FS ? kTileFS : kTile;
     constexpr int STAGES = FS ? kStagesFS : kStages;
     constexpr int AHEAD = FS ? STAGES - 1 : STAGES;
-    using WS = typename std::conditional<FS, ScoreWarpSmemFS<HPT>, ScoreWarpSmem<HPT>>::type;
+    using WS = typename std::conditional<FS, ScoreWarpSmemFS<HPT>,
+                                         typename std::conditional<BOX, ScoreWarpSmemBox<HPT>, ScoreWarpSmem<HPT>>::type>::type;
     static_assert(NB <= 32 && (TILE % G) == 0 && (kTile % TILE) == 0, "a batch is at most 32 tests and divides a tile");
     extern __shared__ __align__(128) unsigned char score_smem[];
     const unsigned full = 0xffffffffu;
     const int lane = threadIdx.x & 31;
     const int warp = __shfl_sync(full, (int)(threadIdx.x >> 5), 0);
     const unsigned lt = lanemask_lt();
-    if (a.mode_flag && *a.mode_flag != MODE) return;
+    if (a.mode_flag && (*a.mode_flag == MODE_FULL) != (MODE == MODE_FULL)) return;
     WS& ws = reinterpret_cast<WS*>(score_smem)[warp];
 
     if (lane == 0) {
@@ -302,21 +444,23 @@
         const double* Ep = a.E + 9 * (long long)pair * a.h;
         const ModelRow* Rw = a.rows + (long long)pair * a.h + hyp_w;
         const Corr* pbeg = a.pts + begin;
-        const P* src = reinterpret_cast<const P*>(SCREEN ? a.spts : (const void*)a.pts);
+        const P* src = reinterpret_cast<const P*>(a.spts);
+        const int box0 = (int)(begin / kTile);
 
         auto issue = [&](int t) {
             const int s = (int)((gt + (unsigned)t) % STAGES);
             const long long first = begin + (long long)t * TILE;
             const long long rem = end - first;
             const uint32_t bytes = (uint32_t)((rem < TILE ? rem : TILE) * sizeof(P));
-            mbar_expect_tx(&ws.full_bar[s], bytes);
+            mbar_expect_tx(&ws.full_bar[s], bytes + (BOX ? (uint32_t)sizeof(double4) : 0u));
             bulk_g2s(&ws.tile[s][0], src + first, bytes, &ws.full_bar[s]);
+            if constexpr (BOX) bulk_g2s(&ws.box[s], a.boxes + box0 + t, (uint32_t)sizeof(double4), &ws.full_bar[s]);
         };
         if (lane == 0) {
             for (int t = 0; t < AHEAD && t < ntiles; ++t) issue(t);
         }
 
-        T e[HPT][9], kap[HPT];
+        T e[HPT][9], kap[HPT], tb[HPT];
 #pragma unroll
         for (int j = 0; j < HPT; ++j) {
             const long long hyp = hyp_w + 32 * j + lane;
@@ -337,9 +481,10 @@
             }
             const double nrm = F32 ? rsqrt(f2) : 1.0;
 #pragma unroll
-            for (int k = 0; k < 9; ++k) e[j][k] = (T)((SCREEN && (k % 3) != 2) ? v[k] * nrm * a.s : v[k] * nrm);
+            for (int k = 0; k < 9; ++k) e[j][k] = (T)((SCALED && (k % 3) != 2) ? v[k] * nrm * a.s : v[k] * nrm);
             if (F32) kap[j] = (T)(real ? ((f2 > 0.0 && f2 < 1e300) ? ab2 : __longlong_as_double(0x7ff0000000000000LL)) : -1.0);
             else kap[j] = (T)(real ? f2 * ab2 : -1.0);
+            if constexpr (BOX) ws.kap[j][lane] = kap[j];
         }
 
         auto accumulate = [&](bool act, double sv, int slot, int owner) {
@@ -461,13 +606,38 @@
             const long long first = begin + (long long)t * TILE;
             const int np = (int)((end - first < TILE) ? (end - first) : TILE);
             const P* tp = reinterpret_cast<const P*>(&ws.tile[s][0]);
+            if constexpr (BOX) {
+                const double4 bx = ws.box[s];
+#pragma unroll
+                for (int j = 0; j < HPT; ++j) tb[j] = tile_bound(e[j], bx, a.thr_pre, ws.kap[j][lane]);
+            }
             for (int p = 0; p < np; p += G) {
                 unsigned pm = 0;
 #pragma unroll
                 for (int g = 0; g < G; ++g) {
                     const P c = tp[p + g];
                     T d[HPT];
-                    if (SCREEN) {
+                    if constexpr (BOX) {
+                        double t0[HPT], t1[HPT], t2[HPT];
+#pragma unroll
+                        for (int j = 0; j < HPT; ++j) {
+                            t0[j] = fma(c.yb, e[j][3], e[j][6]);
+                            t1[j] = fma(c.yb, e[j][4], e[j][7]);
+                            t2[j] = fma(c.yb, e[j][5], e[j][8]);
+                        }
+#pragma unroll
+                        for (int j = 0; j < HPT; ++j) {
+                            t0[j] = fma(c.xb, e[j][0], t0[j]);
+                            t1[j] = fma(c.xb, e[j][1], t1[j]);
+                            t2[j] = fma(c.xb, e[j][2], t2[j]);
+                        }
+#pragma unroll
+                        for (int j = 0; j < HPT; ++j) t2[j] = fma(c.ya, t1[j], t2[j]);
+#pragma unroll
+                        for (int j = 0; j < HPT; ++j) t2[j] = fma(c.xa, t0[j], t2[j]);
+#pragma unroll
+                        for (int j = 0; j < HPT; ++j) d[j] = fma(t2[j], t2[j], -tb[j]);
+                    } else if (SCREEN) {
                         T t0[HPT], t1[HPT], t2[HPT];
 #pragma unroll
                         for (int j = 0; j < HPT; ++j) {
@@ -546,11 +716,11 @@
     score_body<HPT, G, MODE>(a);
 }
 
-template <int HPT, int G>
+template <int HPT, int G, int SMODE>
 __global__ void __launch_bounds__(kScoreThreads, score_min_blocks(HPT)) k_score_auto(const ScoreArgs a, const ScoreArgs a_full) {
     chain_enter();
     if (*a.mode_flag == MODE_FULL) score_body<HPT, G, MODE_FULL>(a_full);
-    else score_body<HPT, G, MODE_SCREEN>(a);
+    else score_body<HPT, G, SMODE>(a);
 }
 
 enum { AGG_SUM = 0, AGG_SQUARE = 1, AGG_MEAN = 2, AGG_RMS = 3 };
```
